# muhanzhang/IGMC

Measured on AMD Instinct MI355X. Metric: enclosing-subgraphs/sec (train step, batch=50) + test RMSE, higher is better.
Workload: dtype f32; 1 GPU; ml_1m, hop 1, max-nodes-per-hop 100, batch 50 per GPU, adj-dropout 0, dynamic-train, ARR 0.001, Adam; parallelism=dp1, global_batch=50, graphs_captured_before_timing=True, steps_per_graph_launch=100, group_steps=50

## Files before the change

### igmc_amd/csrc/capi.hip

```cpp
#include "launch.h"
#include "sortpool.h"
#include "g2_image.h"

#include <algorithm>
#include <climits>
#include <cmath>
#include <cstdio>
#include <cstring>
#include <map>
#include <string>
#include <vector>

static thread_local std::string g_err;
int g_igmc_prof_on = 0;

#define IGMC_FAIL(msg)                                                      \
  do {                                                                      \
    g_err = std::string(__func__) + ": " + (msg);                           \
    return 1;                                                               \
  } while (0)
#define HIPCHECK(expr)                                                      \
  do {                                                                      \
    hipError_t e_ = (expr);                                                 \
    if (e_ != hipSuccess) {                                                 \
// ... 626 lines not shown
  if (!out) IGMC_FAIL("null out");
  if (num_bases != 4) IGMC_FAIL("the gfx950 kernels are built for num_bases == 4 (reference Main.py:393)");
  if (num_relations < 1 || num_relations > 255) IGMC_FAIL("num_relations out of range");
  if (num_relations * num_labels + num_labels + 1 > 320) IGMC_FAIL("num_relations * num_labels too large for the layer-0 gradient kernel");
  if (num_labels < 2 || n_side < 0 || max_nodes < 1 || max_graphs < 1) IGMC_FAIL("bad sizes");
  HIPCHECK(hipSetDevice(device));
  igmc_model* m = new igmc_model();
  m->device = device;
  m->last_B = 0;
  m->last_training = 0;
  m->last_flags = 0;
  m->img_valid = 0;
  m->img_hint = 0;
  m->img_params = nullptr;
  ModelDev& d = m->d;
  d.img_current = 0;
  d.adam_m1 = nullptr;
  d.adam_m2 = nullptr;
  d.R = num_relations;
  d.Bs = 4;
  d.L = num_labels;
  d.S = n_side;
  d.D = 256 + n_side;
  int64_t off = 0;
  for (int l = 0; l < 4; ++l) {
    const int fin = l == 0 ? d.L : 32;
    d.off_basis[l] = off; off += (int64_t)4 * fin * 32;
    d.off_root[l] = off;  off += (int64_t)fin * 32;
    d.off_bias[l] = off;  off += 32;
    d.off_att[l] = off;   off += (int64_t)d.R * 4;
  }
  d.off_l1w = off; off += (int64_t)128 * d.D;
  d.off_l1b = off; off += 128;
  d.off_l2w = off; off += 128;
  d.off_l2b = off; off += 1;
  d.n_params = off;
  d.node_cap = max_nodes;
  d.edge_cap = max_edges;
  d.graph_cap = max_graphs;
  Allocs& M = m->mem;
  int fail = 0;
  const size_t N = (size_t)max_nodes, Bc = (size_t)max_graphs;
  for (int l = 0; l < 4; ++l) fail |= M.get(&d.h[l], N * 32) | M.get(&d.dpre[l], N * 32);
  fail |= M.get(&d.agg, N * 128);
  for (int l = 0; l < 3; ++l) fail |= M.get(&d.gagg[l], N * 128) | M.get(&d.Y[l], N * 128);
  fail |= M.get(&d.feat, Bc * d.D) | M.get(&d.a1, Bc * 128) | M.get(&d.lmask, Bc * 128) | M.get(&d.dz, Bc * 128) |
          M.get(&d.gfeat, Bc * d.D) | M.get(&d.err, Bc) | M.get(&d.cnt0, N * d.R * d.L);
  const size_t rows0 = (size_t)d.R * d.L + d.L + 1;
  d.ts_part = nullptr;
  d.ts_raw = nullptr;
  d.ts_stride = (d.R * 32 + 33) * 32;
  d.fin_stash = nullptr;
  d.datt_part = nullptr;
  if (d.R <= G2_NR * G2_NG_MAX)
  {
    fail |= M.get(&d.ts_part, (size_t)4 * IGMC_TS_BLOCKS * d.ts_stride) |
            M.get(&d.ts_raw, (size_t)4 * d.ts_stride + (size_t)4 * d.ts_stride / 32 * 4);
    if (!fail) d.datt_part = d.ts_raw + (size_t)4 * d.ts_stride;
  }
  if (d.R <= 128) fail |= M.get(&d.fin_stash, (size_t)4 * IGMC_STASH_LAYER + 16);
  d.g2_ex = nullptr;
  d.g2_fx = nullptr;
  d.g2_px = nullptr;
  d.g2_px_stride = 0;
  d.g2_w = nullptr;
  d.g2_graphs = 0;
  d.ex_nodes = 256;
  d.g2_ex_stride = (size_t)Bc * 2 * 32 * d.ex_nodes;
  const int wide = d.R <= G2_NR * G2_NG_MAX;
  const int xcd_ok = igmc_g2_xcd_ok();
  if (wide && Bc <= 2048 && xcd_ok) {
    fail |= M.get(&d.g2_ex, 5 * d.g2_ex_stride) | M.get(&d.g2_fx, Bc * 256) | M.get(&d.g2_w, g2_w_words(d.R, d.L));
    d.g2_graphs = (int)Bc;
    if (d.R <= G2_NR && Bc <= 1024) {
      d.g2_px_stride = (size_t)Bc * 2 * 32768;
      fail |= M.get(&d.g2_px, 5 * d.g2_px_stride);
    } else if (d.R <= G2_NR) {
      static bool told = false;
      if (!told) fprintf(stderr, "[igmc] batches of more than 1024 subgraphs: no plane-exchange regions -- the dense-layer / per-layer kernels take the steps, not the subgraph kernel\n");
      told = true;
    }
  } else if (wide) {
    fail |= M.get(&d.g2_w, g2_w_words(d.R, d.L));
  }
  fail |= M.get(&d.gs_bar, 2 * Bc + 1);
  fail |= M.get(&d.gs_ts, 4);
  d.gs_err = d.gs_bar ? d.gs_bar + 2 * Bc : nullptr;
  fail |= M.get(&d.wg_part, (size_t)4 * IGMC_WG_BLOCKS * igmc_wg_stride()) |
          M.get(&d.gatt_part, (size_t)3 * IGMC_GATHER_BLOCKS * d.R * 4) |
          M.get(&d.l0_part, (size_t)IGMC_L0_BLOCKS * rows0 * 32) |
          M.get(&d.graw, (size_t)3 * igmc_wg_stride() + 3 * d.R * 4 + rows0 * 32) | M.get(&d.arr_part, 4);
  d.side = nullptr;
  d.ctrl = nullptr;
  d.dcat[0] = d.dcat[1] = d.dcat[2] = nullptr;
  fail |= M.get(&m->done_ctr, 8);
  if (fail) {
    M.release();
    delete m;
    IGMC_FAIL("hipMalloc failed (model workspace)");
  }
  {
    hipStream_t st1, st2;
    if (hipStreamCreateWithFlags(&st1, hipStreamNonBlocking) != hipSuccess ||
        hipStreamCreateWithFlags(&st2, hipStreamNonBlocking) != hipSuccess) {
      M.release();
      delete m;
      IGMC_FAIL("hipStreamCreate failed");
    }
    m->ax.s1 = st1;
    m->ax.s2 = st2;
    for (int i = 0; i < 8; ++i) {
      hipEvent_t e;
      if (hipEventCreateWithFlags(&e, hipEventDisableTiming) != hipSuccess) IGMC_FAIL("hipEventCreate failed");
      m->ax.ev[i] = e;
    }
  }
  HIPCHECK(hipMemset(m->done_ctr, 0, 8 * sizeof(int)));
  HIPCHECK(hipMemset(m->d.gs_bar, 0, (2 * (size_t)max_graphs + 1) * sizeof(int)));
  {
    const unsigned long long ts0[4] = {~0ull, 0ull, 0ull, 0ull};
    HIPCHECK(hipMemcpy(m->d.gs_ts, ts0, sizeof(ts0), hipMemcpyHostToDevice));
  }
  if (m->d.g2_ex) {
    HIPCHECK(hipMemset(m->d.g2_ex, 0, 5 * m->d.g2_ex_stride * sizeof(unsigned long long)));
    HIPCHECK(hipMemset(m->d.g2_fx, 0, (size_t)max_graphs * 256 * sizeof(unsigned long long)));
    if (m->d.g2_px) HIPCHECK(hipMemset(m->d.g2_px, 0, 5 * m->d.g2_px_stride));
  }
  if (igmc_model_prepare(d)) {
    M.release();
    delete m;
    IGMC_FAIL("hipFuncSetAttribute failed");
  }
  *out = m;
  return 0;
}

extern "C" int igmc_debug_lin_mask(const igmc_model* m, uint8_t* h_out, int64_t n) {
  if (!m || !h_out) IGMC_FAIL("null argument");
  if (n < 0 || n > (int64_t)m->d.graph_cap * 128) IGMC_FAIL("mask size out of range");
  HIPCHECK(hipDeviceSynchronize());
  HIPCHECK(hipMemcpy(h_out, m->d.lmask, (size_t)n, hipMemcpyDeviceToHost));
  return 0;
}

extern "C" int igmc_debug_head_array(const igmc_model* m, int which, float* h_out, int64_t n) {
  if (!m || !h_out) IGMC_FAIL("null argument");
  if (which < 0 || which > 3) IGMC_FAIL("no such array");
  const float* src = which == 0 ? m->d.a1 : which == 1 ? m->d.dz : which == 2 ? m->d.feat : m->d.gfeat;
  if (n < 0 || n > (int64_t)m->d.graph_cap * (which < 2 ? 128 : m->d.D)) IGMC_FAIL("size out of range");
  HIPCHECK(hipDeviceSynchronize());
  HIPCHECK(hipMemcpy(h_out, src, (size_t)n * sizeof(float), hipMemcpyDeviceToHost));
  return 0;
}

extern "C" void igmc_model_destroy(igmc_model* m) {
  if (!m) return;
  for (int i = 0; i < 8; ++i) hipEventDestroy((hipEvent_t)m->ax.ev[i]);
  hipStreamDestroy((hipStream_t)m->ax.s1);
  hipStreamDestroy((hipStream_t)m->ax.s2);
  m->mem.release();
  delete m;
}

extern "C" int64_t igmc_param_count(const igmc_model* m) { return m ? m->d.n_params : 0; }

extern "C" int64_t igmc_param_offset(const igmc_model* m, int layer, int which, int64_t* count) {
  if (!m) return -1;
  const ModelDev& d = m->d;
  const int fin = (layer == 0) ? d.L : 32;
  int64_t off = -1, n = 0;
  switch (which) {
    case IGMC_P_BASIS: off = d.off_basis[layer & 3]; n = (int64_t)4 * fin * 32; break;
    case IGMC_P_ROOT: off = d.off_root[layer & 3]; n = (int64_t)fin * 32; break;
    case IGMC_P_BIAS: off = d.off_bias[layer & 3]; n = 32; break;
    case IGMC_P_ATT: off = d.off_att[layer & 3]; n = (int64_t)d.R * 4; break;
    case IGMC_P_LIN1_W: off = d.off_l1w; n = (int64_t)128 * d.D; break;
    case IGMC_P_LIN1_B: off = d.off_l1b; n = 128; break;
    case IGMC_P_LIN2_W: off = d.off_l2w; n = 128; break;
    case IGMC_P_LIN2_B: off = d.off_l2b; n = 1; break;
  }
  if (count) *count = n;
  return off;
}

static StepPlan plan_query(const igmc_model* m, const igmc_batch* b, int B) {
  StepPlan sp;
  igmc_step_plan(m->d, b->d, B, IGMC_CALL_STEP, &sp);
  return sp;
}

extern "C" int igmc_model_dense_layers(const igmc_model* m, const igmc_batch* b, int B) {
  return (m && b) ? plan_query(m, b, B).dense_layers : 0;
}

extern "C" int igmc_model_dense_path(const igmc_model* m, const igmc_batch* b, int B) {
  return (m && b) ? plan_query(m, b, B).family == IGMC_FAM_G2 : 0;
}

extern "C" int igmc_model_step_form(const igmc_model* m, const igmc_batch* b, int B) {
  return (m && b) ? plan_query(m, b, B).step_form : 0;
}

extern "C" int igmc_model_step_geometry(const igmc_model* m, const igmc_batch* b, int B, int32_t* out, int n) {
  if (!m || !b || !out || n < 0) IGMC_FAIL("bad arguments");
// ... 215 lines not shown
  if (n < 1 || n > (int64_t)INT32_MAX) IGMC_FAIL("n must be in [1, 2^31)");
  if (nq < 0 || nq > (int64_t)INT32_MAX) IGMC_FAIL("nq must be in [0, 2^31)");
  if (ns < 1 || geometry < 0 || geometry > IGMC_SEGSEL_MAX_SPLIT) IGMC_FAIL("ns must be at least 1, geometry in [0, 64]");
  igmc_launch_rank_segments(d_keys, d_ids, n, d_seg_off, ns, d_q_off, d_q_id, nq,
                            geometry > 0 ? geometry : igmc_segsel_default_split(ns), d_q_pos, d_q_rank, d_err, stream);
  HIPCHECK(hipGetLastError());
  return 0;
}
extern "C" int igmc_rank_metrics(const int32_t* d_q_rank, const int64_t* d_q_off, const uint8_t* d_q_rel, int64_t nq, int ns,
                                 const int32_t* d_ks, int nk, int32_t* d_cnt, double* d_dcg, int32_t* d_err, int grid,
                                 void* stream) {
  if (!d_q_off || !d_ks || !d_cnt || !d_dcg || !d_err) IGMC_FAIL("null argument");
  if (nq > 0 && !d_q_rank) IGMC_FAIL("null argument");
  if (nq < 0 || nq > (int64_t)INT32_MAX) IGMC_FAIL("nq must be in [0, 2^31)");
  if (ns < 1 || nk < 1 || nk > IGMC_RANK_MAX_KS || grid < 0 || grid > 65536)
    IGMC_FAIL("ns must be at least 1, nk in [1, 8], grid in [0, 65536]");
  igmc_launch_rank_metrics(d_q_rank, d_q_off, d_q_rel, d_ks, nk, ns, nq, grid, d_cnt, d_dcg, d_err, stream);
  HIPCHECK(hipGetLastError());
  return 0;
}

extern "C" int igmc_ctrl_tick(int64_t* d_ctrl, void* stream) {
  if (!d_ctrl) IGMC_FAIL("null ctrl");
  igmc_launch_tick(d_ctrl, stream);
  HIPCHECK(hipGetLastError());
  return 0;
}
extern "C" int igmc_ctrl_regroup(int64_t* d_ctrl, int M, int64_t first_cur, int64_t first_next, void* stream) {
  if (!d_ctrl || M < 1 || first_cur < 0 || first_next < 0) IGMC_FAIL("bad arguments");
  igmc_launch_regroup(d_ctrl, M, first_cur, first_next, stream);
  HIPCHECK(hipGetLastError());
  return 0;
}
extern "C" int igmc_ctrl_gate(int64_t* d_ctrl, int q, int gk_min, double delay_us, int delay_always, double timeout_us,
                              void* stream) {
  if (!d_ctrl || gk_min < 0 || !(timeout_us >= 0.0) || !(delay_us >= 0.0) || delay_us > 1000.0) IGMC_FAIL("bad arguments");
  igmc_launch_gate(d_ctrl, q & 1, gk_min, (long long)(delay_us * 100.0), delay_always != 0, (long long)(timeout_us * 100.0), stream);
  HIPCHECK(hipGetLastError());
  return 0;
}
extern "C" int igmc_batch_set_ctrl(igmc_batch* b, const int64_t* d_ctrl) {
  if (!b) IGMC_FAIL("null batch");
  b->ctrl = d_ctrl;
  return 0;
}
extern "C" int igmc_model_set_ctrl(igmc_model* m, const int64_t* d_ctrl) {
  if (!m) IGMC_FAIL("null model");
  m->d.ctrl = d_ctrl;
  return 0;
}
extern "C" int igmc_model_reset_exchange(igmc_model* m, void* stream) {
  if (!m) IGMC_FAIL("null model");
  hipStream_t st = (hipStream_t)stream;
  if (m->d.g2_ex) {
    HIPCHECK(hipMemsetAsync(m->d.g2_ex, 0, 5 * m->d.g2_ex_stride * sizeof(unsigned long long), st));
    HIPCHECK(hipMemsetAsync(m->d.g2_fx, 0, (size_t)m->d.g2_graphs * 256 * sizeof(unsigned long long), st));
    if (m->d.g2_px) HIPCHECK(hipMemsetAsync(m->d.g2_px, 0, 5 * m->d.g2_px_stride, st));
  }
  return 0;
}
extern "C" int igmc_model_check(igmc_model* m, void* stream) {
  if (!m) IGMC_FAIL("null model");
  int v = 0;
  if (m->d.gs_err) {
    HIPCHECK(hipStreamSynchronize((hipStream_t)stream));
    HIPCHECK(hipMemcpy(&v, m->d.gs_err, sizeof(int), hipMemcpyDeviceToHost));
    if (v) {
      HIPCHECK(hipMemset(m->d.gs_bar, 0, (2 * (size_t)m->d.graph_cap + 1) * sizeof(int)));
      (void)igmc_model_reset_exchange(m, stream);
      HIPCHECK(hipStreamSynchronize((hipStream_t)stream));
      IGMC_FAIL("a workgroup-cluster exchange of k_graph_step2 timed out (GPU shared with another job?): results of the "
                "affected steps are invalid; set IGMC_GS_CLUSTER=1 or IGMC_GRAPH_STEP=0");
    }
  }
  return 0;
}
extern "C" int igmc_adam_step_ctrl(float* d_params, const float* d_grad, float* d_exp_avg, float* d_exp_avg_sq,
                                   int64_t n, const int64_t* d_ctrl, void* stream) {
  if (!d_params || !d_grad || !d_exp_avg || !d_exp_avg_sq || n <= 0 || !d_ctrl) IGMC_FAIL("bad arguments");
  igmc_launch_adam(d_params, d_grad, d_exp_avg, d_exp_avg_sq, n, 0.f, 0.f, 0.f, 0.f, 0.f, 0.f, (int64_t*)d_ctrl, 0, stream);
  HIPCHECK(hipGetLastError());
  return 0;
}

extern "C" int igmc_step_finish(igmc_model* m, const igmc_batch* b, float* d_params, const float* d_grad,
                                float* d_exp_avg, float* d_exp_avg_sq, float ARR, float* d_loss, double* d_total,
                                int64_t* d_ctrl, int64_t step, float lr, float beta1, float beta2, float eps,
                                float weight_decay, void* stream) {
  if (!m || !b || !d_params || !d_grad || !d_exp_avg || !d_exp_avg_sq || !d_loss) IGMC_FAIL("bad arguments");
  if (!d_ctrl && step < 1) IGMC_FAIL("step must be >= 1");
  const AdamScalars as = adam_scalars(d_ctrl, step, lr, beta1, beta2);
  igmc_launch_finish(m->d, b->d, d_params, d_grad, d_exp_avg, d_exp_avg_sq, as.step_size, as.inv_sqrt_bc2, beta1, beta2, eps,
                     weight_decay, d_ctrl, ARR, d_loss, d_total, m->last_flags, stream);
  m->img_valid = 0;
  m->img_hint = 0;
  HIPCHECK(hipGetLastError());
  return 0;
}

extern "C" int igmc_train_step(igmc_model* m, float* d_params, const igmc_batch* b, int use_edge_flags,
                               const uint8_t* d_lin_mask, uint64_t seed, uint64_t step, float multiply_by, float ARR,
                               float* d_out, float* d_grad, float* d_exp_avg, float* d_exp_avg_sq, float* d_loss,
                               double* d_total, int64_t* d_ctrl, int64_t adam_t, float lr, float beta1, float beta2,
                               float eps, float weight_decay, void* stream) {
  std::string why;
  if (check_call(m, b, d_params && d_out && d_grad && d_exp_avg && d_exp_avg_sq && d_loss, &why)) IGMC_FAIL(why);
  if (!d_ctrl && adam_t < 1) IGMC_FAIL("adam_t must be >= 1");
  const AdamScalars as = adam_scalars(d_ctrl, adam_t, lr, beta1, beta2);
  const StepPlan sp = begin_call(m, b, IGMC_CALL_STEP, stream);
  ImgScope img(m, d_params);
  int emitted = 0;
  igmc_launch_train_step(m->d, b->d, sp, d_params, b->last_B, use_edge_flags, d_lin_mask, seed, step, multiply_by, ARR,
                         d_out, d_grad, d_exp_avg, d_exp_avg_sq, as.step_size, as.inv_sqrt_bc2, beta1, beta2, eps, weight_decay,
                         d_ctrl, m->done_ctr, d_loss, d_total, stream, 0.f, nullptr, &emitted);
  img.done_updated(emitted);
  HIPCHECK(hipGetLastError());
  end_call(m, b, 1, use_edge_flags);
  return 0;
}

#define IGMC_MAX_PEERS 16
struct igmc_comm {
  void* nccl;
  int rank, world, device;
  igmc_allreduce_fn host_fn;
// ... 564 lines not shown
```

### igmc_amd/csrc/g2_compose.h

```cpp
#pragma once

__global__ __launch_bounds__(G2C_THREADS) void k_g2_compose(ModelDev m, const float* P, float* w) {
  __shared__ float s_att[4 * G2_NR * G2_NG_MAX];
  const int tid = threadIdx.x, R = m.R, L = m.L, RL = R * L, LF = L * 32;
  const int ng = g2_groups(R, L);
  const int tableb = 2 * 3 * ng * (G2_NR + 1);
  const int mi = (int)(blockIdx.x >> 1);
  const int l = ((int)blockIdx.x >= tableb) ? 0 : 1 + mi / (ng * (G2_NR + 1)), trans = blockIdx.x & 1;
  if ((int)blockIdx.x >= tableb) {
    const int c0 = 32 * ((int)blockIdx.x - tableb);
    const float attv = (tid < R * 4) ? P[m.off_att[0] + tid] : 0.f;
    float bv[4][4], rv[4];
#pragma unroll
    for (int q = 0; q < 4; ++q) {
      const int i = tid + q * G2C_THREADS, c = c0 + (i >> 5), f = i & 31;
      const int cf = (c < RL) ? (c % L) * 32 + f : 0;
#pragma unroll
      for (int bb = 0; bb < 4; ++bb) bv[q][bb] = (c < RL) ? P[m.off_basis[0] + bb * LF + cf] : 0.f;
      rv[q] = (c >= RL && c < RL + L) ? P[m.off_root[0] + (c - RL) * 32 + f] : ((c == RL + L) ? P[m.off_bias[0] + f] : 0.f);
    }
    if (tid < 4 * G2_NR * G2_NG_MAX) s_att[tid] = attv;
    __syncthreads();
#pragma unroll
    for (int q = 0; q < 4; ++q) {
// ... 32 lines not shown
      } else {
#pragma unroll
        for (int q = 0; q < 4; ++q) bq[bb][q] = basis[bb * 1024 + (4 * kg + q) * 32 + n];
      }
    }
    float at[4];
#pragma unroll
    for (int bb = 0; bb < 4; ++bb) at[bb] = P[m.off_att[l] + r * 4 + bb];
#pragma unroll
    for (int q = 0; q < 4; ++q) v[q] = g2_wsum(at[0], at[1], at[2], at[3], bq[0][q], bq[1][q], bq[2][q], bq[3][q]);
  }
  uint32_t h01, m01, l01, h23, m23, l23;
  g2_split2(v[0], v[1], h01, m01, l01);
  g2_split2(v[2], v[3], h23, m23, l23);
  const int lane = (kg & 3) * 16 + (n & 15), nt = n >> 4, e0 = 4 * (kg >> 2);
  const uint32_t t3[3][2] = {{h01, h23}, {m01, m23}, {l01, l23}};
#pragma unroll
  for (int t = 0; t < G2_NT; ++t)
    *(uint2*)(img + ((size_t)(((t * (G2_NR + 1) + blk) * 2 + nt) * 64 + lane)) * 8 + e0) = make_uint2(t3[t][0], t3[t][1]);
}

static int igmc_g2_layout(const ModelDev& m, const BatchDev& b, int cs, G2Layout* lay) {
  const int RL = m.R * m.L;
  if (m.S != 0 || m.D != 256 || m.R > G2_NR || m.L > 8 || RL + m.L + 1 > 32 || !m.ts_part || !m.g2_px || !m.g2_fx || !m.g2_w || !b.relm) return 0;
  const int half = 2 * cs;
  const int cmax = b.cap_u > b.cap_v ? b.cap_u : b.cap_v;
  if (cmax > 16 * half || cmax > 128) return 0;
  if (b.graph_cap > m.g2_graphs) return 0;
  const int kmax = ((cmax + 31) >> 5) << 5;
  lay->kp = kmax + 8;
  lay->nsides = (cs == 1) ? 2 : 1;
  lay->rmr = ((cmax + 15) >> 4) << 4;
  lay->rmc = kmax;
  int o = 0;
  lay->pside = ((G2_NT * 32 * lay->kp * 2 + 1023) & ~1023) >> 2;
  lay->planes = o; o += lay->nsides * lay->pside;
  lay->ohp = o; o += lay->nsides * (8 * lay->kp >> 1);
  lay->lab = o; o += 64;
  lay->xo = o; o += 2 * G2_NB * 16 * G2_XP;
  lay->hs = o; o += G2_NB * 16 * G2_XP;
  int tw = G2_NB * 16 * G2_TP;
  if (tw < (G2_THREADS / 64) * 256) tw = (G2_THREADS / 64) * 256;
  const int rw = 2 * lay->rmr * (lay->rmc + 8) / 4;
  if (rw > tw) tw = rw;
  if (tw < 1024) tw = 1024;
  lay->tile = o; o += tw;
  lay->hist = o; o += G2_NB * 16 * G2_XP;
  lay->px = o; o += G2_NB * 2 * 64 * 4;
  lay->wreg = o; o += G2_WIMG;
  lay->t0 = o; o += 1024;
  lay->att = o; o += 64;
  lay->head = o; o += 256 + 256 + 3 * 128 + 512 + 16;
  lay->words = o;
  return (size_t)o * 4 <= 160 * 1024;
}

__global__ void k_g2_xcc_probe(int* out) {
  if (threadIdx.x == 0) out[blockIdx.x] = (int)(g2_xcc_id() & 15ull);
}
int igmc_g2_xcd_ok() {
#ifdef IGMC_HIPEMU
  return 1;
#else
  static int oks[64];
  static bool init = false;
  if (!init) {
    for (int i = 0; i < 64; ++i) oks[i] = -1;
    init = true;
  }
  int dev = 0;
  if (hipGetDevice(&dev) != hipSuccess || dev < 0 || dev >= 64) dev = 0;
  int& ok = oks[dev];
  if (ok >= 0) return ok;
  ok = 0;
  int* d = nullptr;
  int h[64];
  if (hipMalloc((void**)&d, sizeof(h)) != hipSuccess) return ok;
  hipLaunchKernelGGL(k_g2_xcc_probe, dim3(64), dim3(64), 0, 0, d);
  if (hipMemcpy(h, d, sizeof(h), hipMemcpyDeviceToHost) == hipSuccess) {
    ok = 1;
    for (int b = 0; b + 8 < 64; ++b)
      if (h[b] != h[b + 8]) ok = 0;
  }
  (void)hipFree(d);
  if (!ok) fprintf(stderr, "[igmc] device %d: workgroups b and b + 8 of a launch do not share an XCD: the subgraph kernel and the one-launch dense layers are not used\n", dev);
  return ok;
#endif
}

int g_igmc_compose_count = 0;

int igmc_launch_graph_step2(const ModelDev& m, const BatchDev& b, const StepPlan& sp, const float* P, int B, int training,
                            int use_flags, const uint8_t* inj_mask, uint64_t seed, uint64_t step, float mult, float grad_scale,
                            float* out, void* stream) {
  const G2Layout& lay = sp.lay;
  const int cs = sp.cs;
  G2Args a;
  memset(&a, 0, sizeof(a));
  a.n_users = b.n_users; a.n_items = b.n_items; a.B = B; a.s_lab = b.s_lab; a.relm = b.relm; a.y = b.y;
  a.cap_u = b.cap_u; a.cap_v = b.cap_v; a.slot = b.slot; a.relm_ld = b.relm_ld; a.graph_cap = b.graph_cap;
  a.R = m.R; a.L = m.L; a.D = m.D; a.ts_stride = m.ts_stride;
  for (int l = 0; l < 4; ++l) {
    a.h[l] = m.h[l];
    a.off_bias[l] = (int)m.off_bias[l];
  }
  a.ts_part = m.ts_part; a.g2_px = m.g2_px; a.g2_fx = m.g2_fx; a.g2_px_stride = m.g2_px_stride; a.g2_w = m.g2_w;
  a.gs_bar = m.gs_bar; a.gs_err = m.gs_err; a.a1 = m.a1; a.dz = m.dz; a.feat = m.feat; a.gfeat = m.gfeat; a.err = m.err;
  a.lmask = m.lmask; a.ctrl = m.ctrl;
  a.off_l1w = (int)m.off_l1w; a.off_l1b = (int)m.off_l1b; a.off_l2w = (int)m.off_l2w; a.off_l2b = (int)m.off_l2b;
  a.P = P;
  a.inj_mask = inj_mask;
  a.seed = seed;
  a.step = step;
  a.mult = mult;
  a.grad_scale = grad_scale;
  a.out = out;
  a.lay2 = lay;
  a.timing = getenv("IGMC_GS_TIMING") ? 1 : 0;
  a.ts = (g_igmc_prof_on == 2) ? m.gs_ts : nullptr;
  a.self_seq = (!training || a.ts) ? 1 : 0;
  a.cs = cs;
  a.stride = (cs > 1) ? ((B + 7) & ~7) : 1;
  const int grid = sp.grid;
  const size_t sm = (size_t)lay.words * 4;
  if (!m.img_current) {
    IGMC_PLAUNCH("k_g2_compose", k_g2_compose, 2 * 3 * g2_groups(m.R, m.L) * (G2_NR + 1) + g2_t0_rows(m.R, m.L) / 32, G2C_THREADS, 0, stream, m, P, m.g2_w);
    ++g_igmc_compose_count;
  }
#ifdef IGMC_HIPEMU
  if (cs > 1) {
    hipemu::rt().co_cs = cs;
    hipemu::rt().co_stride = 8;
    hipemu::rt().co_block = 8 * cs;
  }
#endif
  if (getenv("IGMC_GS_TRACE")) fprintf(stderr, "[igmc] k_graph_step B=%d train=%d flags=%d v2 kp=%d lds=%zu cluster=%d grid=%d\n", B, training, use_flags, lay.kp, sm, cs, grid);
  igmc_dispatch([&](auto uf, auto tr, auto cl) {
    IGMC_PLAUNCH(tr() ? "k_graph_step" : "k_graph_fwd", (k_graph_step2<uf(), tr(), cl()>), grid, G2_THREADS, sm, stream, a);
  }, use_flags != 0, training != 0, cs > 1);
  return a.self_seq ? 0 : 1;
}

int igmc_dl_prepare();
int igmc_gs_prepare() { return igmc_g2_prepare(); }
int igmc_g2_prepare() {
  if (igmc_dl_prepare()) return 1;
  (void)igmc_g2_xcd_ok();
#ifndef IGMC_HIPEMU
  const int mx = 160 * 1024;
  const void* fns[8] = {(const void*)k_graph_step2<true, true, true>,   (const void*)k_graph_step2<false, true, true>,
                        (const void*)k_graph_step2<true, false, true>,  (const void*)k_graph_step2<false, false, true>,
                        (const void*)k_graph_step2<true, true, false>,  (const void*)k_graph_step2<false, true, false>,
                        (const void*)k_graph_step2<true, false, false>, (const void*)k_graph_step2<false, false, false>};
  for (const void* fn : fns)
    if (hipFuncSetAttribute(fn, hipFuncAttributeMaxDynamicSharedMemorySize, mx) != hipSuccess) return 1;
#endif
  return 0;
}
```

### igmc_amd/csrc/g2_prims.h

```cpp
#pragma once

#ifdef IGMC_HIPEMU
#define G2_STAMP(k) do { } while (0)
#else
#define G2_STAMP(k)                                                                                        \
  do {                                                                                                     \
    if (a.timing && threadIdx.x == 0) {                                                                    \
      if (blockIdx.x == 0) g_g2_clk[k] = __builtin_readcyclecounter();                                     \
      else if (a.cs > 2 && (int)blockIdx.x == 8 * (a.cs / 2) && (k) < 40) g_g2_clk[64 + (k)] = __builtin_readcyclecounter(); \
    }                                                                                                      \
  } while (0)
#endif

#ifdef IGMC_HIPEMU
#define DL_STAMP(k) do { } while (0)
#else
#define DL_STAMP(k)                                                                               \
  do {                                                                                            \
    if (a.timing && threadIdx.x == 0 && (int)blockIdx.x == a.timing - 1 && (k) < 128)             \
      g_g2_clk[k] = __builtin_readcyclecounter();                                                 \
  } while (0)
#endif

#ifdef IGMC_HIPEMU
// ... 23 lines not shown
  const uint32_t eq = ~(t + 0x7F7F7F7Fu) & 0x80808080u;
  const uint32_t mask = (eq >> 7) * 0xFFu;
#ifdef IGMC_HIPEMU
  o01 = ((mask & 0xFFu) ? 0x3F80u : 0u) | ((mask & 0xFF00u) ? 0x3F800000u : 0u);
  o23 = ((mask & 0xFF0000u) ? 0x3F80u : 0u) | ((mask & 0xFF000000u) ? 0x3F800000u : 0u);
#else
  o01 = __builtin_amdgcn_perm(mask, mask, 0x01010000u) & 0x3F803F80u;
  o23 = __builtin_amdgcn_perm(mask, mask, 0x03030202u) & 0x3F803F80u;
#endif
}

template <bool FLAGS>
__device__ __forceinline__ uint32_t g2_bytemask(uint32_t w, uint32_t r1, int keepbit) {
  uint32_t mk = w & (0x01010101u * IGMC_RELM_CODE);
  if (FLAGS) mk &= ((w >> keepbit) & 0x01010101u) * IGMC_RELM_CODE;
  const uint32_t t = mk ^ (0x01010101u * r1);
  const uint32_t eq = ~(t + 0x7F7F7F7Fu) & 0x80808080u;
  return (eq >> 7) * 0xFFu;
}
__device__ __forceinline__ u32x4 g2_mask_frag(uint32_t m0, uint32_t m1) {
  u32x4 f;
#ifdef IGMC_HIPEMU
  f[0] = ((m0 & 0xFFu) ? 0x3F80u : 0u) | ((m0 & 0xFF00u) ? 0x3F800000u : 0u);
  f[1] = ((m0 & 0xFF0000u) ? 0x3F80u : 0u) | ((m0 & 0xFF000000u) ? 0x3F800000u : 0u);
  f[2] = ((m1 & 0xFFu) ? 0x3F80u : 0u) | ((m1 & 0xFF00u) ? 0x3F800000u : 0u);
  f[3] = ((m1 & 0xFF0000u) ? 0x3F80u : 0u) | ((m1 & 0xFF000000u) ? 0x3F800000u : 0u);
#else
  f[0] = __builtin_amdgcn_perm(m0, m0, 0x01010000u) & 0x3F803F80u;
  f[1] = __builtin_amdgcn_perm(m0, m0, 0x03030202u) & 0x3F803F80u;
  f[2] = __builtin_amdgcn_perm(m1, m1, 0x01010000u) & 0x3F803F80u;
  f[3] = __builtin_amdgcn_perm(m1, m1, 0x03030202u) & 0x3F803F80u;
#endif
  return f;
}

__device__ __forceinline__ float g2_tanh(float x) {
#ifdef IGMC_HIPEMU
  return tanhf(x);
#else
  return 1.f - 2.f * __builtin_amdgcn_rcpf(1.f + __expf(2.f * x));
#endif
}

template <int AUX = 0>
__device__ __forceinline__ void g2_glds16(const float4* src_wave, float4* lds_wave, int lane) {
#ifndef IGMC_HIPEMU
  __builtin_amdgcn_global_load_lds((const __attribute__((address_space(1))) void*)(src_wave + lane),
                                   (__attribute__((address_space(3))) void*)lds_wave, 16, 0, AUX);
#else
  lds_wave[lane] = src_wave[lane];
#endif
}

__device__ __forceinline__ void g2_pub_f32(unsigned long long* p, float v, uint32_t tag) {
#ifndef IGMC_HIPEMU
  __hip_atomic_store(p, ((unsigned long long)tag << 32) | (unsigned long long)__float_as_uint(v), __ATOMIC_RELAXED,
                     __HIP_MEMORY_SCOPE_WAVEFRONT);
#else
  uint32_t bits;
  memcpy(&bits, &v, 4);
  *p = ((unsigned long long)tag << 32) | (unsigned long long)bits;
#endif
}

#define G2_PX_BYTES 32768
#define G2_PX_FLAGS 28672
#define DLX_PX_BYTES 65536
#define DLX_PX_FLAGS 61440
__device__ __forceinline__ void g2_publish_planes(unsigned char* px, int kp, int f, int node0, const float (&v)[4]) {
  uint32_t h0, m0, l0, h1, m1, l1;
  g2_split2(v[0], v[1], h0, m0, l0);
  g2_split2(v[2], v[3], h1, m1, l1);
  unsigned char* p = px + ((size_t)f * kp + node0) * 2;
  const size_t ts = (size_t)32 * kp * 2;
  *(uint2*)p = make_uint2(h0, h1);
  *(uint2*)(p + ts) = make_uint2(m0, m1);
  *(uint2*)(p + 2 * ts) = make_uint2(l0, l1);
}
__device__ __forceinline__ void g2_flag_raise(unsigned char* px, int slot, uint32_t tag, int lane, int flags_off = G2_PX_FLAGS) {
#ifndef IGMC_HIPEMU
  asm volatile("s_waitcnt vmcnt(0)" ::: "memory");
  if (lane == 0) __hip_atomic_store((unsigned long long*)(px + flags_off) + slot, (unsigned long long)tag, __ATOMIC_RELAXED, __HIP_MEMORY_SCOPE_WAVEFRONT);
#else
  if (lane == 0) ((unsigned long long*)(px + flags_off))[slot] = (unsigned long long)tag;
#endif
}
__device__ __forceinline__ void g2_flags_wait(const unsigned char* px, int n, uint32_t tag, int lane, int* err, int flags_off = G2_PX_FLAGS) {
  const unsigned long long* fl = (const unsigned long long*)(px + flags_off);
  for (long it = 0;; ++it) {
#ifndef IGMC_HIPEMU
    const unsigned long long w = (lane < n) ? __hip_atomic_load(fl + lane, __ATOMIC_RELAXED, __HIP_MEMORY_SCOPE_AGENT) : (unsigned long long)tag;
#else
    const unsigned long long w = (lane < n) ? fl[lane] : (unsigned long long)tag;
#endif
    if (__ballot(w != (unsigned long long)tag) == 0ull) break;
    if (it > (1L << 20)) {
      *err = 1;
      break;
    }
#ifndef IGMC_HIPEMU
    __builtin_amdgcn_s_sleep(1);
#else
    hipemu::yield();
#endif
  }
}
__device__ __forceinline__ void g2_planes_load_exact(uint32_t* pl, const unsigned char* px, int bytes, int wave, int lane, int nwaves) {
  const int pieces = (bytes + 1023) >> 10;
  for (int c = wave; c < pieces; c += nwaves)
    if (c * 1024 + lane * 16 < bytes) g2_glds16<16>((const float4*)px + c * 64, (float4*)pl + c * 64, lane);
}
__device__ __forceinline__ void g2_planes_load(uint32_t* pl, const unsigned char* px, int kp, int wave, int lane, int nwaves) {
  const int pieces = (192 * kp + 1023) >> 10;
  for (int c = wave; c < pieces; c += nwaves) g2_glds16<16>((const float4*)px + c * 64, (float4*)pl + c * 64, lane);
}

__device__ __forceinline__ float g2_poll_f32(const unsigned long long* p, uint32_t tag, int* err) {
  for (long it = 0;; ++it) {
#ifndef IGMC_HIPEMU
    const unsigned long long w = __hip_atomic_load(p, __ATOMIC_RELAXED, __HIP_MEMORY_SCOPE_AGENT);
#else
    const unsigned long long w = *p;
#endif
    if ((uint32_t)(w >> 32) == tag) return __uint_as_float((uint32_t)w);
    if (it > (1L << 22)) {
      *err = 1;
      return 0.f;
    }
#ifndef IGMC_HIPEMU
    __builtin_amdgcn_s_sleep(2);
#else
    hipemu::yield();
#endif
  }
}

#ifdef IGMC_HIPEMU
#define G2_SCHED_BARRIER() do { } while (0)
#else
#define G2_SCHED_BARRIER() __builtin_amdgcn_sched_barrier(0)
#endif

__device__ __forceinline__ uint32_t g2_ld_seq(const int* gs_bar) {
#ifndef IGMC_HIPEMU
  return (uint32_t)__hip_atomic_load(gs_bar + 1, __ATOMIC_RELAXED, __HIP_MEMORY_SCOPE_AGENT);
#else
  return (uint32_t)gs_bar[1];
#endif
}
__device__ __forceinline__ bool g2_last_workgroup_advances(int* gs_bar) {
#ifndef IGMC_HIPEMU
  if (__hip_atomic_fetch_add(gs_bar, 1, __ATOMIC_RELAXED, __HIP_MEMORY_SCOPE_AGENT) != (int)gridDim.x - 1) return false;
  __hip_atomic_store(gs_bar, 0, __ATOMIC_RELAXED, __HIP_MEMORY_SCOPE_AGENT);
  __hip_atomic_fetch_add(gs_bar + 1, 1, __ATOMIC_RELAXED, __HIP_MEMORY_SCOPE_AGENT);
  return true;
#else
  if (gs_bar[0]++ != (int)gridDim.x - 1) return false;
  gs_bar[0] = 0;
  gs_bar[1] += 1;
  return true;
#endif
}
__device__ __forceinline__ void g2_wait_vm0() {
#ifndef IGMC_HIPEMU
  asm volatile("s_waitcnt vmcnt(0)" ::: "memory");
#endif
}
__device__ __forceinline__ unsigned long long g2_wall_clock() {
#ifndef IGMC_HIPEMU
  return (unsigned long long)wall_clock64();
#else
  return 0ull;
#endif
}
__device__ __forceinline__ unsigned long long g2_xcc_id() {
#ifndef IGMC_HIPEMU
  return (unsigned long long)__builtin_amdgcn_s_getreg((20 << 0) | (0 << 6) | (3 << 11));
#else
  return 0ull;
#endif
}
__device__ __forceinline__ void g2_clock_open(unsigned long long* ts) {
#ifndef IGMC_HIPEMU
  atomicMin(ts, (unsigned long long)wall_clock64());
#else
  (void)ts;
#endif
}
__device__ __forceinline__ void g2_clock_close(unsigned long long* ts, unsigned long long t1) {
// ... 23 lines not shown
```

### igmc_amd/csrc/g2_subgraph.h

```cpp
#pragma once

struct G2Args {
  const int32_t* n_users;
  const int32_t* n_items;
  int B;
  const uint8_t* s_lab;
  const uint8_t* relm;
  const float* y;
  int cap_u, cap_v, slot, relm_ld, graph_cap;
  int R, L, D, ts_stride;
  float* h[4];
  float* ts_part;
  unsigned char* g2_px;
  unsigned long long* g2_fx;
  size_t g2_px_stride;
  const float* g2_w;
  int* gs_bar;
  int* gs_err;
  float* a1;
  float* dz;
  float* feat;
  float* gfeat;
  float* err;
  uint8_t* lmask;
  const int64_t* ctrl;
  int off_bias[4];
  int off_l1w, off_l1b, off_l2w, off_l2b;
  const float* P;
  const uint8_t* inj_mask;
  uint64_t seed, step;
  float mult, grad_scale;
  float* out;
  unsigned long long* ts;
  int timing, cs, stride, self_seq;
  G2Layout lay2;
};

template <bool FLAGS, bool TRAIN, bool ONCE>
__global__ __launch_bounds__(G2_THREADS) void k_graph_step2(G2Args a) {
  __builtin_amdgcn_s_setprio(3);
  const float* P = a.P;
  IGMC_DYN_SMEM(smem);
  float* S = (float*)smem;
  const G2Layout lay = a.lay2;
  const int kp = lay.kp, nsides = lay.nsides;
  uint32_t* PLN = (uint32_t*)(S + lay.planes);
  uint32_t* OHP = (uint32_t*)(S + lay.ohp);
  unsigned char* slab = (unsigned char*)(S + lay.lab);
  float* XOA = S + lay.xo;
  float* HSS = S + lay.hs;
  float* TILES = S + lay.tile;
  float* HIST = S + lay.hist;
  float* PXA = S + lay.px;
  float2* sW2 = (float2*)(S + lay.wreg);
  float* sT0 = S + lay.t0;
  float* sfeat = S + lay.head;
  float* sgf = sfeat + 256;
  float* sa1 = sgf + 256;
  float* skeep = sa1 + 128;
  float* sdz = skeep + 128;
  float* sred = sdz + 128;
  float* misc = sred + 512;
  const int R = a.R, L = a.L, RL = R * L;
  const int tid = threadIdx.x, lane = tid & 63, wave = tid >> 6;
  const int li = lane & 15, kq = lane >> 4;
  const int B = a.B;
  const int ts = a.ts_stride;
  const int cs = a.cs;
  const int cm = (cs > 1) ? (int)((blockIdx.x >> 3) % cs) : 0;
  const int half = 2 * cs;
  const uint32_t seq = g2_ld_seq(a.gs_bar);
  const uint32_t tag0 = seq * 8u + 1u;
  const uint64_t step = a.ctrl ? (uint64_t)a.ctrl[IGMC_CTRL_STEP] : a.step;
  if (a.ts && tid == 0) g2_clock_open(a.ts);
  auto xtag = [&](int x) { return tag0 + (uint32_t)x; };
  G2_STAMP(0);
  if (a.timing && tid == 0 && blockIdx.x < 1024) {
    g_g2_wg[blockIdx.x][0] = g2_wall_clock();
    g_g2_wg[blockIdx.x][2] = g2_xcc_id();
  }

  const int g_first = (cs > 1) ? (int)(blockIdx.x / (8 * cs)) * 8 + (int)(blockIdx.x & 7) : (int)blockIdx.x;
  const int g_pre = (g_first < a.graph_cap) ? g_first : a.graph_cap - 1;
  const int pre_cu = a.n_users[g_pre], pre_cv = a.n_items[g_pre];
  const int ld = a.relm_ld;
  auto load_label = [&](int g2) {
    const int hi = (tid >> 7) & 1, t7 = tid & 127;
    const int capx = a.cap_u + hi * (a.cap_v - a.cap_u);
    return (int)a.s_lab[(size_t)g2 * a.slot + hi * a.cap_u + ((t7 < capx) ? t7 : 0)];
  };
  int labv_raw = 0;
  if (tid < 256) g2_glds16((const float4*)(a.g2_w + 6 * G2_WIMG) + (tid & ~63), (float4*)sT0 + (tid & ~63), tid & 63);
  const int tslot = (cs > 1) ? g_first + cm * a.stride : (int)blockIdx.x;
  f32x4 acc0 = (f32x4){0.f, 0.f, 0.f, 0.f};
  bool first_graph = true;
  G2_STAMP(1);

  int g = g_first;
  if (g < B) do {
    int tid_g = threadIdx.x;
    G2_OPAQUE(tid_g);
    const int tid = tid_g, lane = tid & 63, wave = tid >> 6;
    const int li = lane & 15, kq = lane >> 4;
    const int bw = wave >> 1, hf = wave & 1;
    const int gw = cm * G2_NB + bw;
    const int side = gw / half, bi = gw - side * half;
    labv_raw = load_label(g);
    uint32_t bw0[G2_KS], bw1[G2_KS];
    {
      const unsigned char* rmg = a.relm + (size_t)g * a.cap_u * ld;
      const uint32_t rrow = (uint32_t)(16 * bi + li);
#pragma unroll
      for (int s = 0; s < G2_KS; ++s) {
        const uint32_t c0 = (uint32_t)(32 * s + 8 * kq);
        if (side == 0) {
          const uint32_t* p4 = (const uint32_t*)(rmg + (rrow * (uint32_t)ld + c0));
          bw0[s] = p4[0];
          bw1[s] = p4[1];
        } else {
          const unsigned char* pc = rmg + (c0 * (uint32_t)ld + rrow);
          bw0[s] = (uint32_t)pc[0] | ((uint32_t)pc[ld] << 8) | ((uint32_t)pc[2 * ld] << 16) | ((uint32_t)pc[3 * ld] << 24);
          bw1[s] = (uint32_t)pc[4 * ld] | ((uint32_t)pc[5 * ld] << 8) | ((uint32_t)pc[6 * ld] << 16) | ((uint32_t)pc[7 * ld] << 24);
        }
      }
    }
    G2_STAMP(48);
    {
      const float4 z4 = make_float4(0.f, 0.f, 0.f, 0.f);
      for (int i = tid; i < 2 * G2_NB * 16 * G2_XP / 4; i += G2_THREADS) ((float4*)XOA)[i] = z4;
      for (int i = tid; i < G2_NB * 16 * G2_XP / 4; i += G2_THREADS) ((float4*)HIST)[i] = z4;
    }
    G2_STAMP(49);
    const int cu = first_graph ? pre_cu : a.n_users[g], cv = first_graph ? pre_cv : a.n_items[g];
// ... 426 lines not shown
            for (int s4 = 0; s4 < 4; ++s4) {
              av[s4] = Hb[(4 * s4 + kq) * G2_XP + m2w * 16 + li];
              const float* tb = Tb + (4 * s4 + kq) * G2_TP + li;
              const float* db = Db + (4 * s4 + kq) * G2_XP + li;
#pragma unroll
              for (int i3 = 0; i3 < 3; ++i3) {
                const int nt = 3 * wo + i3;
                bw3[s4][i3] = (nt < 2 * G2_NR) ? tb[nt * 16] : db[(nt - 2 * G2_NR) * 16];
              }
            }
            G2_SCHED_BARRIER();
#pragma unroll
            for (int s4 = 0; s4 < 4; ++s4)
#pragma unroll
              for (int i3 = 0; i3 < 3; ++i3)
                w3[i3] = __builtin_amdgcn_mfma_f32_16x16x4f32(av[s4], bw3[s4][i3], w3[i3], 0, 0, 0);
          }
#pragma unroll
          for (int i3 = 0; i3 < 3; ++i3) {
            const int m2 = m2w, nt = 3 * wo + i3;
            const int r = nt >> 1;
            if (r >= R && r < G2_NR) continue;
            float* pp = wpart + (kq * 4) * 32 + li + (r < R ? r : R) * 1024 + m2 * 512 + (nt & 1) * 16;
            if (first_graph) {
#pragma unroll
              for (int rr = 0; rr < 4; ++rr) pp[rr * 32] = w3[i3][rr];
            } else {
#pragma unroll
              for (int rr = 0; rr < 4; ++rr) pp[rr * 32] += w3[i3][rr];
            }
          }
        }
        G2_STAMP(22 + 5 * (3 - l));
        if (l > 1) fetch(6 - l);
        __syncthreads();
        G2_STAMP(23 + 5 * (3 - l));
      }

      if (wave < 4) {
        const int m2 = wave >> 1, wn = wave & 1;
        for (int wb = 0; wb < G2_NB; ++wb) {
          const float* Hb = HIST + wb * 16 * G2_XP;
          const float* Db = XOA + (G2_NB + wb) * 16 * G2_XP;
#pragma unroll
          for (int s4 = 0; s4 < 4; ++s4)
            acc0 = __builtin_amdgcn_mfma_f32_16x16x4f32(Hb[(4 * s4 + kq) * G2_XP + m2 * 16 + li],
                                                        Db[(4 * s4 + kq) * G2_XP + wn * 16 + li], acc0, 0, 0, 0);
        }
      }
      first_graph = false;
      __syncthreads();
      G2_STAMP(34);
    }
  } while (!ONCE && (g += (int)gridDim.x) < B);

  if (TRAIN && wave < 4) {
    float* part0 = a.ts_part + (size_t)tslot * ts;
    const int m2 = wave >> 1, wn = wave & 1;
#pragma unroll
    for (int rr = 0; rr < 4; ++rr) {
      const int c = m2 * 16 + kq * 4 + rr;
      if (c < RL + L + 1) part0[c * 32 + wn * 16 + li] = acc0[rr];
    }
  }
  if (tid == 0 && a.self_seq) {
    const unsigned long long t1 = a.ts ? g2_wall_clock() : 0ull;
    if (g2_last_workgroup_advances(a.gs_bar) && a.ts) g2_clock_close(a.ts, t1);
  }
  G2_STAMP(35);
  if (a.timing && tid == 0 && blockIdx.x < 1024) g_g2_wg[blockIdx.x][1] = g2_wall_clock();
}

extern "C" int igmc_debug_g2_wg_clocks(unsigned long long* out, int n_wg) {
#ifndef IGMC_HIPEMU
  if (n_wg > 1024) n_wg = 1024;
  if (hipDeviceSynchronize() != hipSuccess) return 1;
  if (hipMemcpyFromSymbol(out, HIP_SYMBOL(g_g2_wg), (size_t)n_wg * 3 * sizeof(unsigned long long)) != hipSuccess) return 1;
#else
  for (int i = 0; i < 3 * n_wg; ++i) out[i] = 0;
#endif
  return 0;
}

extern "C" int igmc_debug_g2_clocks(unsigned long long* out, int n) {
#ifndef IGMC_HIPEMU
  if (n > 128) n = 128;
  if (hipDeviceSynchronize() != hipSuccess) return 1;
  if (hipMemcpyFromSymbol(out, HIP_SYMBOL(g_g2_clk), (size_t)n * sizeof(unsigned long long)) != hipSuccess) return 1;
#else
  for (int i = 0; i < n; ++i) out[i] = 0;
#endif
  return 0;
}
```

### igmc_amd/csrc/graphstep2.hip

```cpp
#include "launch.h"
#include "g2_image.h"
#include "head_sub.h"
#include <stdlib.h>
#include <stdio.h>
#include <string.h>

#define G2_THREADS 512
#define G2_NB 4
#define G2C_THREADS 256
#define G2_KS 4
#define G2_TP (G2_NR * 32 + 4)
#define G2_XP 36
#define G2_FXTAG 7

__device__ unsigned long long g_g2_clk[128];
__device__ unsigned long long g_g2_wg[1024][3];
#include "g2_prims.h"

template <typename Frag>
__device__ __forceinline__ void g2_gather_h(const uint32_t* pl, int kp, int nks, Frag frag, int li, int kq, int hf, f32x4 (&acc)[G2_NR]) {
#pragma unroll
  for (int r = 0; r < G2_NR; ++r) acc[r] = (f32x4){0.f, 0.f, 0.f, 0.f};
  const int tstride = 32 * kp >> 1;
  const uint32_t* base = pl + ((16 * hf + li) * kp >> 1) + 4 * kq;
  u32x4 pf[2][G2_NT];
  auto request = [&](int s, int buf) {
#pragma unroll
    for (int sp = 0; sp < G2_NT; ++sp) pf[buf][sp] = *(const u32x4*)(base + sp * tstride + 16 * s);
  };
  request(0, 0);
#pragma unroll
  for (int s = 0; s < G2_KS; ++s) {
    if (s < nks) {
      if (s + 1 < G2_KS) request(s + 1, (s + 1) & 1);
      G2_SCHED_BARRIER();
#pragma unroll
      for (int r = 0; r < G2_NR; ++r) {
        const u32x4 fr = frag(r, s);
#pragma unroll
        for (int q = 0; q < G2_NT; ++q) acc[r] = g2_mfma_bf16(pf[s & 1][q], fr, acc[r]);
      }
      G2_SCHED_BARRIER();
    }
  }
}

__device__ __forceinline__ void g2_transform_h(const f32x4 (&acc)[G2_NR], const float* xrows, const uint32_t* sW, int li, int kq, int hf,
                                               f32x4 (&o)[2]) {
  f32x4 o0a = (f32x4){0.f, 0.f, 0.f, 0.f}, o0b = o0a, o1a = o0a, o1b = o0a;
  const float4 xv = *(const float4*)(xrows + li * G2_XP + 16 * hf + 4 * kq);
  const uint2* wf = (const uint2*)sW + 2 * (kq * 16 + li) + hf;
  uint2 bf[2][2 * G2_NT][2];
  auto request = [&](int st, int buf) {
#pragma unroll
    for (int t = 0; t < G2_NT; ++t)
// ... 114 lines not shown
```

### igmc_amd/csrc/launch.h

```cpp
#pragma once
#include "model.h"
#include <string.h>
#include <type_traits>

size_t igmc_extract_smem_bytes(const GraphDev& g);
void igmc_launch_extract(const GraphDev& g, const BatchDev& b, const int32_t* link_u, const int32_t* link_v,
                         const float* link_y, const int32_t* link_idx, int first, int B, int replay,
                         double sample_ratio, uint64_t seed, uint64_t epoch, const int64_t* ctrl, int lean, void* stream);
void igmc_launch_extract_set(const GraphDev& g, const BatchDev* d_set, const BatchDev& b0, int count, const int32_t* link_u,
                             const int32_t* link_v, const float* link_y, const int32_t* link_idx, int sel0, int B,
                             double sample_ratio, uint64_t seed, const int64_t* ctrl, float drop_p, int force_undirected,
                             uint64_t drop_seed, void* stream);
void igmc_launch_emit(const BatchDev& b, int B, void* stream);
void igmc_launch_emit_nodes(const BatchDev& b, int B, void* stream);
void igmc_launch_load_nodes(const BatchDev& b, const int64_t* uoff, const int32_t* unodes, const uint8_t* udist,
                            const int64_t* voff, const int32_t* vnodes, const uint8_t* vdist, const float* link_y,
                            const int32_t* link_idx, int first, int B, const int64_t* ctrl, void* stream);
void igmc_launch_edge_flags(const BatchDev& b, float p, int force_undirected, uint64_t seed, uint64_t step,
                            const int64_t* ctrl, void* stream);
void igmc_launch_relm_flags(const BatchDev& b, void* stream);
void igmc_launch_relm_dropout(const BatchDev& b, int B, float p, int force_undirected, uint64_t seed, uint64_t step,
                              const int64_t* ctrl, void* stream);
void igmc_launch_tick(int64_t* ctrl, void* stream);
void igmc_launch_regroup(int64_t* ctrl, int M, int64_t first_cur, int64_t first_next, void* stream);
// ... 51 lines not shown
                                 void* stream);
int igmc_segsel_default_split(int ns);
void igmc_launch_select_segments(const float* keys, const int64_t* seg_off, int ns, int num, int k, void* scratch,
                                 int32_t* idx_out, float* key_out, int32_t* count, void* stream);
#define IGMC_RANK_MAX_KS 8
void igmc_launch_rank_segments(const float* keys, const int32_t* ids, int64_t n, const int64_t* seg_off, int ns,
                               const int64_t* q_off, const int32_t* q_id, int64_t nq, int k, int32_t* q_pos, int32_t* q_rank,
                               int32_t* err, void* stream);
void igmc_launch_rank_metrics(const int32_t* q_rank, const int64_t* q_off, const uint8_t* q_rel, const int32_t* ks, int nk,
                              int ns, int64_t nq, int grid, int32_t* cnt, double* dcg, int32_t* err, void* stream);
int igmc_model_prepare(const ModelDev& m);
void igmc_launch_adam(float* p, const float* g, float* m1, float* m2, int64_t n, float step_size,
                      float inv_sqrt_bc2, float beta1, float beta2, float eps, float wd, int64_t* ctrl, int tick,
                      void* stream);
void igmc_launch_finish(const ModelDev& m, const BatchDev& b, float* p, const float* g, float* m1, float* m2,
                        float step_size, float inv_sqrt_bc2, float beta1, float beta2, float eps, float wd,
                        int64_t* ctrl, float ARR, float* loss, double* total, int use_flags, void* stream);

int igmc_g2_xcd_ok();
struct G2Layout {
  int kp, nsides, rmr, rmc, pside;
  int planes, ohp, lab, xo, hs, tile, hist, px, wreg, t0, att, head, words;
};
void igmc_launch_side_gather(const float* src, int S, const int32_t* link_idx, int first, int B, const int64_t* ctrl,
                             float* dst, void* stream);
int igmc_gs_prepare();
int igmc_g2_prepare();

#define IGMC_CALL_EVAL 0
#define IGMC_CALL_CONV 1
#define IGMC_CALL_STEP 2
#define IGMC_FAM_ROWS 0
#define IGMC_FAM_G2 1
#define IGMC_FAM_DLF 2
#define IGMC_FAM_DL 3
#define IGMC_TAIL_HANDOFF 0
#define IGMC_TAIL_TS 1
#define IGMC_TAIL_BS 2
struct StepPlan {
  int kind;
  int fast_head;
  int family;
  int cs, grid;
  G2Layout lay;
  int wide, dl, dlts, dlf, dlb;
  int nqu, nqv, dl_grid;
  int gsplit;
  int self_seq;
  int head_inside;
  int bwd_dense;
  int need_y;
  int tail;
  int exchange_inside;
  int needs_csr;
  int dense_layers;
  int step_form;
};
void igmc_step_plan(const ModelDev& m, const BatchDev& b, int B, int kind, StepPlan* p);
int igmc_dl_always();
void igmc_launch_g2_compose(const ModelDev& m, const float* P, void* stream);
void igmc_launch_dl_layer0(const ModelDev& m, const BatchDev& b, int B, int training, int use_flags, void* stream);
struct DlHead {
  const float* P;
  const uint8_t* inj_mask;
  uint64_t seed, step;
  float mult, grad_scale;
  float* out;
};
void igmc_launch_dl_bwd(const ModelDev& m, const BatchDev& b, const StepPlan& sp, int B, int use_flags, void* stream,
                        const DlHead* head = nullptr, int dense3 = 0);
void igmc_launch_dl_fwd(const ModelDev& m, const BatchDev& b, const StepPlan& sp, const float* P, int B, int training,
                        int use_flags, float* zero_out, void* stream);
void igmc_launch_head_sub(const ModelDev& m, const BatchDev& b, const float* P, int B, const uint8_t* inj_mask, uint64_t seed,
                          uint64_t step, float mult, float grad_scale, float* out, void* stream);
void igmc_launch_dl_layer(const ModelDev& m, const BatchDev& b, const float* P, int B, int l, int bwd, int use_flags,
                          float* zero_out, void* stream, int tables = 0);
int igmc_launch_graph_step2(const ModelDev& m, const BatchDev& b, const StepPlan& sp, const float* P, int B, int training,
                            int use_flags, const uint8_t* inj_mask, uint64_t seed, uint64_t step, float mult, float grad_scale,
                            float* out, void* stream);

void igmc_prof_begin(const char* name, void* stream);
void igmc_prof_end(void* stream);
extern int g_igmc_prof_on;

#define IGMC_PLAUNCH(name, kern, grid, block, shmem, stream, ...)          \
  do {                                                                     \
    if (g_igmc_prof_on == 1) igmc_prof_begin(name, stream);                \
    IGMC_LAUNCH(kern, grid, block, shmem, stream, __VA_ARGS__);            \
    if (g_igmc_prof_on == 1) igmc_prof_end(stream);                        \
  } while (0)

template <typename F>
static inline void igmc_dispatch(F&& f) { f(); }
template <typename F, typename... Rest>
static inline void igmc_dispatch(F&& f, bool v, Rest... rest) {
  if (v) igmc_dispatch([&](auto... cs) { f(std::true_type{}, cs...); }, rest...);
  else igmc_dispatch([&](auto... cs) { f(std::false_type{}, cs...); }, rest...);
}
```

### igmc_amd/csrc/model.h

```cpp
#pragma once
#include "common.h"

#define IGMC_KCAT 160
#ifndef IGMC_WG_BLOCKS
#define IGMC_WG_BLOCKS 64
#endif
#define IGMC_STASH_LAYER 672
#define IGMC_TS_BLOCKS 256
#define IGMC_GATHER_BLOCKS 4096
#define IGMC_FBS_MAX_R 32
#define IGMC_L0_BLOCKS 256
#define IGMC_HG 8

struct ModelDev {
  int R, Bs, L, S, D;
  int64_t off_basis[4], off_root[4], off_bias[4], off_att[4];
  int64_t off_l1w, off_l1b, off_l2w, off_l2b, n_params;
  int node_cap, edge_cap, graph_cap;
  float* h[4];
  float* agg;
  float* gagg[3];
  float* Y[3];
  float* dpre[4];
  float* feat;
  float* a1;
  uint8_t* lmask;
  float* dz;
  float* gfeat;
  float* err;
  uint16_t* cnt0;
  float* wg_part;
  float* gatt_part;
  float* l0_part;
  float* graw;
  float* ts_part;
  float* ts_raw;
  int ts_stride;
  float* fin_stash;
  float* datt_part;
  int* gs_bar;
  int* gs_err;
  unsigned long long* gs_ts;
  unsigned long long* g2_ex;
  size_t g2_ex_stride;
  unsigned long long* g2_fx;
  unsigned char* g2_px;
  size_t g2_px_stride;
  int g2_graphs;
  float* g2_w;
  int ex_nodes;
  int img_current;
  const float* adam_m1;
  const float* adam_m2;
  float* arr_part;
  const float* dcat[3];
  const float* side;
  const int64_t* ctrl;
};

static inline int igmc_wg_stride() { return 32 * IGMC_KCAT + 32; }

__device__ __forceinline__ float igmc_wave_sum_f(float v) {
#pragma unroll
  for (int d = 32; d >= 1; d >>= 1) v += __shfl_xor(v, d, 64);
  return v;
}
__device__ __forceinline__ float igmc_group16_sum_f(float v) {
#ifdef IGMC_HIPEMU
#pragma unroll
  for (int d = 8; d >= 1; d >>= 1) v += __shfl_xor(v, d, 16);
  return v;
#else
  v += __int_as_float(__builtin_amdgcn_update_dpp(0, __float_as_int(v), 0x128, 0xf, 0xf, false));
  v += __int_as_float(__builtin_amdgcn_update_dpp(0, __float_as_int(v), 0x124, 0xf, 0xf, false));
  v += __int_as_float(__builtin_amdgcn_update_dpp(0, __float_as_int(v), 0x122, 0xf, 0xf, false));
  v += __int_as_float(__builtin_amdgcn_update_dpp(0, __float_as_int(v), 0x121, 0xf, 0xf, false));
  return v;
#endif
}
__device__ __forceinline__ float igmc_block_sum_f(float v, float* sm) {
  v = igmc_wave_sum_f(v);
  const int lane = threadIdx.x & 63, wave = threadIdx.x >> 6;
  if (lane == 0) sm[wave] = v;
  __syncthreads();
  float tot = 0.f;
  const int nw = (blockDim.x + 63) >> 6;
  for (int w = 0; w < nw; ++w) tot += sm[w];
  __syncthreads();
  return tot;
}

__device__ __forceinline__ void ctrl_advance(int64_t* ctrl) {
// ... 18 lines not shown
```

### igmc_amd/csrc/model.hip

```cpp
#include "model.h"
#include "g2_image.h"
#include <stdlib.h>

struct XcdSeg {
  int lo, hi;
  int j, nj;
};
__device__ __forceinline__ XcdSeg igmc_xcd_segment(const BatchDev& b) {
  XcdSeg s;
  const int B = b.totals[3];
  const int x = blockIdx.x & 7;
  s.j = blockIdx.x >> 3;
  s.nj = (gridDim.x + 7 - x) >> 3;
  s.lo = b.node_off[(x * B) >> 3];
  s.hi = b.node_off[((x + 1) * B) >> 3];
  return s;
}


template <bool FLAGS, bool STORE>
__global__ __launch_bounds__(IGMC_BLOCK) void k_l0_fwd(BatchDev b, ModelDev m, const float* __restrict__ P,
                                                         float* __restrict__ out) {
  igmc_kernarg_warm<sizeof(BatchDev) + sizeof(ModelDev) + 32>();
  IGMC_DYN_SMEM(smem);
  const int RL = m.R * m.L, LF = m.L * 32;
  float* sW0 = (float*)smem;
  float* sroot = sW0 + RL * 32;
  float* sbias = sroot + LF;
  int* shist = (int*)(sbias + 32);
  for (int i = threadIdx.x; i < RL * 32; i += IGMC_BLOCK) {
    const int r = i / LF, cf = i % LF;
    float s = 0.f;
#pragma unroll
    for (int bb = 0; bb < 4; ++bb) s += P[m.off_att[0] + r * 4 + bb] * P[m.off_basis[0] + bb * LF + cf];
    sW0[i] = s;
  }
  for (int i = threadIdx.x; i < LF; i += IGMC_BLOCK) sroot[i] = P[m.off_root[0] + i];
  if (threadIdx.x < 32) sbias[threadIdx.x] = P[m.off_bias[0] + threadIdx.x];
  __syncthreads();
  const int N = b.totals[0];
  const int lane = threadIdx.x & 63, wave = threadIdx.x >> 6;
  const int grp = lane >> 4, t = lane & 15;
  int* hist = shist + wave * RL;
  const XcdSeg seg = igmc_xcd_segment(b);
  (void)N;
  for (int i = seg.lo + seg.j * 4 + wave; i < seg.hi; i += seg.nj * 4) {
    float ax = 0.f, ay = 0.f;
    if (STORE) {
      for (int c = lane; c < RL; c += 64) hist[c] = 0;
      IGMC_WAVE_SYNC();
    }
    const int beg = b.row_ptr[i], end = b.row_ptr[i + 1];
    for (int c0 = beg + grp * 16; c0 < end; c0 += 64) {
      const int e = c0 + t;
// ... 1038 lines not shown
#pragma unroll
    for (int u = 0; u < 8; ++u) {
      const bool ok = g0 + 4 * u + kq < B;
      if (!ok) { av[u] = 0.f; bv[u] = 0.f; }
      if (extra) {
        dpv[u] = ok ? (from_err ? 2.f * dpv[u] * grad_scale : dpv[u]) * mult : 0.f;
        ad[u] = (ok && mk[u]) ? ad[u] * drop_scale : 0.f;
      }
    }
#pragma unroll
    for (int u = 0; u < 8; ++u) {
      acc = __builtin_amdgcn_mfma_f32_16x16x4f32(av[u], bv[u], acc, 0, 0, 0);
      if (extra) {
        accb1 = __builtin_amdgcn_mfma_f32_16x16x4f32(av[u], (g0 + 4 * u + kq < B) ? 1.f : 0.f, accb1, 0, 0, 0);
        accw2 = __builtin_amdgcn_mfma_f32_16x16x4f32(ad[u], dpv[u], accw2, 0, 0, 0);
        accb2 = __builtin_amdgcn_mfma_f32_16x16x4f32(1.f, dpv[u], accb2, 0, 0, 0);
      }
    }
  }
#pragma unroll
  for (int rr = 0; rr < 4; ++rr) grad[m.off_l1w + (int64_t)(j0 + kq * 4 + rr) * D + n0 + li] = acc[rr];
  if (extra && li == 0) {
#pragma unroll
    for (int rr = 0; rr < 4; ++rr) {
      grad[m.off_l1b + j0 + kq * 4 + rr] = accb1[rr];
      grad[m.off_l2w + j0 + kq * 4 + rr] = accw2[rr];
    }
    if (bx == 0 && kq == 0) grad[m.off_l2b] = accb2[0];
  }
}

__global__ __launch_bounds__(IGMC_BLOCK) void k_head_bwd_w_mfma(BatchDev b, ModelDev m, const float* __restrict__ P,
                                                                  const float* __restrict__ gout, int from_err,
                                                                  float grad_scale, float mult, float drop_scale,
                                                                  float* __restrict__ grad) {
  igmc_kernarg_warm<sizeof(BatchDev) + sizeof(ModelDev) + 32>();
  head_bwd_w_body(b, m, P, gout, from_err, grad_scale, mult, drop_scale, grad, blockIdx.x, blockIdx.y);
}

__global__ __launch_bounds__(IGMC_BLOCK) void k_wgrad_head(BatchDev b, ModelDev m, const float* __restrict__ P,
                                                             const float* __restrict__ gout, int from_err,
                                                             float grad_scale, float mult, float drop_scale,
                                                             float* __restrict__ grad, int nsl) {
  igmc_kernarg_warm<sizeof(BatchDev) + sizeof(ModelDev) + 32>();
  if ((int)blockIdx.y < nsl) {
    wgrad_body(b, m, blockIdx.y);
  } else {
    const int ny = (m.D / 16 + 3) / 4;
    if ((int)blockIdx.x < 8 * ny)
      head_bwd_w_body(b, m, P, gout, from_err, grad_scale, mult, drop_scale, grad, blockIdx.x & 7, blockIdx.x >> 3);
  }
}

__device__ __forceinline__ void fin_stash_body(const ModelDev& m, const float* __restrict__ P, int l, const int64_t* ctrl);

__global__ __launch_bounds__(IGMC_BLOCK) void k_reduce_partials(ModelDev m, int n_gatt_parts, int l0_mfma,
                                                                  int n_wg_parts, const float* __restrict__ P,
                                                                  const int64_t* ctrl, int nstash) {
  igmc_kernarg_warm<sizeof(ModelDev) + 32>();
  __shared__ float sred[4][64];
  if (nstash && (int)blockIdx.x >= (int)gridDim.x - nstash) {
    fin_stash_body(m, P, (int)blockIdx.x - ((int)gridDim.x - nstash), ctrl);
    return;
  }
  const int wgs = 32 * IGMC_KCAT + 32, na = m.R * 4, rows0 = m.R * m.L + m.L + 1, n0 = rows0 * 32;
  const int nlay = l0_mfma ? 4 : 3;
  const int nblkA = (nlay * wgs + 63) / 64, nblkB = (3 * na + 3) / 4, nblkC = l0_mfma ? 0 : (n0 + 63) / 64;
  const int lane = threadIdx.x & 63, wave = threadIdx.x >> 6;
  int blk = blockIdx.x;
  if (blk < nblkA + nblkC) {
    const bool secA = blk < nblkA;
    const int o = (secA ? blk : blk - nblkA) * 64 + lane;
    const int nout = secA ? nlay * wgs : n0;
    float s = 0.f;
    if (o < nout) {
      if (secA) {
        const int l = o / wgs, i = o % wgs;
        const float* p = m.wg_part + (size_t)l * IGMC_WG_BLOCKS * wgs + i;
        for (int k0 = wave; k0 < n_wg_parts; k0 += 64) {
          float v[16];
#pragma unroll
          for (int u = 0; u < 16; ++u) {
            const int k = k0 + 4 * u;
            v[u] = p[(size_t)(k < n_wg_parts ? k : n_wg_parts - 1) * wgs];
          }
#pragma unroll
          for (int u = 0; u < 16; ++u)
            if (k0 + 4 * u < n_wg_parts) s += v[u];
        }
      } else {
        const float* p = m.l0_part + o;
        for (int k0 = wave; k0 < IGMC_L0_BLOCKS; k0 += 64) {
          float v[16];
#pragma unroll
          for (int u = 0; u < 16; ++u) {
            const int k = k0 + 4 * u;
            v[u] = p[(size_t)(k < IGMC_L0_BLOCKS ? k : IGMC_L0_BLOCKS - 1) * n0];
          }
#pragma unroll
          for (int u = 0; u < 16; ++u)
            if (k0 + 4 * u < IGMC_L0_BLOCKS) s += v[u];
        }
      }
    }
    sred[wave][lane] = s;
    __syncthreads();
    if (wave == 0 && o < nout) {
      const float tot = (sred[0][lane] + sred[1][lane]) + (sred[2][lane] + sred[3][lane]);
      if (secA && o >= 3 * wgs) {
        const int i = o - 3 * wgs, c = i / IGMC_KCAT, col = i % IGMC_KCAT;
        if (i < 32 * IGMC_KCAT && c < rows0 && col >= 128) m.graw[3 * wgs + 3 * na + c * 32 + (col - 128)] = tot;
      } else {
        m.graw[secA ? o : 3 * wgs + 3 * na + o] = tot;
      }
    }
  } else {
    blk -= nblkA + nblkC;
    const int o = blk * 4 + wave;
    if (o < 3 * na && blk < nblkB) {
      const int l = o / na, i = o % na;
      const float* p = m.gatt_part + (size_t)l * IGMC_GATHER_BLOCKS * na + i;
      float s = 0.f;
      for (int k0 = lane; k0 < n_gatt_parts; k0 += 64 * 8) {
        float v[8];
#pragma unroll
        for (int u = 0; u < 8; ++u) {
          const int k = k0 + 64 * u;
          v[u] = p[(size_t)(k < n_gatt_parts ? k : n_gatt_parts - 1) * na];
        }
#pragma unroll
        for (int u = 0; u < 8; ++u)
          if (k0 + 64 * u < n_gatt_parts) s += v[u];
      }
      s = igmc_wave_sum_f(s);
      if (lane == 0) m.graw[3 * wgs + o] = s;
    }
  }
}

__device__ __forceinline__ void reduce_ts_body(const ModelDev& m, int nparts, int stride, int B, int blk,
                                               const float* __restrict__ Pold = nullptr) {
  __shared__ float4 sred4[16][16];
  const int ts = m.ts_stride, rows0 = m.R * m.L + m.L + 1;
  const int lane = threadIdx.x & 63, wave = threadIdx.x >> 6;
  const int o4 = lane & 15, pg = wave * 4 + (lane >> 4);
  const int o0 = blk * 64 + 4 * o4;
  const int l = o0 / ts, i0 = o0 % ts;
  const bool ok4 = l < 4 && (l > 0 || i0 < rows0 * 32);
  float pbv[4] = {0.f, 0.f, 0.f, 0.f};
  if (Pold && wave == 0) {
    const int o = blk * 64 + lane, lo_ = o / ts, i = o % ts;
    if (lo_ < 4) {
      const int nE = ((lo_ == 0) ? m.L : 32) * 32;
      if (i < m.R * nE) {
        const float* basis = Pold + m.off_basis[lo_] + i % nE;
#pragma unroll
        for (int bb = 0; bb < 4; ++bb) pbv[bb] = basis[bb * nE];
      }
    }
  }
  float4 s4 = make_float4(0.f, 0.f, 0.f, 0.f);
  if (ok4) {
    const float* p = m.ts_part + (size_t)l * IGMC_TS_BLOCKS * ts + i0;
    const int ng = (nparts < stride) ? nparts : ((B < stride) ? B : stride), cs = (nparts + stride - 1) / stride;
    const int nq = cs * ng;
    for (int q0 = pg; q0 < nq; q0 += 16 * 14) {
      float4 v[14];
#pragma unroll
      for (int u = 0; u < 14; ++u) {
        const int q = q0 + 16 * u, qc = q < nq ? q : nq - 1;
        const int c = qc / ng, g = qc - c * ng;
        v[u] = *(const float4*)(p + (size_t)(c * stride + g) * ts);
      }
#pragma unroll
      for (int u = 0; u < 14; ++u)
        if (q0 + 16 * u < nq) {
          s4.x += v[u].x; s4.y += v[u].y; s4.z += v[u].z; s4.w += v[u].w;
        }
    }
  }
  sred4[pg][o4] = s4;
  __syncthreads();
  if (wave == 0) {
    const float* sr = (const float*)sred4;
    float tot = 0.f;
#pragma unroll
    for (int g16 = 0; g16 < 16; ++g16) tot += sr[(g16 * 16 + (lane >> 2)) * 4 + (lane & 3)];
    const int o = blk * 64 + lane;
    const int lo_ = o / ts, i = o % ts;
    const bool ok = lo_ < 4 && (lo_ > 0 || i < rows0 * 32);
    if (!ok) tot = 0.f;
    if (ok) m.ts_raw[o] = tot;
    if (Pold) {
      float pb[4];
#pragma unroll
      for (int bb = 0; bb < 4; ++bb) pb[bb] = tot * pbv[bb];
#pragma unroll
      for (int bb = 0; bb < 4; ++bb)
#pragma unroll
        for (int d = 16; d >= 1; d >>= 1) pb[bb] += __shfl_xor(pb[bb], d, 64);
      if ((lane & 31) == 0 && lo_ < 4) *(float4*)(m.datt_part + (size_t)(o >> 5) * 4) = make_float4(pb[0], pb[1], pb[2], pb[3]);
    }
  }
}

#define IGMC_STASH_G 0
#define IGMC_STASH_M 16
#define IGMC_STASH_ATTM1 32
#define IGMC_STASH_ATTM2 96
#define IGMC_STASH_ATT 160
#define IGMC_STASH_SCAL (4 * IGMC_STASH_LAYER)
__device__ __forceinline__ void fin_stash_body(const ModelDev& m, const float* __restrict__ P, int l,
                                               const int64_t* ctrl) {
  __shared__ float sg10[4][10];
  __shared__ float sG[16];
  __shared__ float s_att[128];
  const int tid = threadIdx.x, lane = tid & 63, wave = tid >> 6;
  const int nE = ((l == 0) ? m.L : 32) * 32, R = m.R, na = R * 4;
  const float* basis = P + m.off_basis[l];
  const float* attg = P + m.off_att[l];
  float* st = m.fin_stash + l * IGMC_STASH_LAYER;
  const bool small = na <= 128;
  const float attv = (small && tid < na) ? attg[tid] : 0.f;
  float bq[4][4];
#pragma unroll
  for (int it = 0; it < 4; ++it) {
    const int e = tid + it * IGMC_BLOCK, ec = e < nE ? e : nE - 1;
#pragma unroll
    for (int q = 0; q < 4; ++q) bq[it][q] = (e < nE) ? basis[q * nE + ec] : 0.f;
  }
  float m1v = 0.f, m2v = 0.f;
  const bool mom = m.adam_m1 && na <= 64 && tid >= 128 && tid < 128 + na;
  if (mom) {
    m1v = m.adam_m1[m.off_att[l] + tid - 128];
    m2v = m.adam_m2[m.off_att[l] + tid - 128];
  }
  double scal = 0.0;
  const bool sc = l == 0 && ctrl && tid >= 192 && tid < 198;
  if (sc) {
    const double* d = (const double*)ctrl;
    const int k = tid - 192;
    const int src = (k == 0) ? IGMC_CTRL_STEP_SIZE : (k == 1) ? IGMC_CTRL_INV_SQRT_BC2 : (k == 2) ? IGMC_CTRL_BETA1
                  : (k == 3) ? IGMC_CTRL_BETA2 : (k == 4) ? IGMC_CTRL_EPS : IGMC_CTRL_WD;
    scal = d[src];
  }
  if (small && tid < na) s_att[tid] = attv;
  float gp[10];
#pragma unroll
  for (int q = 0; q < 10; ++q) gp[q] = 0.f;
#pragma unroll
  for (int it = 0; it < 4; ++it) {
    if (tid + it * IGMC_BLOCK < nE) {
      const float b0 = bq[it][0], b1 = bq[it][1], b2 = bq[it][2], b3 = bq[it][3];
      gp[0] += b0 * b0; gp[1] += b0 * b1; gp[2] += b0 * b2; gp[3] += b0 * b3;
      gp[4] += b1 * b1; gp[5] += b1 * b2; gp[6] += b1 * b3;
      gp[7] += b2 * b2; gp[8] += b2 * b3; gp[9] += b3 * b3;
    }
  }
  for (int e = tid + 4 * IGMC_BLOCK; e < nE; e += IGMC_BLOCK) {
    const float b0 = basis[e], b1 = basis[nE + e], b2 = basis[2 * nE + e], b3 = basis[3 * nE + e];
    gp[0] += b0 * b0; gp[1] += b0 * b1; gp[2] += b0 * b2; gp[3] += b0 * b3;
    gp[4] += b1 * b1; gp[5] += b1 * b2; gp[6] += b1 * b3;
    gp[7] += b2 * b2; gp[8] += b2 * b3; gp[9] += b3 * b3;
  }
#pragma unroll
  for (int q = 0; q < 10; ++q) gp[q] = igmc_wave_sum_f(gp[q]);
  if (lane == 0) {
#pragma unroll
    for (int q = 0; q < 10; ++q) sg10[wave][q] = gp[q];
  }
  __syncthreads();
  const float* att = small ? (const float*)s_att : attg;
  if (tid >= 64 && tid < 80) {
    const int bb = (tid - 64) >> 2, bp = tid & 3;
    float sacc = 0.f;
    for (int r = 0; r < R; ++r) {
      const float dm = (r > 0) ? att[r * 4 + bp] - att[(r - 1) * 4 + bp] : 0.f;
      const float dn = (r + 1 < R) ? att[(r + 1) * 4 + bp] - att[r * 4 + bp] : 0.f;
      sacc += att[r * 4 + bb] * 2.f * (dm - dn);
    }
    st[IGMC_STASH_M + tid - 64] = sacc;
  }
  if (tid >= 128 && na <= IGMC_STASH_LAYER - IGMC_STASH_ATT) {
    for (int i = tid - 128; i < na; i += IGMC_BLOCK - 128) {
      st[IGMC_STASH_ATT + i] = att[i];
      if (m.adam_m1 && na <= 64) {
        st[IGMC_STASH_ATTM1 + i] = mom && i == tid - 128 ? m1v : m.adam_m1[m.off_att[l] + i];
        st[IGMC_STASH_ATTM2 + i] = mom && i == tid - 128 ? m2v : m.adam_m2[m.off_att[l] + i];
      }
    }
  }
  if (sc) m.fin_stash[IGMC_STASH_SCAL + tid - 192] = (float)scal;
  if (tid == 0) {
    const int ij[10][2] = {{0, 0}, {0, 1}, {0, 2}, {0, 3}, {1, 1}, {1, 2}, {1, 3}, {2, 2}, {2, 3}, {3, 3}};
    for (int q = 0; q < 10; ++q) {
      const float v = (sg10[0][q] + sg10[1][q]) + (sg10[2][q] + sg10[3][q]);
      sG[ij[q][0] * 4 + ij[q][1]] = v;
      sG[ij[q][1] * 4 + ij[q][0]] = v;
    }
    float reg = 0.f;
    for (int r = 0; r + 1 < R; ++r) {
      float d[4];
      for (int q = 0; q < 4; ++q) d[q] = att[(r + 1) * 4 + q] - att[r * 4 + q];
      for (int p1 = 0; p1 < 4; ++p1)
        for (int p2 = 0; p2 < 4; ++p2) reg += d[p1] * sG[p1 * 4 + p2] * d[p2];
    }
    m.arr_part[l] = reg;
    for (int q = 0; q < 16; ++q) st[IGMC_STASH_G + q] = sG[q];
  }
}

__global__ __launch_bounds__(IGMC_BLOCK) void k_tail_ts(BatchDev b, ModelDev m, const float* __restrict__ P,
                                                          float grad_scale, float mult, float drop_scale,
                                                          float* __restrict__ grad, int nlin, int nparts, int stride,
                                                          int B, int nstash, const int64_t* ctrl, int bump_seq) {
  __builtin_amdgcn_s_setprio(3);
  igmc_kernarg_warm<sizeof(BatchDev) + sizeof(ModelDev) + 64>();
  const int nred = (int)gridDim.x - nlin - nstash;
  if (bump_seq && blockIdx.x == 0 && threadIdx.x == 0) m.gs_bar[1] += 1;
  if ((int)blockIdx.x < nlin)
    head_bwd_w_body(b, m, P, nullptr, 1, grad_scale, mult, drop_scale, grad, blockIdx.x & 7, blockIdx.x >> 3, B);
  else if ((int)blockIdx.x < nlin + nred)
    reduce_ts_body(m, nparts, stride, B, blockIdx.x - nlin, nstash ? P : nullptr);
  else
    fin_stash_body(m, P, blockIdx.x - nlin - nred, ctrl);
}

struct FinishArgs {
  int enabled;
  int use_flags;
  BatchDev b;
  ModelDev m;
  float ARR;
  float* loss;
  double* total;
};

__device__ __forceinline__ void ctrl_check_and_advance(int64_t* ctrl, const BatchDev& b, int use_flags) {
  const int64_t gq = ctrl[IGMC_CTRL_GQ] & 1;
  const int64_t want = ctrl[gq ? IGMC_CTRL_FIRST_ODD : IGMC_CTRL_FIRST] + ctrl[IGMC_CTRL_GK] * ctrl[IGMC_CTRL_BATCH];
  const int64_t got = b.stamp[0];
  int bad = 0;
  if (got >= 0 && got != want) bad |= 2;
  if (use_flags && got >= 0 && b.stamp[1] >= 0 && (uint64_t)b.stamp[1] != igmc_ctrl_drop_key(ctrl, (int)want)) bad |= 4;
  if (bad) ctrl[IGMC_CTRL_SYNC_ERR] |= bad;
  ctrl_advance(ctrl);
}

__device__ __forceinline__ void loss_body(const BatchDev& b, const ModelDev& m, float ARR, float* loss,
                                          double* total, float* smf) {
  const int B = b.totals[3];
  float s = 0.f;
  for (int g = threadIdx.x; g < B; g += IGMC_BLOCK) s += m.err[g] * m.err[g];
  s = igmc_block_sum_f(s, smf);
  if (threadIdx.x == 0) {
    const float reg = m.arr_part[0] + m.arr_part[1] + m.arr_part[2] + m.arr_part[3];
    const float l0 = s / (float)B + ARR * reg;
    loss[0] = l0;
    loss[1] = s;
    if (total) total[0] += (double)l0 * (double)B;
  }
}

__device__ __forceinline__ void adam_elem(float* __restrict__ p, const float* __restrict__ g, float* __restrict__ m1,
                                          float* __restrict__ m2, int64_t i, float step_size, float inv_sqrt_bc2,
                                          float beta1, float beta2, float eps, float wd) {
  float gi = g[i];
  const float pi = p[i];
  if (wd != 0.f) gi += wd * pi;
  const float a = beta1 * m1[i] + (1.f - beta1) * gi;
  const float v = beta2 * m2[i] + (1.f - beta2) * gi * gi;
  m1[i] = a;
  m2[i] = v;
  p[i] = pi - step_size * a / (sqrtf(v) * inv_sqrt_bc2 + eps);
}

template <int NB>
__device__ __forceinline__ void adam_range(float* p, const float* g, float* m1, float* m2, int64_t lo, int64_t hi,
                                           float step_size, float inv_sqrt_bc2, float beta1, float beta2, float eps,
                                           float wd) {
  for (int64_t i0 = lo + threadIdx.x; i0 < hi; i0 += (int64_t)NB * IGMC_BLOCK) {
    float gv[NB], pv[NB], av[NB], vv[NB];
#pragma unroll
    for (int k = 0; k < NB; ++k) {
      const int64_t i = i0 + (int64_t)k * IGMC_BLOCK;
      const int64_t ic = i < hi ? i : hi - 1;
      gv[k] = g[ic];
      pv[k] = p[ic];
      av[k] = m1[ic];
      vv[k] = m2[ic];
    }
#pragma unroll
    for (int k = 0; k < NB; ++k) {
      const int64_t i = i0 + (int64_t)k * IGMC_BLOCK;
      if (i < hi) {
        float gi = gv[k];
        if (wd != 0.f) gi += wd * pv[k];
        const float a = beta1 * av[k] + (1.f - beta1) * gi;
        const float v = beta2 * vv[k] + (1.f - beta2) * gi * gi;
        m1[i] = a;
        m2[i] = v;
        p[i] = pv[k] - step_size * a / (sqrtf(v) * inv_sqrt_bc2 + eps);
      }
    }
  }
}

struct AdamTail {
  int enabled;
  float* p;
  float* m1;
  float* m2;
  float step_size, inv_sqrt_bc2, beta1, beta2, eps, wd;
  int64_t* ctrl;
  int* done;
  BatchDev b;
  float ARR;
  float* loss;
  double* total;
  int use_flags;
  const int* skip;
};

#define IGMC_FIN_NB 8
__global__ __launch_bounds__(IGMC_BLOCK) void k_finalize(ModelDev m, const float* P, float* __restrict__ grad,
                                                           float arr_coef, AdamTail at, int ts_mode) {
  igmc_kernarg_warm<sizeof(ModelDev) + sizeof(AdamTail) + 32>();
  if (at.skip && *at.skip) return;
  __shared__ float smf[8];
  __shared__ float sG[16], sM[16];
  __shared__ int s_lastl;
  __shared__ float sg10[4][10];
  __shared__ int s_last;
  if (at.enabled && at.ctrl) {
    const double* d = (const double*)at.ctrl;
    at.step_size = (float)d[IGMC_CTRL_STEP_SIZE];
    at.inv_sqrt_bc2 = (float)d[IGMC_CTRL_INV_SQRT_BC2];
    at.beta1 = (float)d[IGMC_CTRL_BETA1];
    at.beta2 = (float)d[IGMC_CTRL_BETA2];
    at.eps = (float)d[IGMC_CTRL_EPS];
    at.wd = (float)d[IGMC_CTRL_WD];
  }
  auto finish = [&](int64_t i, float g) { grad[i] = g; };
  if (blockIdx.x >= 4 * IGMC_FIN_NB) {
    const int64_t n_lin = m.n_params - m.off_l1w;
    const int nb = gridDim.x - 4 * IGMC_FIN_NB;
    const int64_t chunk = (n_lin + nb - 1) / nb;
    const int64_t lo = m.off_l1w + (int64_t)(blockIdx.x - 4 * IGMC_FIN_NB) * chunk;
    const int64_t hi = (lo + chunk < m.n_params) ? lo + chunk : m.n_params;
    adam_range<8>(at.p, grad, at.m1, at.m2, lo, hi, at.step_size, at.inv_sqrt_bc2, at.beta1, at.beta2, at.eps, at.wd);
  } else {
    const int l = blockIdx.x / IGMC_FIN_NB, part = blockIdx.x % IGMC_FIN_NB, tid = threadIdx.x;
    const int lane = tid & 63, wave = tid >> 6;
    const int fin = (l == 0) ? m.L : 32;
    const int nE = fin * 32;
    const int wgs = 32 * IGMC_KCAT + 32, na = m.R * 4, R = m.R;
// ... 99 lines not shown
      if (lane == 0) finish(m.off_att[l] + rb, g);
    }
    if (at.enabled) {
      __syncthreads();
      if (tid == 0) {
        __threadfence();
        s_lastl = (atomicAdd(at.done + 1 + l, 1) == IGMC_FIN_NB - 1);
      }
      __syncthreads();
      if (s_lastl) {
        __threadfence();
        adam_range<12>(at.p, grad, at.m1, at.m2, m.off_basis[l], m.off_att[l] + na, at.step_size, at.inv_sqrt_bc2,
                       at.beta1, at.beta2, at.eps, at.wd);
        if (tid == 0) at.done[1 + l] = 0;
      }
    }
  }
  if (at.enabled) {
    __syncthreads();
    if (threadIdx.x == 0) {
      __threadfence();
      s_last = (atomicAdd(at.done, 1) == (int)gridDim.x - 1);
    }
    __syncthreads();
    if (s_last) {
      __threadfence();
      loss_body(at.b, m, at.ARR, at.loss, at.total, smf);
      if (threadIdx.x == 0) {
        *at.done = 0;
        if (at.ctrl) ctrl_check_and_advance(at.ctrl, at.b, at.use_flags);
      }
    }
  }
}

#define IGMC_FTS_NB 4
__device__ __forceinline__ float fts_emit(float* __restrict__ grad, const AdamTail& at, int64_t i, float g, float pold,
                                          float m1old, float m2old, bool store = true) {
  if (store) grad[i] = g;
  if (!at.enabled) return pold;
  float gi = g;
  if (at.wd != 0.f) gi += at.wd * pold;
  const float a = at.beta1 * m1old + (1.f - at.beta1) * gi;
  const float v = at.beta2 * m2old + (1.f - at.beta2) * gi * gi;
  const float pnew = pold - at.step_size * a / (sqrtf(v) * at.inv_sqrt_bc2 + at.eps);
  if (store) {
    at.m1[i] = a;
    at.m2[i] = v;
    at.p[i] = pnew;
  }
  return pnew;
}

__global__ __launch_bounds__(IGMC_BLOCK) void k_finalize_ts(ModelDev m, const float* P, float* __restrict__ grad,
                                                              float arr_coef, AdamTail at, int nlin, int bs, int img) {
  __builtin_amdgcn_s_setprio(3);
  igmc_kernarg_warm<sizeof(ModelDev) + sizeof(AdamTail) + 48>();
  if (at.skip && *at.skip) return;
  __shared__ float smf[8];
  const int tid = threadIdx.x;
  const float* stash = m.fin_stash;
  if (at.enabled && at.ctrl) {
    at.step_size = stash[IGMC_STASH_SCAL + 0];
    at.inv_sqrt_bc2 = stash[IGMC_STASH_SCAL + 1];
    at.beta1 = stash[IGMC_STASH_SCAL + 2];
    at.beta2 = stash[IGMC_STASH_SCAL + 3];
    at.eps = stash[IGMC_STASH_SCAL + 4];
    at.wd = stash[IGMC_STASH_SCAL + 5];
  }
  if ((int)blockIdx.x < 4 * IGMC_FTS_NB) {
    const int l = blockIdx.x / IGMC_FTS_NB, part = blockIdx.x % IGMC_FTS_NB;
    const int fin = (l == 0) ? m.L : 32, nE = fin * 32, R = m.R, na = R * 4;
    const float* stg = stash + l * IGMC_STASH_LAYER;
    __shared__ float s_st[IGMC_STASH_LAYER];
    float stq[(IGMC_STASH_LAYER + IGMC_BLOCK - 1) / IGMC_BLOCK];
#pragma unroll
    for (int u = 0; u < (IGMC_STASH_LAYER + IGMC_BLOCK - 1) / IGMC_BLOCK; ++u) {
      const int i = tid + u * IGMC_BLOCK;
      stq[u] = stg[i < IGMC_STASH_LAYER ? i : IGMC_STASH_LAYER - 1];
    }
    const float* st = s_st;
    const int wgs = 32 * IGMC_KCAT + 32;
    const bool table = !bs || l == 0;
    const float* t0 = bs ? m.graw + 3 * wgs + 3 * na : m.ts_raw + (size_t)l * m.ts_stride;
    const float* raw = m.graw + (size_t)(l >= 1 ? l - 1 : 0) * wgs;
    __shared__ float s_gatt0[512];
    if (bs && l == 0) {
      if (part == 0) {
        __shared__ float s_gpart[IGMC_BLOCK / 64][32];
        const int lane = tid & 63, wave = tid >> 6;
        if (R <= 8) {
          float acc[32];
#pragma unroll
          for (int i = 0; i < 32; ++i) acc[i] = 0.f;
          for (int e0 = 0; e0 < nE; e0 += IGMC_BLOCK) {
            const int e = e0 + tid, ec = e < nE ? e : nE - 1;
            float tv[8], bq[4];
#pragma unroll
            for (int r = 0; r < 8; ++r) tv[r] = t0[(size_t)(r < R ? r : R - 1) * nE + ec];
#pragma unroll
            for (int bb = 0; bb < 4; ++bb) bq[bb] = P[m.off_basis[0] + (int64_t)bb * nE + ec];
#pragma unroll
            for (int r = 0; r < 8; ++r)
#pragma unroll
              for (int bb = 0; bb < 4; ++bb)
                if (r < R && e < nE) acc[r * 4 + bb] += tv[r] * bq[bb];
// ... 46 lines not shown
      m2v[q] = (has && at.enabled) ? at.m2[idx[q]] : 0.f;
      g[q] = 0.f;
    }
#pragma unroll
    for (int r = 0; r < 8; ++r) tv[r] = 0.f;
    if (has) {
      if (table) {
#pragma unroll
        for (int r = 0; r < 8; ++r) tv[r] = (r < R) ? t0[(size_t)r * nE + e] : 0.f;
        g[4] = t0[(size_t)R * nE + e];
      } else {
#pragma unroll
        for (int bb = 0; bb < 4; ++bb) g[bb] = raw[(e >> 5) * IGMC_KCAT + bb * 32 + (e & 31)];
        g[4] = raw[(e >> 5) * IGMC_KCAT + 128 + (e & 31)];
      }
    }
    const bool roles = part == 0 || emit;
    const bool bias_role = roles && tid < 32 && part == 0;
    const bool att_role = roles && !bias_role && tid >= 64 && tid - 64 < na;
    float bq[4] = {0.f, 0.f, 0.f, 0.f};
    if (bias_role) {
      const int64_t i = m.off_bias[l] + tid;
      bq[0] = table ? t0[(size_t)(R * fin + fin) * 32 + tid] : raw[32 * IGMC_KCAT + tid];
      bq[1] = P[i];
      bq[2] = at.enabled ? at.m1[i] : 0.f;
      bq[3] = at.enabled ? at.m2[i] : 0.f;
    }
    float dpre[32], am1 = 0.f, am2 = 0.f, ag = 0.f;
#pragma unroll
    for (int k = 0; k < 32; ++k) dpre[k] = 0.f;
    if (att_role) {
      const int rb = tid - 64, r = rb >> 2, bb = rb & 3;
      const int64_t i = m.off_att[l] + rb;
      if (at.enabled && !emit) {
        am1 = at.m1[i];
        am2 = at.m2[i];
      }
      if (bs) {
        if (l > 0) ag = m.graw[3 * wgs + (size_t)(l - 1) * na + rb];
      } else {
        const float* dp = m.datt_part + ((size_t)l * m.ts_stride + (size_t)r * nE) / 32 * 4 + bb;
#pragma unroll
        for (int k = 0; k < 32; ++k) dpre[k] = (k < fin) ? dp[(size_t)k * 4] : 0.f;
      }
    }
#pragma unroll
    for (int u = 0; u < (IGMC_STASH_LAYER + IGMC_BLOCK - 1) / IGMC_BLOCK; ++u) {
      const int i = tid + u * IGMC_BLOCK;
      if (i < IGMC_STASH_LAYER) s_st[i] = stq[u];
    }
    __syncthreads();
    if (roles) {
      if (bias_role) {
        const int64_t i = m.off_bias[l] + tid;
        const float bnew = fts_emit(grad, at, i, bq[0], bq[1], bq[2], bq[3]);
        if (emit && l == 0) m.g2_w[g2_t0_off(ng) + (R * fin + fin) * 32 + tid] = bnew;
      } else if (tid >= 64) {
       for (int rb = tid - 64; rb < na; rb += IGMC_BLOCK - 64) {
        const int r = rb >> 2, bb = rb & 3;
        const bool first = rb == tid - 64;
        const int64_t i = m.off_att[l] + rb;
        const float pold = st[IGMC_STASH_ATT + rb];
        const float m1o = !at.enabled ? 0.f : emit ? st[IGMC_STASH_ATTM1 + rb] : first ? am1 : at.m1[i];
        const float m2o = !at.enabled ? 0.f : emit ? st[IGMC_STASH_ATTM2 + rb] : first ? am2 : at.m2[i];
        float g = 0.f;
        if (bs) {
          g = (l == 0) ? s_gatt0[rb] : first ? ag : m.graw[3 * wgs + (size_t)(l - 1) * na + rb];
        } else if (first && fin <= 32) {
#pragma unroll
          for (int k = 0; k < 32; ++k) g += dpre[k];
        } else {
          const float* dp = m.datt_part + ((size_t)l * m.ts_stride + (size_t)r * nE) / 32 * 4 + bb;
          for (int k0 = 0; k0 < fin; k0 += 32) {
            float v[32];
#pragma unroll
            for (int k = 0; k < 32; ++k) v[k] = (k0 + k < fin) ? dp[(size_t)(k0 + k) * 4] : 0.f;
#pragma unroll
            for (int k = 0; k < 32; ++k) g += v[k];
          }
        }
        if (arr_coef != 0.f) {
          float sacc = 0.f;
          for (int bp = 0; bp < 4; ++bp) {
            const float a0 = st[IGMC_STASH_ATT + r * 4 + bp];
            const float dm = (r > 0) ? a0 - st[IGMC_STASH_ATT + (r - 1) * 4 + bp] : 0.f;
            const float dn = (r + 1 < R) ? st[IGMC_STASH_ATT + (r + 1) * 4 + bp] - a0 : 0.f;
            sacc += 2.f * (dm - dn) * st[IGMC_STASH_G + bp * 4 + bb];
          }
          g += arr_coef * sacc;
        }
        const float anew = fts_emit(grad, at, i, g, pold, m1o, m2o, part == 0);
        if (emit) s_attn[rb] = anew;
       }
      }
    }
    if (has) {
      if (table) {
#pragma unroll
        for (int r = 0; r < 8; ++r)
          if (r < R) {
#pragma unroll
            for (int bb = 0; bb < 4; ++bb) g[bb] += st[IGMC_STASH_ATT + r * 4 + bb] * tv[r];
          }
        for (int r = 8; r < R; ++r) {
          const float tvr = t0[(size_t)r * nE + e];
#pragma unroll
          for (int bb = 0; bb < 4; ++bb) g[bb] += st[IGMC_STASH_ATT + r * 4 + bb] * tvr;
        }
      }
      if (arr_coef != 0.f) {
#pragma unroll
        for (int bb = 0; bb < 4; ++bb)
          g[bb] += arr_coef * (st[IGMC_STASH_M + bb * 4 + 0] * pv[0] + st[IGMC_STASH_M + bb * 4 + 1] * pv[1] +
                               st[IGMC_STASH_M + bb * 4 + 2] * pv[2] + st[IGMC_STASH_M + bb * 4 + 3] * pv[3]);
      }
#pragma unroll
      for (int q = 0; q < 5; ++q) pn[q] = fts_emit(grad, at, idx[q], g[q], pv[q], m1v[q], m2v[q]);
      e_img = e;
    }
    if (emit) {
      __syncthreads();
      if (e_img >= 0) {
        const int c = e_img >> 5, f = e_img & 31;
        if (l == 0) {
          float* t0w = m.g2_w + g2_t0_off(ng);
          for (int r = 0; r < R; ++r)
            t0w[(r * fin + c) * 32 + f] = g2_wsum(s_attn[r * 4], s_attn[r * 4 + 1], s_attn[r * 4 + 2], s_attn[r * 4 + 3],
                                                  pn[0], pn[1], pn[2], pn[3]);
          t0w[(R * fin + c) * 32 + f] = pn[4];
        } else {
#pragma unroll 3
          for (int r = 0; r <= R; ++r) {
            const float v = (r == R) ? pn[4]
                          : g2_wsum(s_attn[r * 4], s_attn[r * 4 + 1], s_attn[r * 4 + 2], s_attn[r * 4 + 3], pn[0], pn[1], pn[2], pn[3]);
            const int grp = (r == R) ? 0 : r / G2_NR, blk = (r == R) ? G2_NR : r % G2_NR;
            uint16_t* imf = (uint16_t*)(m.g2_w + g2_img_off(ng, l, 0, grp));
            uint16_t* imt = (uint16_t*)(m.g2_w + g2_img_off(ng, l, 1, grp));
            uint32_t h, mi, lo;
            g2_split2(v, 0.f, h, mi, lo);
            const uint32_t t3[3] = {h, mi, lo};
#pragma unroll
            for (int t = 0; t < G2_NT; ++t) {
              imf[g2_img_index(t, blk, c, f)] = (uint16_t)t3[t];
              imt[g2_img_index(t, blk, f, c)] = (uint16_t)t3[t];
            }
          }
        }
      }
    }
  } else if ((int)blockIdx.x < 4 * IGMC_FTS_NB + nlin) {
    const int64_t n_lin = m.n_params - m.off_l1w;
    const int64_t chunk = (n_lin + nlin - 1) / nlin;
    const int64_t lo = m.off_l1w + (int64_t)(blockIdx.x - 4 * IGMC_FTS_NB) * chunk;
    const int64_t hi = (lo + chunk < m.n_params) ? lo + chunk : m.n_params;
    adam_range<8>(at.p, grad, at.m1, at.m2, lo, hi, at.step_size, at.inv_sqrt_bc2, at.beta1, at.beta2, at.eps, at.wd);
  } else {
    loss_body(at.b, m, at.ARR, at.loss, at.total, smf);
    if (tid == 0 && at.ctrl) ctrl_check_and_advance(at.ctrl, at.b, at.use_flags);
  }
}

__global__ __launch_bounds__(IGMC_BLOCK) void k_loss(BatchDev b, ModelDev m, float ARR, float* __restrict__ loss) {
  igmc_kernarg_warm<sizeof(BatchDev) + sizeof(ModelDev) + 32>();
  __shared__ float smf[8];
  loss_body(b, m, ARR, loss, nullptr, smf);
}

__global__ __launch_bounds__(IGMC_BLOCK) void k_sse_acc(BatchDev b, const float* __restrict__ out, double* acc, int64_t* ctrl) {
  igmc_kernarg_warm<sizeof(BatchDev) + 32>();
  __shared__ float smf[8];
  const int B = b.totals[3];
  float s = 0.f;
  for (int g = threadIdx.x; g < B; g += IGMC_BLOCK) {
    const float d = out[g] - b.y[g];
    s += d * d;
  }
  s = igmc_block_sum_f(s, smf);
  if (threadIdx.x == 0) {
    acc[0] += (double)s;
    acc[1] += (double)B;
    if (ctrl) ctrl_advance(ctrl);
  }
}

__global__ void k_tick(int64_t* ctrl) {
  if (threadIdx.x == 0 && blockIdx.x == 0) ctrl_advance(ctrl);
}
__global__ void k_regroup(int64_t* ctrl, int M, int64_t first_cur, int64_t first_next) {
  if (threadIdx.x != 0 || blockIdx.x != 0) return;
  ctrl[IGMC_CTRL_GROUP] = M > 0 ? M : 1;
  ctrl[IGMC_CTRL_GK] = 0;
  ctrl[IGMC_CTRL_GQ] = 0;
  ctrl[IGMC_CTRL_FIRST] = first_cur;
  ctrl[IGMC_CTRL_FIRST_ODD] = first_next;
}

__global__ void k_step_gate(int64_t* ctrl, int q, int gk_min, long long delay_ticks, int delay_always,
                            long long timeout_ticks) {
#ifndef IGMC_HIPEMU
  if (threadIdx.x != 0 || blockIdx.x != 0) return;
  const long long t0 = wall_clock64();
  bool waited = false;
  for (;;) {
    if ((igmc_ctrl_ld(ctrl + IGMC_CTRL_GQ) & 1) != (int64_t)(q & 1)) return;
    if (igmc_ctrl_ld(ctrl + IGMC_CTRL_GK) >= (int64_t)gk_min) break;
    if (wall_clock64() - t0 > timeout_ticks) {
      atomicAdd((unsigned long long*)(ctrl + IGMC_CTRL_GATE_TIMEOUTS), 1ull);
      return;
    }
    waited = true;
    __builtin_amdgcn_s_sleep(16);
// ... 69 lines not shown
  if (sp.dl) igmc_launch_g2_compose(m, P, stream);
  if (sp.dlf) {
    igmc_launch_dl_fwd(m, b, sp, P, B, training, use_flags, training ? m.dpre[3] : nullptr, stream);
  } else if (sp.dl) {
    igmc_launch_dl_layer0(m, b, B, training, use_flags, stream);
  } else {
    const size_t l0s = (size_t)(m.R * m.L * 32 + m.L * 32 + 32) * sizeof(float) + (size_t)4 * m.R * m.L * sizeof(int);
    igmc_dispatch([&](auto uf, auto tr) {
      IGMC_PLAUNCH("k_l0_fwd", (k_l0_fwd<uf(), tr()>), igmc_l0_grid(m, B), IGMC_BLOCK, l0s, stream, b, m, P, m.h[0]);
    }, use_flags != 0, training != 0);
  }
  const int gt = igmc_xcd_grid(m, B, 16, 2048);
  const size_t fsm4 = (size_t)(16 * IGMC_TP + 1024 + m.R * 4) * sizeof(float);
  for (int l = 1; l < 4 && !sp.dlf; ++l) {
    float* zo = (training && l == 3) ? m.dpre[3] : nullptr;
    if (sp.dl) igmc_launch_dl_layer(m, b, P, B, l, 0, use_flags, zo, stream);
    else igmc_dispatch([&](auto uf) {
      IGMC_PLAUNCH("k_rgcn_layer_fwd", (k_rgcn_layer4<uf(), false>), gt, IGMC_BLOCK, fsm4, stream, b, m, P, l, zo);
    }, use_flags != 0);
  }
  if (training && sp.need_y)
    IGMC_PLAUNCH("k_dense_y_all", k_dense_y_all, dim3(igmc_rows_grid(m.node_cap, 64, 512), 3), IGMC_BLOCK,
                 (size_t)32 * (128 + 4) * sizeof(float), stream, b, m, P);
}

static void launch_layers_bwd(const ModelDev& m, const BatchDev& b, const StepPlan& sp, const float* P, int B, int use_flags,
                              int tables, void* stream) {
  const int gt = igmc_xcd_grid(m, B, 16, 2048);
  const size_t bsm4 = (size_t)(16 * IGMC_TP + 1024 + m.R * 4 + 16 * m.R * 4) * sizeof(float);
  for (int l = 3; l >= 1; --l) {
    if (sp.bwd_dense) igmc_launch_dl_layer(m, b, P, B, l, 1, use_flags, nullptr, stream, tables);
    else igmc_dispatch([&](auto uf) {
      IGMC_PLAUNCH("k_rgcn_layer_bwd", (k_rgcn_layer4<uf(), true>), gt, IGMC_BLOCK, bsm4, stream, b, m, P, l, (float*)nullptr);
    }, use_flags != 0);
  }
}

static void launch_reduce(const ModelDev& m, const BatchDev& b, const StepPlan& sp, const float* P, int B, const int64_t* ctrl,
                          int nstash, void* stream) {
  const int rows0 = m.R * m.L + m.L + 1, l0_mfma = rows0 <= 32;
  const float* d0 = m.dpre[0];
  if (l0_mfma) {
  } else if (rows0 <= 64) IGMC_PLAUNCH("k_l0_bwd", (k_l0_bwd<8>), IGMC_L0_BLOCKS, IGMC_BLOCK, 0, stream, b, m, d0, m.l0_part);
  else IGMC_PLAUNCH("k_l0_bwd", (k_l0_bwd<40>), IGMC_L0_BLOCKS, IGMC_BLOCK, 0, stream, b, m, d0, m.l0_part);
  const int nblk = ((l0_mfma ? 4 : 3) * igmc_wg_stride() + 63) / 64 + (l0_mfma ? 0 : (rows0 * 32 + 63) / 64) + (3 * m.R * 4 + 3) / 4;
  IGMC_PLAUNCH("k_reduce_partials", k_reduce_partials, nblk + nstash, IGMC_BLOCK, 0, stream, m,
               sp.bwd_dense ? sp.dl_grid : igmc_xcd_grid(m, B, 16, 2048), l0_mfma, IGMC_WG_BLOCKS, P, ctrl, nstash);
}

static void launch_tail_ts(const ModelDev& m, const BatchDev& b, const float* P, int B, float grad_scale, float mult, float* grad,
                           int nlin, int nparts, int stride, int nstash, const int64_t* ctrl, int bump_seq, void* stream) {
  IGMC_PLAUNCH("k_tail_ts", k_tail_ts, nlin + (4 * m.ts_stride + 63) / 64 + nstash, IGMC_BLOCK, 0, stream, b, m, P, grad_scale,
               mult, 2.f, grad, nlin, nparts, stride, B, nstash, ctrl, bump_seq);
}

static int launch_exchange(const ModelDev& m, int tail, const StepExchange* xch, float* grad, void* stream) {
  if (!xch || tail == IGMC_TAIL_HANDOFF) return 0;
  const int rows0 = m.R * m.L + m.L + 1;
  const int64_t n = tail == IGMC_TAIL_TS ? (int64_t)4 * m.ts_stride + (int64_t)4 * m.ts_stride / 32 * 4
                                         : (int64_t)3 * igmc_wg_stride() + 3 * m.R * 4 + rows0 * 32;
  return xch->sum(xch->user, tail == IGMC_TAIL_TS ? m.ts_raw : m.graw, n, grad + m.off_l1w, m.n_params - m.off_l1w, stream);
}

static void launch_finalize(const ModelDev& m, const BatchDev& b, const float* P, float* grad, float arr_coef, int tail,
                            int ts_mode, const AdamTail& at, int img, float ARR, float* loss, int* img_emitted, void* stream) {
  const int bs = tail == IGMC_TAIL_BS;
  if (tail == IGMC_TAIL_HANDOFF) {
    if (at.enabled) IGMC_PLAUNCH("k_finalize_adam", k_finalize, 4 * IGMC_FIN_NB + 32, IGMC_BLOCK, 0, stream, m, P, grad, arr_coef, at, ts_mode);
    else IGMC_PLAUNCH("k_finalize", k_finalize, 4 * IGMC_FIN_NB, IGMC_BLOCK, 0, stream, m, P, grad, arr_coef, at, ts_mode);
  } else if (at.enabled) {
    IGMC_PLAUNCH("k_finalize_adam", k_finalize_ts, 4 * IGMC_FTS_NB + 32 + 1, IGMC_BLOCK, 0, stream, m, P, grad, arr_coef, at, 32, bs, img);
    if (img_emitted) *img_emitted = img;
  } else {
    IGMC_PLAUNCH("k_finalize", k_finalize_ts, 4 * IGMC_FTS_NB, IGMC_BLOCK, 0, stream, m, P, grad, arr_coef, at, 0, bs, 0);
  }
  if (!at.enabled && loss) igmc_launch_loss(m, b, ARR, loss, stream);
}


void igmc_launch_forward(const ModelDev& m, const BatchDev& b, const StepPlan& sp, const float* P, int B, int training,
                         int use_flags, const uint8_t* inj_mask, uint64_t seed, uint64_t step, float mult,
                         float* out, void* stream) {
  if (sp.family == IGMC_FAM_G2) {
    igmc_launch_graph_step2(m, b, sp, P, B, 0, use_flags, nullptr, seed, step, mult, 0.f, out, stream);
    return;
  }
  launch_conv_fwd(m, b, sp, P, B, training, use_flags, stream);
  const int hgrid = (B + IGMC_HG - 1) / IGMC_HG;
  const size_t fs = (size_t)IGMC_HG * m.D * sizeof(float);
  if (m.D % 16 == 0)
    IGMC_PLAUNCH("k_head_fwd", k_head_fwd_mfma, (B + 15) / 16, 512, 0, stream, b, m, P, training, inj_mask, seed, step,
                 mult, out);
  else if (fs <= 48 * 1024)
    IGMC_PLAUNCH("k_head_fwd", (k_head_fwd<true>), hgrid, 512, fs, stream, b, m, P, training, inj_mask, seed, step,
                 mult, out);
  else
    IGMC_PLAUNCH("k_head_fwd", (k_head_fwd<false>), hgrid, 512, 0, stream, b, m, P, training, inj_mask, seed, step,
                 mult, out);
}

void igmc_launch_conv_forward(const ModelDev& m, const BatchDev& b, const StepPlan& sp, const float* P, int B, int training,
                              int use_flags, void* stream) {
  launch_conv_fwd(m, b, sp, P, B, training, use_flags, stream);
}

void igmc_launch_backward(const ModelDev& m, const BatchDev& b, const StepPlan& sp, const float* P, int B, int use_flags,
// ... 18 lines not shown
void igmc_launch_conv_backward(const ModelDev& m, const BatchDev& b, const StepPlan& sp, const float* P, int B, int use_flags,
                               float arr_coef, float* grad, void* stream) {
  AdamTail none;
  memset(&none, 0, sizeof(none));
  if (sp.dlb) {
    const int gstride = (B + 7) & ~7;
    igmc_launch_dl_bwd(m, b, sp, B, use_flags, stream, nullptr, 1);
    launch_tail_ts(m, b, P, B, 0.f, 1.f, grad, 0, (sp.nqu + sp.nqv) * gstride, gstride, 4, nullptr, 1, stream);
  } else {
    const int l0_mfma = m.R * m.L + m.L + 1 <= 32;
    launch_layers_bwd(m, b, sp, P, B, use_flags, 0, stream);
    IGMC_PLAUNCH("k_wgrad", k_wgrad, dim3(IGMC_WG_BLOCKS, l0_mfma ? 4 : 3), IGMC_BLOCK, 0, stream, b, m, 0);
    launch_reduce(m, b, sp, nullptr, B, nullptr, 0, stream);
  }
  launch_finalize(m, b, P, grad, arr_coef, sp.tail, 0, none, 0, 0.f, nullptr, nullptr, stream);
}

int igmc_launch_loss_grad(const ModelDev& m_in, const BatchDev& b, const StepPlan& sp, float* P, int B, int use_flags,
                          const uint8_t* inj_mask, uint64_t seed, uint64_t step, float mult, float ARR,
                          float grad_scale, float arr_scale, float* out, float* grad, float* loss, const AdamTail* adam,
                          void* stream, const StepExchange* xch, int* img_emitted) {
  ModelDev m = m_in;
  m.adam_m1 = adam ? adam->m1 : nullptr;
  m.adam_m2 = adam ? adam->m2 : nullptr;
  if (img_emitted) *img_emitted = 0;
  const int rows0 = m.R * m.L + m.L + 1;
  const int img = adam && m.g2_w && m.R <= G2_NR * G2_NG_MAX && rows0 <= (g2_t0_rows(m.R, m.L) == 32 ? 32 : 48);
  const int ny = (m.D / 16 + 3) / 4;
  const float* Pc = P;
  AdamTail at;
  memset(&at, 0, sizeof(at));
  if (adam) {
    at = *adam;
    at.enabled = sp.fast_head;
    at.b = b;
    at.ARR = ARR;
  }
  at.use_flags = use_flags;
  at.skip = xch ? xch->failed : nullptr;
  const int64_t* ctrl = adam ? at.ctrl : nullptr;
  if (!sp.fast_head) {
    igmc_launch_forward(m, b, sp, Pc, B, 1, use_flags, inj_mask, seed, step, mult, out, stream);
    igmc_launch_backward(m, b, sp, Pc, B, use_flags, nullptr, 1, grad_scale, mult, 2.f, ARR * arr_scale, grad, stream);
    if (adam) {
      igmc_launch_finish(m, b, at.p, grad, at.m1, at.m2, at.step_size, at.inv_sqrt_bc2, at.beta1, at.beta2, at.eps, at.wd,
                         at.ctrl, ARR, at.loss, at.total, use_flags, stream);
    } else if (loss) {
      igmc_launch_loss(m, b, ARR, loss, stream);
    }
    return 0;
  }
  const int tables = sp.tail == IGMC_TAIL_TS;
  if (sp.family == IGMC_FAM_G2) {
    const int bump_seq = igmc_launch_graph_step2(m, b, sp, Pc, B, 1, use_flags, inj_mask, seed, step, mult, grad_scale, out, stream);
    launch_tail_ts(m, b, Pc, B, grad_scale, mult, grad, 8 * ny, sp.grid, (sp.cs > 1) ? ((B + 7) & ~7) : IGMC_TS_BLOCKS,
                   tables ? 4 : 0, ctrl, bump_seq, stream);
  } else {
    launch_conv_fwd(m, b, sp, Pc, B, 1, use_flags, stream);
    if (sp.dlts) {
      const DlHead hd = {Pc, inj_mask, seed, step, mult, grad_scale, out};
      const int inside = sp.dlb && sp.head_inside;
      if (!inside) igmc_launch_head_sub(m, b, Pc, B, inj_mask, seed, step, mult, grad_scale, out, stream);
      if (sp.dlb) igmc_launch_dl_bwd(m, b, sp, B, use_flags, stream, inside ? &hd : nullptr);
      else launch_layers_bwd(m, b, sp, Pc, B, use_flags, 1, stream);
      const int gstride = (B + 7) & ~7;
      launch_tail_ts(m, b, Pc, B, grad_scale, mult, grad, 8 * ny, (sp.nqu + sp.nqv) * gstride, gstride, 4, ctrl, sp.dlf ? 1 : 0, stream);
    } else {
      const int gy = igmc_rows_grid(m.node_cap, 128, 512), hb = (B + 15) / 16, nsl = rows0 <= 32 ? 4 : 3;
      IGMC_PLAUNCH("k_head_train", k_head_train, dim3(hb > gy ? hb : gy, 4), 512, (size_t)32 * (128 + 4) * sizeof(float), stream,
                   b, m, Pc, inj_mask, seed, step, mult, grad_scale, out);
      launch_layers_bwd(m, b, sp, Pc, B, use_flags, 0, stream);
      IGMC_PLAUNCH("k_wgrad_head", k_wgrad_head, dim3(IGMC_WG_BLOCKS, nsl + 1), IGMC_BLOCK, 0, stream, b, m, Pc,
                   (const float*)nullptr, 1, grad_scale, mult, 2.f, grad, nsl);
      launch_reduce(m, b, sp, Pc, B, ctrl, sp.tail == IGMC_TAIL_BS ? 4 : 0, stream);
    }
  }
  if (const int rc = launch_exchange(m, sp.tail, xch, grad, stream)) return rc;
  launch_finalize(m, b, Pc, grad, ARR * arr_scale, sp.tail, sp.family == IGMC_FAM_G2, at, img, ARR, loss, img_emitted, stream);
  return 0;
}

int igmc_launch_train_step(const ModelDev& m, const BatchDev& b, const StepPlan& sp, float* P, int B, int use_flags,
                           const uint8_t* inj_mask, uint64_t seed, uint64_t step, float mult, float ARR, float* out,
                           float* grad, float* m1, float* m2, float step_size, float inv_sqrt_bc2, float beta1,
                           float beta2, float eps, float wd, int64_t* ctrl, int* done, float* loss, double* total,
                           void* stream, float grad_scale, const StepExchange* xch, int* img_emitted) {
  AdamTail at;
  memset(&at, 0, sizeof(at));
  at.p = P; at.m1 = m1; at.m2 = m2;
  at.step_size = step_size; at.inv_sqrt_bc2 = inv_sqrt_bc2; at.beta1 = beta1; at.beta2 = beta2; at.eps = eps; at.wd = wd;
  at.ctrl = ctrl; at.done = done; at.loss = loss; at.total = total;
  return igmc_launch_loss_grad(m, b, sp, P, B, use_flags, inj_mask, seed, step, mult, ARR,
                               grad_scale != 0.f ? grad_scale : 1.0f / (float)B, 1.0f, out, grad, nullptr, &at, stream, xch,
                               img_emitted);
}

void igmc_launch_loss(const ModelDev& m, const BatchDev& b, float ARR, float* loss, void* stream) {
  IGMC_PLAUNCH("k_loss", k_loss, 1, IGMC_BLOCK, 0, stream, b, m, ARR, loss);
}

void igmc_launch_sse(const BatchDev& b, const float* out, double* acc, int64_t* ctrl, void* stream) {
  IGMC_PLAUNCH("k_sse_acc", k_sse_acc, 1, IGMC_BLOCK, 0, stream, b, out, acc, ctrl);
}

void igmc_launch_tick(int64_t* ctrl, void* stream) { IGMC_PLAUNCH("k_tick", k_tick, 1, 64, 0, stream, ctrl); }
void igmc_launch_regroup(int64_t* ctrl, int M, int64_t first_cur, int64_t first_next, void* stream) {
  IGMC_PLAUNCH("k_regroup", k_regroup, 1, 64, 0, stream, ctrl, M, first_cur, first_next);
// ... 49 lines not shown
```

### igmc_amd/csrc/step_plan.h

```cpp
#include <limits.h>

#define IGMC_HOOK_UNSET INT_MIN
struct StepHooks {
  int graph_step;
  int gs_cluster;
  int gs_grid;
  int dl;
  int dl_fused;
  int dl_ts;
  int dl_gsplit;
  int dl_head;
  int fin_mode;
};
static int step_hook(const char* name, int unset) {
  const char* e = getenv(name);
  return e ? atoi(e) : unset;
}
static StepHooks step_hooks() {
  StepHooks hk;
  hk.graph_step = step_hook("IGMC_GRAPH_STEP", 1);
  hk.gs_cluster = step_hook("IGMC_GS_CLUSTER", IGMC_HOOK_UNSET);
  hk.gs_grid = step_hook("IGMC_GS_GRID", 0);
  hk.dl = step_hook("IGMC_DL", 1);
  hk.dl_fused = step_hook("IGMC_DL_FUSED", IGMC_HOOK_UNSET);
  hk.dl_ts = step_hook("IGMC_DL_TS", 1);
  hk.dl_gsplit = step_hook("IGMC_DL_GSPLIT", 1);
  hk.dl_head = step_hook("IGMC_DL_HEAD", 1);
  hk.fin_mode = step_hook("IGMC_FIN_MODE", 1);
  return hk;
}
int igmc_dl_always() { return step_hook("IGMC_DL_ALWAYS", 0) == 1; }

static int gs_cluster(const StepHooks& hk, int B) {
#ifdef IGMC_HIPEMU
  int want = 1;
#else
  static int cus = -1;
  if (cus < 0) {
    hipDeviceProp_t prop;
    int dev = 0;
    cus = (hipGetDevice(&dev) == hipSuccess && hipGetDeviceProperties(&prop, dev) == hipSuccess) ? prop.multiProcessorCount : 0;
  }
  int want = (cus >= 240) ? 4 : 1;
#endif
  if (hk.gs_cluster != IGMC_HOOK_UNSET) want = hk.gs_cluster;
  const int stride = (B + 7) & ~7;
  if (want >= 4 && 4 * stride <= 224) return 4;
  if (want >= 2 && 2 * stride <= 224) return 2;
  return 1;
}
static int gs_grid(const StepHooks& hk, int B) {
  int cap = IGMC_WG_BLOCKS;
  if (hk.gs_grid > 0 && hk.gs_grid < cap) cap = hk.gs_grid;
  return B < cap ? B : cap;
}
static int g2_eligible(const StepHooks& hk, const ModelDev& m, const BatchDev& b, int B, G2Layout* lay, int* cs_out) {
  if (hk.graph_step == 0 || !igmc_g2_xcd_ok()) return 0;
  const int cs = gs_cluster(hk, B);
  if (!igmc_g2_layout(m, b, cs, lay)) return 0;
  *cs_out = cs;
  return 1;
}

static int dl_kp(const BatchDev& b) {
  const int cmax = b.cap_u > b.cap_v ? b.cap_u : b.cap_v;
  return 32 * ((cmax + 31) >> 5) + 8;
}
static int dl_base_ok(const StepHooks& hk, const ModelDev& m, const BatchDev& b, int B, int wide) {
  if (hk.dl == 0) return 0;
  if (!b.relm || !b.relmT || !m.g2_w || m.L > 8) return 0;
  const int rows0 = m.R * m.L + m.L + 1;
  if (wide ? (g2_groups(m.R, m.L) == 1 || m.R > G2_NR * G2_NG_MAX || rows0 > 48) : (m.R > G2_NR || rows0 > 32)) return 0;
  const int cmax = b.cap_u > b.cap_v ? b.cap_u : b.cap_v;
  const DlSplit sq = dl_split(b.cap_u, b.cap_v, B);
  return cmax <= 256 && B * (sq.nqu + sq.nqv) <= IGMC_GATHER_BLOCKS;
}
static int dl_eligible(const StepHooks& hk, const ModelDev& m, const BatchDev& b, int B) {
  return dl_base_ok(hk, m, b, B, 0) && dl_lds(dl_kp(b)) <= (size_t)160 * 1024;
}
static int dl_ts_eligible(const StepHooks& hk, const ModelDev& m, const BatchDev& b, int B) {
  if (hk.dl_ts == 0 || !dl_eligible(hk, m, b, B) || !m.ts_part || !m.cnt0) return 0;
// ... 2 lines not shown
  if ((sq.nqu + sq.nqv) * stride > IGMC_TS_BLOCKS || m.R * m.L > 20) return 0;
  return dl_lds(dl_kp(b), true) <= (size_t)160 * 1024;
}
static int dl_fwd_eligible(const StepHooks& hk, const ModelDev& m, const BatchDev& b, int B) {
  if (!igmc_g2_xcd_ok() || hk.dl_fused == 0) return 0;
  if (!dl_eligible(hk, m, b, B) || !m.g2_ex || m.ex_nodes < DLX_K || b.graph_cap > m.g2_graphs) return 0;
  const DlSplit sq = dl_split(b.cap_u, b.cap_v, B);
  if (B * (sq.nqu + sq.nqv) > 224) return 0;
  return (size_t)dlf_words(dl_kp(b)) * 4 <= (size_t)160 * 1024;
}
static int dl_bwd_eligible(const StepHooks& hk, const ModelDev& m, const BatchDev& b, int B) {
  if (!dl_fwd_eligible(hk, m, b, B) || !dl_ts_eligible(hk, m, b, B) || hk.dl_fused == 1) return 0;
  return (size_t)dlb_words(dl_kp(b)) * 4 <= (size_t)160 * 1024;
}
static int dl_wide(const StepHooks& hk, const ModelDev& m, const BatchDev& b, int B, int tables_tail) {
  if (!igmc_g2_xcd_ok() || !dl_base_ok(hk, m, b, B, 1)) return 0;
  if ((hk.dl_fused != IGMC_HOOK_UNSET && hk.dl_fused != 2) || hk.dl_ts == 0 || !tables_tail) return 0;
  if (!m.g2_ex || m.ex_nodes < DLX_K || b.graph_cap > m.g2_graphs || !m.ts_part || !m.cnt0) return 0;
  const DlSplit sq = dl_split(b.cap_u, b.cap_v, B);
  const int stride = (B + 7) & ~7, kp = dl_kp(b);
  if (B * (sq.nqu + sq.nqv) > 224 || (sq.nqu + sq.nqv) * stride > IGMC_TS_BLOCKS) return 0;
  const int ng = g2_groups(m.R, m.L);
  return (size_t)dlf_words(kp, ng) * 4 <= (size_t)160 * 1024 && (size_t)dlb_words(kp, ng) * 4 <= (size_t)160 * 1024;
}
static int dl_gsplit(const StepHooks& hk, const ModelDev& m, const BatchDev& b, int B) {
  if (g2_groups(m.R, m.L) != 2 || g2_rel_groups(m.R) != 2 || hk.dl_gsplit == 0) return 0;
  const DlSplit sq = dl_split(b.cap_u, b.cap_v, B);
  const int nbu = (b.cap_u + 15) >> 4, nbv = (b.cap_v + 15) >> 4;
  if ((nbu + sq.nqu - 1) / sq.nqu > DL_GB || (nbv + sq.nqv - 1) / sq.nqv > DL_GB) return 0;
  const int kp = dl_kp(b);
  return (size_t)dlf_words_gs(kp) * 4 <= 160 * 1024 && (size_t)dlb_words_gs(kp) * 4 <= 160 * 1024;
}

void igmc_step_plan(const ModelDev& m, const BatchDev& b, int B, int kind, StepPlan* p) {
  memset(p, 0, sizeof(*p));
  const StepHooks hk = step_hooks();
  const int ny = (m.D / 16 + 3) / 4;
  const int l0_mfma = m.R * m.L + m.L + 1 <= 32;
  const int fin = hk.fin_mode && m.fin_stash;
  const int tables_tail = fin && m.datt_part;
  const int fts = tables_tail && m.R <= 8;
  p->kind = kind;
  p->fast_head = (m.D % 16 == 0) && 8 * ny <= IGMC_WG_BLOCKS;
  const int fused = kind == IGMC_CALL_STEP && p->fast_head;
  const int g2 = l0_mfma && g2_eligible(hk, m, b, B, &p->lay, &p->cs);
  const int narrow = dl_eligible(hk, m, b, B), wide = dl_wide(hk, m, b, B, tables_tail);
  p->dense_layers = narrow || wide;
  p->needs_csr = !(narrow || (kind != IGMC_CALL_CONV && (g2 || wide)));
  if (g2 && (fused || kind == IGMC_CALL_EVAL)) {
    p->family = IGMC_FAM_G2;
    p->grid = (p->cs > 1) ? p->cs * ((B + 7) & ~7) : gs_grid(hk, B);
    p->tail = fts ? IGMC_TAIL_TS : IGMC_TAIL_HANDOFF;
    p->exchange_inside = fused && fts;
    p->step_form = 1;
    return;
  }
  const int dlf1 = narrow && dl_fwd_eligible(hk, m, b, B), dlb1 = dlf1 && dl_bwd_eligible(hk, m, b, B);
  p->wide = wide;
  p->dl = wide || narrow;
  p->dlf = wide || dlf1;
  if (fused) {
    p->dlts = wide || (narrow && l0_mfma && fts && dl_ts_eligible(hk, m, b, B));
    p->dlb = p->dlts && (wide || dlb1);
    p->self_seq = !p->dlts;
    p->head_inside = hk.dl_head != 0;
    p->bwd_dense = p->dl;
    p->exchange_inside = fin && m.R <= IGMC_FBS_MAX_R;
    p->tail = p->dlts ? IGMC_TAIL_TS : p->exchange_inside ? IGMC_TAIL_BS : IGMC_TAIL_HANDOFF;
  } else {
    p->dlts = p->dlb = fts && l0_mfma && m.dcat[0] && dlb1;
    p->self_seq = 1;
    p->bwd_dense = narrow;
    p->need_y = kind != IGMC_CALL_EVAL && !p->dlts;
    p->tail = p->dlts ? IGMC_TAIL_TS : IGMC_TAIL_HANDOFF;
  }
  p->gsplit = p->dlf && dl_gsplit(hk, m, b, B);
  p->family = p->dlf ? IGMC_FAM_DLF : p->dl ? IGMC_FAM_DL : IGMC_FAM_ROWS;
  if (p->dl) {
    const DlSplit sq = dl_split(b.cap_u, b.cap_v, B);
    p->nqu = sq.nqu;
    p->nqv = sq.nqv;
    p->dl_grid = B * (sq.nqu + sq.nqv);
  }
  p->step_form = (wide && p->gsplit) ? 3 : p->dlf ? 2 : 0;
}
```

### igmc_amd/stepgraph.py

```python
import ctypes as C
import os
import struct
import sys

import numpy as np
import torch

from . import _lib, parallel

MAX_GROUP = 50
SPARSE_CANDIDATES = 128.0
GROUP_EXTRACT_CHUNK = 2


def _ctrl_words(step, epoch, adam_t, batch, group, lr, beta1, beta2, eps, wd):
    w = np.zeros(_lib.CTRL['WORDS'], dtype=np.int64)
    w[_lib.CTRL['STEP']], w[_lib.CTRL['EPOCH']], w[_lib.CTRL['K']] = step, epoch, 0
    w[_lib.CTRL['FIRST']], w[_lib.CTRL['FIRST_ODD']] = 0, group * batch
    w[_lib.CTRL['GROUP']], w[_lib.CTRL['GK']], w[_lib.CTRL['GQ']] = group, 0, 0
    w[_lib.CTRL['ADAM_T']], w[_lib.CTRL['BATCH']] = adam_t, batch
    step_size = float(lr) / (1.0 - float(beta1) ** adam_t)
    inv_sqrt_bc2 = 1.0 / (1.0 - float(beta2) ** adam_t) ** 0.5
    for key, val in (('LR', lr), ('BETA1', beta1), ('BETA2', beta2), ('EPS', eps), ('WD', wd),
                     ('STEP_SIZE', step_size), ('INV_SQRT_BC2', inv_sqrt_bc2)):
# ... 577 lines not shown
        launches = min(max(1, int(os.environ.get('IGMC_PRIME_LAUNCHES', '3'))), (room - 1) // 2)
        graphs = graphs if graphs is not None else [self.graph] * 3
        for g in graphs[:launches]:
            g.replay()
            torch.cuda.synchronize()
        if launches > 0 and self.pacing_fallback is None and self._paced_default() and \
                os.environ.get('IGMC_EXTRACT_PACED') is None:
            gave_up = int(self.ctrl[_lib.CTRL['GATE_TIMEOUTS']].item())
            if self.comm is not None and self.world > 1:
                gave_up = parallel.all_reduce_max_int(gave_up, self.dev.index)
            if gave_up >= 4:
                sys.stderr.write('igmc_amd: %d pacing gates timed out while the step graph was primed (streams not served '
                                 'concurrently?); pacing by graph edges\n' % gave_up)
                self.pacing_fallback = '1'
                self.drop_graphs()
        for t, k in zip((m.flat_parameters(), self.opt.exp_avg, self.opt.exp_avg_sq, self.ctrl, self.total, self.loss), keep):
            t.copy_(k)
        self._regroup()

    def run_epoch(self, perm, epoch):
        self.begin_epoch(perm, epoch)
        n = self.n_links
        self.steps(n // self.B)
        if n % self.B:
            self.step(n % self.B)
        self.detach()
        self.check()
        return self.total, n

    def check(self):
        self.lib.call('igmc_model_check', self.ws.handle, C.c_void_p(torch.cuda.current_stream().cuda_stream))
        if self.comm is not None and hasattr(self.comm, 'check'):
            self.comm.check(torch.cuda.current_stream().cuda_stream)
        words = self.ctrl.cpu()
        err = int(words[_lib.CTRL['SYNC_ERR']])
        gave_up = int(words[_lib.CTRL['GATE_TIMEOUTS']])
        if self.comm is not None and self.world > 1 and self.pacing_fallback is None and self._paced_default():
            gave_up_all = parallel.all_reduce_max_int(gave_up, self.dev.index)
        else:
            gave_up_all = gave_up
        if gave_up_all >= 4 and self.pacing_fallback is None:
            sys.stderr.write('igmc_amd: %d pacing gates of the extraction chain timed out (streams not served concurrently?); '
                             'pacing by graph edges from here on\n' % gave_up_all)
            self.pacing_fallback = '1'
            self.drop_graphs()
        if gave_up:
            self.ctrl[_lib.CTRL['GATE_TIMEOUTS']] = 0
        if err:
            what = []
            if err & 2:
                what.append('a step trained on an arena whose stamp is not the batch of its cursor')
            if err & 4:
                what.append('a step trained on edge-dropout draws keyed by another batch')
            raise RuntimeError('device-side step control: %s (sync_err=%d); results of the affected steps are invalid'
                               % ('; '.join(what) or 'error', err))


class EvalGraph(StepGraph):
    SLOT = 'evalgraph'
    TRAINING = False

    def __init__(self, model, dataset, batch_size, use_graph=None, overlap=None, group=None):
        StepGraph.__init__(self, model, None, dataset, batch_size, 0.0, use_graph=use_graph, overlap=overlap, group=group)
        if self.sp is not None:
            raise NotImplementedError('the sort-pool family evaluates through its own forward (train_eval.eval_loss)')
        self.acc = torch.zeros(2, dtype=torch.float64, device=self.dev)

    def _enqueue_step(self, arena, B):
        m, st = self.model, torch.cuda.current_stream().cuda_stream
        self.ws.forward(m.flat_parameters().data_ptr(), arena, self.out.data_ptr(), training=False,
                        multiply_by=float(m.multiply_by), stream=st)
        self.ws.sse_accumulate(self.out.data_ptr(), arena, self.acc.data_ptr(), stream=st, ctrl=self.ctrl.data_ptr())

    def _count(self, n):
        pass

    def run(self, perm, epoch):
        self.acc.zero_()
        self.begin_epoch(perm, epoch)
        n = self.n_links
        self.steps(n // self.B)
        if n % self.B:
            self.step(n % self.B)
        self.detach()
        self.check()
        return self.acc


class ScoreGraph(EvalGraph):
    SLOT = 'scoregraph'

    def __init__(self, model, dataset, batch_size, use_graph=None, overlap=None, group=None):
        EvalGraph.__init__(self, model, dataset, batch_size, use_graph=use_graph, overlap=overlap, group=group)
        n = max(len(dataset), 1)
        self.scores = torch.zeros(n, dtype=torch.float32, device=self.dev)
        self.labels = torch.zeros(n, dtype=torch.float32, device=self.dev)
        self.err = torch.zeros(1, dtype=torch.int32, device=self.dev)
        self.params_ptr = model.flat_parameters().data_ptr()

    def _enqueue_step(self, arena, B):
        m, st = self.model, torch.cuda.current_stream().cuda_stream
        self.ws.forward(self.params_ptr, arena, self.out.data_ptr(), training=False,
                        multiply_by=float(m.multiply_by), stream=st)
        self.ws.scores_store(self.out.data_ptr(), arena, self.acc.data_ptr(), self.scores.data_ptr(),
                             self.labels.data_ptr(), self.scores.numel(), self.err.data_ptr(), first=-1, stream=st,
                             ctrl=self.ctrl.data_ptr())
# ... 25 lines not shown
```

Before: 803,800 subgraphs/s.

## Fold stash computation into graph step and fuse tail into one launch

Moves the per-layer fin_stash work (basis Gram, attention moments, Adam scalars) into extra workgroups of k_graph_step2. It also replaces the two-launch tail (reduction plus finalize) with a single k_tail_fin kernel. Inside that kernel, workgroups hand off attention-gradient partials through tagged words in global memory that other workgroups poll. This removes a kernel launch and a serialized dependency per training step, at the cost of spin-waiting, a timeout error path, and slightly less dynamic LDS for the step kernel.

After: 824,500 subgraphs/s, median of 6. +2.6%, better.

```diff
diff --git a/igmc_amd/csrc/capi.hip b/igmc_amd/csrc/capi.hip
--- a/igmc_amd/csrc/capi.hip
+++ b/igmc_amd/csrc/capi.hip
@@ -702,11 +702,13 @@
   d.ts_stride = (d.R * 32 + 33) * 32;
   d.fin_stash = nullptr;
   d.datt_part = nullptr;
+  d.fold_w = nullptr;
   if (d.R <= G2_NR * G2_NG_MAX)
   {
     fail |= M.get(&d.ts_part, (size_t)4 * IGMC_TS_BLOCKS * d.ts_stride) |
             M.get(&d.ts_raw, (size_t)4 * d.ts_stride + (size_t)4 * d.ts_stride / 32 * 4);
     if (!fail) d.datt_part = d.ts_raw + (size_t)4 * d.ts_stride;
+    fail |= M.get(&d.fold_w, (size_t)4 * 32 * IGMC_FOLD_NA);
   }
   if (d.R <= 128) fail |= M.get(&d.fin_stash, (size_t)4 * IGMC_STASH_LAYER + 16);
   d.g2_ex = nullptr;
@@ -771,6 +773,7 @@
     const unsigned long long ts0[4] = {~0ull, 0ull, 0ull, 0ull};
     HIPCHECK(hipMemcpy(m->d.gs_ts, ts0, sizeof(ts0), hipMemcpyHostToDevice));
   }
+  if (m->d.fold_w) HIPCHECK(hipMemset(m->d.fold_w, 0, (size_t)4 * 32 * IGMC_FOLD_NA * sizeof(unsigned long long)));
   if (m->d.g2_ex) {
     HIPCHECK(hipMemset(m->d.g2_ex, 0, 5 * m->d.g2_ex_stride * sizeof(unsigned long long)));
     HIPCHECK(hipMemset(m->d.g2_fx, 0, (size_t)max_graphs * 256 * sizeof(unsigned long long)));
@@ -800,6 +803,19 @@
   if (n < 0 || n > (int64_t)m->d.graph_cap * (which < 2 ? 128 : m->d.D)) IGMC_FAIL("size out of range");
   HIPCHECK(hipDeviceSynchronize());
   HIPCHECK(hipMemcpy(h_out, src, (size_t)n * sizeof(float), hipMemcpyDeviceToHost));
+  return 0;
+}
+
+extern "C" int igmc_debug_weight_images(const igmc_model* m, float* h_out, int64_t* n_words) {
+  if (!m || !n_words) IGMC_FAIL("null argument");
+  const int64_t n = m->d.g2_w ? (int64_t)g2_w_words(m->d.R, m->d.L) : 0;
+  if (h_out) {
+    if (*n_words < 0 || *n_words > n) IGMC_FAIL("size out of range");
+    HIPCHECK(hipDeviceSynchronize());
+    if (*n_words) HIPCHECK(hipMemcpy(h_out, m->d.g2_w, (size_t)*n_words * sizeof(float), hipMemcpyDeviceToHost));
+  } else {
+    *n_words = n;
+  }
   return 0;
 }
 
@@ -1121,6 +1137,7 @@
 extern "C" int igmc_model_reset_exchange(igmc_model* m, void* stream) {
   if (!m) IGMC_FAIL("null model");
   hipStream_t st = (hipStream_t)stream;
+  if (m->d.fold_w) HIPCHECK(hipMemsetAsync(m->d.fold_w, 0, (size_t)4 * 32 * IGMC_FOLD_NA * sizeof(unsigned long long), st));
   if (m->d.g2_ex) {
     HIPCHECK(hipMemsetAsync(m->d.g2_ex, 0, 5 * m->d.g2_ex_stride * sizeof(unsigned long long), st));
     HIPCHECK(hipMemsetAsync(m->d.g2_fx, 0, (size_t)m->d.g2_graphs * 256 * sizeof(unsigned long long), st));
@@ -1138,8 +1155,9 @@
       HIPCHECK(hipMemset(m->d.gs_bar, 0, (2 * (size_t)m->d.graph_cap + 1) * sizeof(int)));
       (void)igmc_model_reset_exchange(m, stream);
       HIPCHECK(hipStreamSynchronize((hipStream_t)stream));
-      IGMC_FAIL("a workgroup-cluster exchange of k_graph_step2 timed out (GPU shared with another job?): results of the "
-                "affected steps are invalid; set IGMC_GS_CLUSTER=1 or IGMC_GRAPH_STEP=0");
+      IGMC_FAIL("a workgroup-cluster exchange of k_graph_step2 or a hand-off of the one-launch tail k_tail_fin timed out (GPU "
+                "shared with another job?): results of the affected steps are invalid; set IGMC_GS_CLUSTER=1 or "
+                "IGMC_GRAPH_STEP=0 (the tail alone: IGMC_TAIL_FOLD=0)");
     }
   }
   return 0;
diff --git a/igmc_amd/csrc/fin_stash.h b/igmc_amd/csrc/fin_stash.h
--- /dev/null
+++ b/igmc_amd/csrc/fin_stash.h
@@ -0,0 +1,117 @@
+#pragma once
+#include "model.h"
+struct FinStashModel {
+  int R, L;
+  int64_t off_basis[4], off_att[4];
+  float* fin_stash;
+  const float* adam_m1;
+  const float* adam_m2;
+  float* arr_part;
+};
+
+#define IGMC_STASH_G 0
+#define IGMC_STASH_M 16
+#define IGMC_STASH_ATTM1 32
+#define IGMC_STASH_ATTM2 96
+#define IGMC_STASH_ATT 160
+#define IGMC_STASH_SCAL (4 * IGMC_STASH_LAYER)
+#define IGMC_STASH_SEQ 8
+template <typename M>
+__device__ __forceinline__ void fin_stash_body(const M& m, const float* __restrict__ P, int l, const int64_t* ctrl) {
+  __shared__ float sg10[4][10];
+  __shared__ float sG[16];
+  __shared__ float s_att[128];
+  const int tid = threadIdx.x, lane = tid & 63, wave = tid >> 6;
+  const int nE = ((l == 0) ? m.L : 32) * 32, R = m.R, na = R * 4;
+  const float* basis = P + m.off_basis[l];
+  const float* attg = P + m.off_att[l];
+  float* st = m.fin_stash + l * IGMC_STASH_LAYER;
+  const bool small = na <= 128;
+  const float attv = (small && tid < na) ? attg[tid] : 0.f;
+  float bq[4][4];
+#pragma unroll
+  for (int it = 0; it < 4; ++it) {
+    const int e = tid + it * IGMC_BLOCK, ec = e < nE ? e : nE - 1;
+#pragma unroll
+    for (int q = 0; q < 4; ++q) bq[it][q] = (e < nE) ? basis[q * nE + ec] : 0.f;
+  }
+  float m1v = 0.f, m2v = 0.f;
+  const bool mom = m.adam_m1 && na <= 64 && tid >= 128 && tid < 128 + na;
+  if (mom) {
+    m1v = m.adam_m1[m.off_att[l] + tid - 128];
+    m2v = m.adam_m2[m.off_att[l] + tid - 128];
+  }
+  double scal = 0.0;
+  const bool sc = l == 0 && ctrl && tid >= 192 && tid < 198;
+  if (sc) {
+    const double* d = (const double*)ctrl;
+    const int k = tid - 192;
+    const int src = (k == 0) ? IGMC_CTRL_STEP_SIZE : (k == 1) ? IGMC_CTRL_INV_SQRT_BC2 : (k == 2) ? IGMC_CTRL_BETA1
+                  : (k == 3) ? IGMC_CTRL_BETA2 : (k == 4) ? IGMC_CTRL_EPS : IGMC_CTRL_WD;
+    scal = d[src];
+  }
+  if (small && tid < na) s_att[tid] = attv;
+  float gp[10];
+#pragma unroll
+  for (int q = 0; q < 10; ++q) gp[q] = 0.f;
+#pragma unroll
+  for (int it = 0; it < 4; ++it) {
+    if (tid + it * IGMC_BLOCK < nE) {
+      const float b0 = bq[it][0], b1 = bq[it][1], b2 = bq[it][2], b3 = bq[it][3];
+      gp[0] += b0 * b0; gp[1] += b0 * b1; gp[2] += b0 * b2; gp[3] += b0 * b3;
+      gp[4] += b1 * b1; gp[5] += b1 * b2; gp[6] += b1 * b3;
+      gp[7] += b2 * b2; gp[8] += b2 * b3; gp[9] += b3 * b3;
+    }
+  }
+  for (int e = tid + 4 * IGMC_BLOCK; e < nE; e += IGMC_BLOCK) {
+    const float b0 = basis[e], b1 = basis[nE + e], b2 = basis[2 * nE + e], b3 = basis[3 * nE + e];
+    gp[0] += b0 * b0; gp[1] += b0 * b1; gp[2] += b0 * b2; gp[3] += b0 * b3;
+    gp[4] += b1 * b1; gp[5] += b1 * b2; gp[6] += b1 * b3;
+    gp[7] += b2 * b2; gp[8] += b2 * b3; gp[9] += b3 * b3;
+  }
+#pragma unroll
+  for (int q = 0; q < 10; ++q) gp[q] = igmc_wave_sum_f(gp[q]);
+  if (lane == 0) {
+#pragma unroll
+    for (int q = 0; q < 10; ++q) sg10[wave][q] = gp[q];
+  }
+  __syncthreads();
+  const float* att = small ? (const float*)s_att : attg;
+  if (tid >= 64 && tid < 80) {
+    const int bb = (tid - 64) >> 2, bp = tid & 3;
+    float sacc = 0.f;
+    for (int r = 0; r < R; ++r) {
+      const float dm = (r > 0) ? att[r * 4 + bp] - att[(r - 1) * 4 + bp] : 0.f;
+      const float dn = (r + 1 < R) ? att[(r + 1) * 4 + bp] - att[r * 4 + bp] : 0.f;
+      sacc += att[r * 4 + bb] * 2.f * (dm - dn);
+    }
+    st[IGMC_STASH_M + tid - 64] = sacc;
+  }
+  if (tid >= 128 && na <= IGMC_STASH_LAYER - IGMC_STASH_ATT) {
+    for (int i = tid - 128; i < na; i += IGMC_BLOCK - 128) {
+      st[IGMC_STASH_ATT + i] = att[i];
+      if (m.adam_m1 && na <= 64) {
+        st[IGMC_STASH_ATTM1 + i] = mom && i == tid - 128 ? m1v : m.adam_m1[m.off_att[l] + i];
+        st[IGMC_STASH_ATTM2 + i] = mom && i == tid - 128 ? m2v : m.adam_m2[m.off_att[l] + i];
+      }
+    }
+  }
+  if (sc) m.fin_stash[IGMC_STASH_SCAL + tid - 192] = (float)scal;
+  if (tid == 0) {
+    const int ij[10][2] = {{0, 0}, {0, 1}, {0, 2}, {0, 3}, {1, 1}, {1, 2}, {1, 3}, {2, 2}, {2, 3}, {3, 3}};
+    for (int q = 0; q < 10; ++q) {
+      const float v = (sg10[0][q] + sg10[1][q]) + (sg10[2][q] + sg10[3][q]);
+      sG[ij[q][0] * 4 + ij[q][1]] = v;
+      sG[ij[q][1] * 4 + ij[q][0]] = v;
+    }
+    float reg = 0.f;
+    for (int r = 0; r + 1 < R; ++r) {
+      float d[4];
+      for (int q = 0; q < 4; ++q) d[q] = att[(r + 1) * 4 + q] - att[r * 4 + q];
+      for (int p1 = 0; p1 < 4; ++p1)
+        for (int p2 = 0; p2 < 4; ++p2) reg += d[p1] * sG[p1 * 4 + p2] * d[p2];
+    }
+    m.arr_part[l] = reg;
+    for (int q = 0; q < 16; ++q) st[IGMC_STASH_G + q] = sG[q];
+  }
+}
diff --git a/igmc_amd/csrc/g2_compose.h b/igmc_amd/csrc/g2_compose.h
--- a/igmc_amd/csrc/g2_compose.h
+++ b/igmc_amd/csrc/g2_compose.h
@@ -108,7 +108,7 @@
   lay->att = o; o += 64;
   lay->head = o; o += 256 + 256 + 3 * 128 + 512 + 16;
   lay->words = o;
-  return (size_t)o * 4 <= 160 * 1024;
+  return (size_t)o * 4 + 768 <= 160 * 1024;
 }
 
 __global__ void k_g2_xcc_probe(int* out) {
@@ -148,7 +148,7 @@
 
 int igmc_launch_graph_step2(const ModelDev& m, const BatchDev& b, const StepPlan& sp, const float* P, int B, int training,
                             int use_flags, const uint8_t* inj_mask, uint64_t seed, uint64_t step, float mult, float grad_scale,
-                            float* out, void* stream) {
+                            float* out, void* stream, int nstash, const int64_t* stash_ctrl) {
   const G2Layout& lay = sp.lay;
   const int cs = sp.cs;
   G2Args a;
@@ -177,7 +177,17 @@
   a.self_seq = (!training || a.ts) ? 1 : 0;
   a.cs = cs;
   a.stride = (cs > 1) ? ((B + 7) & ~7) : 1;
-  const int grid = sp.grid;
+  if (training && nstash) {
+    a.nstash = nstash;
+    a.stash_ctrl = stash_ctrl;
+    a.fs.R = m.R; a.fs.L = m.L;
+    for (int l = 0; l < 4; ++l) {
+      a.fs.off_basis[l] = m.off_basis[l];
+      a.fs.off_att[l] = m.off_att[l];
+    }
+    a.fs.fin_stash = m.fin_stash; a.fs.adam_m1 = m.adam_m1; a.fs.adam_m2 = m.adam_m2; a.fs.arr_part = m.arr_part;
+  }
+  const int grid = sp.grid + a.nstash;
   const size_t sm = (size_t)lay.words * 4;
   if (!m.img_current) {
     IGMC_PLAUNCH("k_g2_compose", k_g2_compose, 2 * 3 * g2_groups(m.R, m.L) * (G2_NR + 1) + g2_t0_rows(m.R, m.L) / 32, G2C_THREADS, 0, stream, m, P, m.g2_w);
@@ -208,8 +218,11 @@
                         (const void*)k_graph_step2<true, false, true>,  (const void*)k_graph_step2<false, false, true>,
                         (const void*)k_graph_step2<true, true, false>,  (const void*)k_graph_step2<false, true, false>,
                         (const void*)k_graph_step2<true, false, false>, (const void*)k_graph_step2<false, false, false>};
-  for (const void* fn : fns)
-    if (hipFuncSetAttribute(fn, hipFuncAttributeMaxDynamicSharedMemorySize, mx) != hipSuccess) return 1;
+  for (const void* fn : fns) {
+    hipFuncAttributes fa;
+    if (hipFuncGetAttributes(&fa, fn) != hipSuccess || (int)fa.sharedSizeBytes > 768) return 1;
+    if (hipFuncSetAttribute(fn, hipFuncAttributeMaxDynamicSharedMemorySize, mx - (int)fa.sharedSizeBytes) != hipSuccess) return 1;
+  }
 #endif
   return 0;
 }
diff --git a/igmc_amd/csrc/g2_prims.h b/igmc_amd/csrc/g2_prims.h
--- a/igmc_amd/csrc/g2_prims.h
+++ b/igmc_amd/csrc/g2_prims.h
@@ -99,16 +99,7 @@
 #endif
 }
 
-__device__ __forceinline__ void g2_pub_f32(unsigned long long* p, float v, uint32_t tag) {
-#ifndef IGMC_HIPEMU
-  __hip_atomic_store(p, ((unsigned long long)tag << 32) | (unsigned long long)__float_as_uint(v), __ATOMIC_RELAXED,
-                     __HIP_MEMORY_SCOPE_WAVEFRONT);
-#else
-  uint32_t bits;
-  memcpy(&bits, &v, 4);
-  *p = ((unsigned long long)tag << 32) | (unsigned long long)bits;
-#endif
-}
+#include "g2_words.h"
 
 #define G2_PX_BYTES 32768
 #define G2_PX_FLAGS 28672
@@ -162,26 +153,6 @@
   for (int c = wave; c < pieces; c += nwaves) g2_glds16<16>((const float4*)px + c * 64, (float4*)pl + c * 64, lane);
 }
 
-__device__ __forceinline__ float g2_poll_f32(const unsigned long long* p, uint32_t tag, int* err) {
-  for (long it = 0;; ++it) {
-#ifndef IGMC_HIPEMU
-    const unsigned long long w = __hip_atomic_load(p, __ATOMIC_RELAXED, __HIP_MEMORY_SCOPE_AGENT);
-#else
-    const unsigned long long w = *p;
-#endif
-    if ((uint32_t)(w >> 32) == tag) return __uint_as_float((uint32_t)w);
-    if (it > (1L << 22)) {
-      *err = 1;
-      return 0.f;
-    }
-#ifndef IGMC_HIPEMU
-    __builtin_amdgcn_s_sleep(2);
-#else
-    hipemu::yield();
-#endif
-  }
-}
-
 #ifdef IGMC_HIPEMU
 #define G2_SCHED_BARRIER() do { } while (0)
 #else
diff --git a/igmc_amd/csrc/g2_subgraph.h b/igmc_amd/csrc/g2_subgraph.h
--- a/igmc_amd/csrc/g2_subgraph.h
+++ b/igmc_amd/csrc/g2_subgraph.h
@@ -34,6 +34,9 @@
   unsigned long long* ts;
   int timing, cs, stride, self_seq;
   G2Layout lay2;
+  int nstash;
+  const int64_t* stash_ctrl;
+  FinStashModel fs;
 };
 
 template <bool FLAGS, bool TRAIN, bool ONCE>
@@ -79,6 +82,22 @@
     g_g2_wg[blockIdx.x][0] = g2_wall_clock();
     g_g2_wg[blockIdx.x][2] = g2_xcc_id();
   }
+  auto arrive = [&]() {
+    if (tid == 0 && a.self_seq) {
+      const unsigned long long t1 = a.ts ? g2_wall_clock() : 0ull;
+      if (g2_last_workgroup_advances(a.gs_bar) && a.ts) g2_clock_close(a.ts, t1);
+    }
+  };
+  const int nwork = (int)gridDim.x - (TRAIN ? a.nstash : 0);
+  if (TRAIN && (int)blockIdx.x >= nwork) {
+    if (tid < IGMC_BLOCK) {
+      const int l = (int)blockIdx.x - nwork;
+      fin_stash_body(a.fs, P, l, a.stash_ctrl);
+      if (l == 0 && tid == 0) a.fs.fin_stash[IGMC_STASH_SCAL + IGMC_STASH_SEQ] = __uint_as_float(seq);
+    }
+    arrive();
+    return;
+  }
 
   const int g_first = (cs > 1) ? (int)(blockIdx.x / (8 * cs)) * 8 + (int)(blockIdx.x & 7) : (int)blockIdx.x;
   const int g_pre = (g_first < a.graph_cap) ? g_first : a.graph_cap - 1;
@@ -611,7 +630,7 @@
       __syncthreads();
       G2_STAMP(34);
     }
-  } while (!ONCE && (g += (int)gridDim.x) < B);
+  } while (!ONCE && (g += nwork) < B);
 
   if (TRAIN && wave < 4) {
     float* part0 = a.ts_part + (size_t)tslot * ts;
@@ -622,10 +641,7 @@
       if (c < RL + L + 1) part0[c * 32 + wn * 16 + li] = acc0[rr];
     }
   }
-  if (tid == 0 && a.self_seq) {
-    const unsigned long long t1 = a.ts ? g2_wall_clock() : 0ull;
-    if (g2_last_workgroup_advances(a.gs_bar) && a.ts) g2_clock_close(a.ts, t1);
-  }
+  arrive();
   G2_STAMP(35);
   if (a.timing && tid == 0 && blockIdx.x < 1024) g_g2_wg[blockIdx.x][1] = g2_wall_clock();
 }
diff --git a/igmc_amd/csrc/g2_words.h b/igmc_amd/csrc/g2_words.h
--- /dev/null
+++ b/igmc_amd/csrc/g2_words.h
@@ -0,0 +1,49 @@
+#pragma once
+#include "common.h"
+
+__device__ __forceinline__ void g2_pub_f32(unsigned long long* p, float v, uint32_t tag) {
+#ifndef IGMC_HIPEMU
+  __hip_atomic_store(p, ((unsigned long long)tag << 32) | (unsigned long long)__float_as_uint(v), __ATOMIC_RELAXED,
+                     __HIP_MEMORY_SCOPE_WAVEFRONT);
+#else
+  uint32_t bits;
+  memcpy(&bits, &v, 4);
+  *p = ((unsigned long long)tag << 32) | (unsigned long long)bits;
+#endif
+}
+
+__device__ __forceinline__ void g2_pub_f32_agent(unsigned long long* p, float v, uint32_t tag) {
+#ifndef IGMC_HIPEMU
+  __hip_atomic_store(p, ((unsigned long long)tag << 32) | (unsigned long long)__float_as_uint(v), __ATOMIC_RELAXED,
+                     __HIP_MEMORY_SCOPE_AGENT);
+#else
+  g2_pub_f32(p, v, tag);
+#endif
+}
+__device__ __forceinline__ unsigned long long g2_ld_word(const unsigned long long* p) {
+#ifndef IGMC_HIPEMU
+  return __hip_atomic_load(p, __ATOMIC_RELAXED, __HIP_MEMORY_SCOPE_AGENT);
+#else
+  return *p;
+#endif
+}
+
+__device__ __forceinline__ float g2_poll_f32(const unsigned long long* p, uint32_t tag, int* err) {
+  for (long it = 0;; ++it) {
+#ifndef IGMC_HIPEMU
+    const unsigned long long w = __hip_atomic_load(p, __ATOMIC_RELAXED, __HIP_MEMORY_SCOPE_AGENT);
+#else
+    const unsigned long long w = *p;
+#endif
+    if ((uint32_t)(w >> 32) == tag) return __uint_as_float((uint32_t)w);
+    if (it > (1L << 22)) {
+      *err = 1;
+      return 0.f;
+    }
+#ifndef IGMC_HIPEMU
+    __builtin_amdgcn_s_sleep(2);
+#else
+    hipemu::yield();
+#endif
+  }
+}
diff --git a/igmc_amd/csrc/graphstep2.hip b/igmc_amd/csrc/graphstep2.hip
--- a/igmc_amd/csrc/graphstep2.hip
+++ b/igmc_amd/csrc/graphstep2.hip
@@ -1,6 +1,7 @@
 #include "launch.h"
 #include "g2_image.h"
 #include "head_sub.h"
+#include "fin_stash.h"
 #include <stdlib.h>
 #include <stdio.h>
 #include <string.h>
diff --git a/igmc_amd/csrc/launch.h b/igmc_amd/csrc/launch.h
--- a/igmc_amd/csrc/launch.h
+++ b/igmc_amd/csrc/launch.h
@@ -127,6 +127,7 @@
   int need_y;
   int tail;
   int exchange_inside;
+  int tail_fold;
   int needs_csr;
   int dense_layers;
   int step_form;
@@ -152,7 +153,7 @@
                           float* zero_out, void* stream, int tables = 0);
 int igmc_launch_graph_step2(const ModelDev& m, const BatchDev& b, const StepPlan& sp, const float* P, int B, int training,
                             int use_flags, const uint8_t* inj_mask, uint64_t seed, uint64_t step, float mult, float grad_scale,
-                            float* out, void* stream);
+                            float* out, void* stream, int nstash = 0, const int64_t* stash_ctrl = nullptr);
 
 void igmc_prof_begin(const char* name, void* stream);
 void igmc_prof_end(void* stream);
diff --git a/igmc_amd/csrc/model.h b/igmc_amd/csrc/model.h
--- a/igmc_amd/csrc/model.h
+++ b/igmc_amd/csrc/model.h
@@ -6,6 +6,7 @@
 #define IGMC_WG_BLOCKS 64
 #endif
 #define IGMC_STASH_LAYER 672
+#define IGMC_FOLD_NA 32
 #define IGMC_TS_BLOCKS 256
 #define IGMC_GATHER_BLOCKS 4096
 #define IGMC_FBS_MAX_R 32
@@ -38,6 +39,7 @@
   int ts_stride;
   float* fin_stash;
   float* datt_part;
+  unsigned long long* fold_w;
   int* gs_bar;
   int* gs_err;
   unsigned long long* gs_ts;
diff --git a/igmc_amd/csrc/model.hip b/igmc_amd/csrc/model.hip
--- a/igmc_amd/csrc/model.hip
+++ b/igmc_amd/csrc/model.hip
@@ -1,5 +1,7 @@
 #include "model.h"
 #include "g2_image.h"
+#include "fin_stash.h"
+#include "g2_words.h"
 #include <stdlib.h>
 
 struct XcdSeg {
@@ -1144,7 +1146,6 @@
   }
 }
 
-__device__ __forceinline__ void fin_stash_body(const ModelDev& m, const float* __restrict__ P, int l, const int64_t* ctrl);
 
 __global__ __launch_bounds__(IGMC_BLOCK) void k_reduce_partials(ModelDev m, int n_gatt_parts, int l0_mfma,
                                                                   int n_wg_parts, const float* __restrict__ P,
@@ -1230,6 +1231,22 @@
   }
 }
 
+struct TsSlots {
+  int ng, nq, stride;
+};
+__device__ __forceinline__ TsSlots ts_slots(int nparts, int stride, int B) {
+  TsSlots s;
+  s.ng = (nparts < stride) ? nparts : ((B < stride) ? B : stride);
+  s.nq = ((nparts + stride - 1) / stride) * s.ng;
+  s.stride = stride;
+  return s;
+}
+__device__ __forceinline__ int ts_slot(const TsSlots& s, int q) {
+  const int qc = q < s.nq ? q : s.nq - 1;
+  const int c = qc / s.ng, g = qc - c * s.ng;
+  return c * s.stride + g;
+}
+
 __device__ __forceinline__ void reduce_ts_body(const ModelDev& m, int nparts, int stride, int B, int blk,
                                                const float* __restrict__ Pold = nullptr) {
   __shared__ float4 sred4[16][16];
@@ -1254,16 +1271,12 @@
   float4 s4 = make_float4(0.f, 0.f, 0.f, 0.f);
   if (ok4) {
     const float* p = m.ts_part + (size_t)l * IGMC_TS_BLOCKS * ts + i0;
-    const int ng = (nparts < stride) ? nparts : ((B < stride) ? B : stride), cs = (nparts + stride - 1) / stride;
-    const int nq = cs * ng;
+    const TsSlots sl = ts_slots(nparts, stride, B);
+    const int nq = sl.nq;
     for (int q0 = pg; q0 < nq; q0 += 16 * 14) {
       float4 v[14];
 #pragma unroll
-      for (int u = 0; u < 14; ++u) {
-        const int q = q0 + 16 * u, qc = q < nq ? q : nq - 1;
-        const int c = qc / ng, g = qc - c * ng;
-        v[u] = *(const float4*)(p + (size_t)(c * stride + g) * ts);
-      }
+      for (int u = 0; u < 14; ++u) v[u] = *(const float4*)(p + (size_t)ts_slot(sl, q0 + 16 * u) * ts);
 #pragma unroll
       for (int u = 0; u < 14; ++u)
         if (q0 + 16 * u < nq) {
@@ -1296,111 +1309,6 @@
   }
 }
 
-#define IGMC_STASH_G 0
-#define IGMC_STASH_M 16
-#define IGMC_STASH_ATTM1 32
-#define IGMC_STASH_ATTM2 96
-#define IGMC_STASH_ATT 160
-#define IGMC_STASH_SCAL (4 * IGMC_STASH_LAYER)
-__device__ __forceinline__ void fin_stash_body(const ModelDev& m, const float* __restrict__ P, int l,
-                                               const int64_t* ctrl) {
-  __shared__ float sg10[4][10];
-  __shared__ float sG[16];
-  __shared__ float s_att[128];
-  const int tid = threadIdx.x, lane = tid & 63, wave = tid >> 6;
-  const int nE = ((l == 0) ? m.L : 32) * 32, R = m.R, na = R * 4;
-  const float* basis = P + m.off_basis[l];
-  const float* attg = P + m.off_att[l];
-  float* st = m.fin_stash + l * IGMC_STASH_LAYER;
-  const bool small = na <= 128;
-  const float attv = (small && tid < na) ? attg[tid] : 0.f;
-  float bq[4][4];
-#pragma unroll
-  for (int it = 0; it < 4; ++it) {
-    const int e = tid + it * IGMC_BLOCK, ec = e < nE ? e : nE - 1;
-#pragma unroll
-    for (int q = 0; q < 4; ++q) bq[it][q] = (e < nE) ? basis[q * nE + ec] : 0.f;
-  }
-  float m1v = 0.f, m2v = 0.f;
-  const bool mom = m.adam_m1 && na <= 64 && tid >= 128 && tid < 128 + na;
-  if (mom) {
-    m1v = m.adam_m1[m.off_att[l] + tid - 128];
-    m2v = m.adam_m2[m.off_att[l] + tid - 128];
-  }
-  double scal = 0.0;
-  const bool sc = l == 0 && ctrl && tid >= 192 && tid < 198;
-  if (sc) {
-    const double* d = (const double*)ctrl;
-    const int k = tid - 192;
-    const int src = (k == 0) ? IGMC_CTRL_STEP_SIZE : (k == 1) ? IGMC_CTRL_INV_SQRT_BC2 : (k == 2) ? IGMC_CTRL_BETA1
-                  : (k == 3) ? IGMC_CTRL_BETA2 : (k == 4) ? IGMC_CTRL_EPS : IGMC_CTRL_WD;
-    scal = d[src];
-  }
-  if (small && tid < na) s_att[tid] = attv;
-  float gp[10];
-#pragma unroll
-  for (int q = 0; q < 10; ++q) gp[q] = 0.f;
-#pragma unroll
-  for (int it = 0; it < 4; ++it) {
-    if (tid + it * IGMC_BLOCK < nE) {
-      const float b0 = bq[it][0], b1 = bq[it][1], b2 = bq[it][2], b3 = bq[it][3];
-      gp[0] += b0 * b0; gp[1] += b0 * b1; gp[2] += b0 * b2; gp[3] += b0 * b3;
-      gp[4] += b1 * b1; gp[5] += b1 * b2; gp[6] += b1 * b3;
-      gp[7] += b2 * b2; gp[8] += b2 * b3; gp[9] += b3 * b3;
-    }
-  }
-  for (int e = tid + 4 * IGMC_BLOCK; e < nE; e += IGMC_BLOCK) {
-    const float b0 = basis[e], b1 = basis[nE + e], b2 = basis[2 * nE + e], b3 = basis[3 * nE + e];
-    gp[0] += b0 * b0; gp[1] += b0 * b1; gp[2] += b0 * b2; gp[3] += b0 * b3;
-    gp[4] += b1 * b1; gp[5] += b1 * b2; gp[6] += b1 * b3;
-    gp[7] += b2 * b2; gp[8] += b2 * b3; gp[9] += b3 * b3;
-  }
-#pragma unroll
-  for (int q = 0; q < 10; ++q) gp[q] = igmc_wave_sum_f(gp[q]);
-  if (lane == 0) {
-#pragma unroll
-    for (int q = 0; q < 10; ++q) sg10[wave][q] = gp[q];
-  }
-  __syncthreads();
-  const float* att = small ? (const float*)s_att : attg;
-  if (tid >= 64 && tid < 80) {
-    const int bb = (tid - 64) >> 2, bp = tid & 3;
-    float sacc = 0.f;
-    for (int r = 0; r < R; ++r) {
-      const float dm = (r > 0) ? att[r * 4 + bp] - att[(r - 1) * 4 + bp] : 0.f;
-      const float dn = (r + 1 < R) ? att[(r + 1) * 4 + bp] - att[r * 4 + bp] : 0.f;
-      sacc += att[r * 4 + bb] * 2.f * (dm - dn);
-    }
-    st[IGMC_STASH_M + tid - 64] = sacc;
-  }
-  if (tid >= 128 && na <= IGMC_STASH_LAYER - IGMC_STASH_ATT) {
-    for (int i = tid - 128; i < na; i += IGMC_BLOCK - 128) {
-      st[IGMC_STASH_ATT + i] = att[i];
-      if (m.adam_m1 && na <= 64) {
-        st[IGMC_STASH_ATTM1 + i] = mom && i == tid - 128 ? m1v : m.adam_m1[m.off_att[l] + i];
-        st[IGMC_STASH_ATTM2 + i] = mom && i == tid - 128 ? m2v : m.adam_m2[m.off_att[l] + i];
-      }
-    }
-  }
-  if (sc) m.fin_stash[IGMC_STASH_SCAL + tid - 192] = (float)scal;
-  if (tid == 0) {
-    const int ij[10][2] = {{0, 0}, {0, 1}, {0, 2}, {0, 3}, {1, 1}, {1, 2}, {1, 3}, {2, 2}, {2, 3}, {3, 3}};
-    for (int q = 0; q < 10; ++q) {
-      const float v = (sg10[0][q] + sg10[1][q]) + (sg10[2][q] + sg10[3][q]);
-      sG[ij[q][0] * 4 + ij[q][1]] = v;
-      sG[ij[q][1] * 4 + ij[q][0]] = v;
-    }
-    float reg = 0.f;
-    for (int r = 0; r + 1 < R; ++r) {
-      float d[4];
-      for (int q = 0; q < 4; ++q) d[q] = att[(r + 1) * 4 + q] - att[r * 4 + q];
-      for (int p1 = 0; p1 < 4; ++p1)
-        for (int p2 = 0; p2 < 4; ++p2) reg += d[p1] * sG[p1 * 4 + p2] * d[p2];
-    }
-    m.arr_part[l] = reg;
-    for (int q = 0; q < 16; ++q) st[IGMC_STASH_G + q] = sG[q];
-  }
-}
 
 __global__ __launch_bounds__(IGMC_BLOCK) void k_tail_ts(BatchDev b, ModelDev m, const float* __restrict__ P,
                                                           float grad_scale, float mult, float drop_scale,
@@ -1435,7 +1343,7 @@
   int bad = 0;
   if (got >= 0 && got != want) bad |= 2;
   if (use_flags && got >= 0 && b.stamp[1] >= 0 && (uint64_t)b.stamp[1] != igmc_ctrl_drop_key(ctrl, (int)want)) bad |= 4;
-  if (bad) ctrl[IGMC_CTRL_SYNC_ERR] |= bad;
+  if (bad) atomicOr((unsigned long long*)(ctrl + IGMC_CTRL_SYNC_ERR), (unsigned long long)bad);
   ctrl_advance(ctrl);
 }
 
@@ -1467,6 +1375,30 @@
   p[i] = pi - step_size * a / (sqrtf(v) * inv_sqrt_bc2 + eps);
 }
 
+__device__ __forceinline__ void adam_store(float* p, float* m1, float* m2, int64_t i, float gi, float pv, float av, float vv,
+                                           float step_size, float inv_sqrt_bc2, float beta1, float beta2, float eps, float wd) {
+  if (wd != 0.f) gi += wd * pv;
+  const float a = beta1 * av + (1.f - beta1) * gi;
+  const float v = beta2 * vv + (1.f - beta2) * gi * gi;
+  m1[i] = a;
+  m2[i] = v;
+  p[i] = pv - step_size * a / (sqrtf(v) * inv_sqrt_bc2 + eps);
+}
+
+__device__ __forceinline__ void adam_store_sep(float* p, float* m1, float* m2, int64_t i, float gi, float pv, float av, float vv,
+                                               float step_size, float inv_sqrt_bc2, float beta1, float beta2, float eps, float wd) {
+  if (wd != 0.f) gi += wd * pv;
+  float a, v;
+  {
+#pragma clang fp contract(off)
+    a = beta1 * av + (1.f - beta1) * gi;
+    v = beta2 * vv + (1.f - beta2) * gi * gi;
+  }
+  m1[i] = a;
+  m2[i] = v;
+  p[i] = pv - step_size * a / (sqrtf(v) * inv_sqrt_bc2 + eps);
+}
+
 template <int NB>
 __device__ __forceinline__ void adam_range(float* p, const float* g, float* m1, float* m2, int64_t lo, int64_t hi,
                                            float step_size, float inv_sqrt_bc2, float beta1, float beta2, float eps,
@@ -1485,15 +1417,7 @@
 #pragma unroll
     for (int k = 0; k < NB; ++k) {
       const int64_t i = i0 + (int64_t)k * IGMC_BLOCK;
-      if (i < hi) {
-        float gi = gv[k];
-        if (wd != 0.f) gi += wd * pv[k];
-        const float a = beta1 * av[k] + (1.f - beta1) * gi;
-        const float v = beta2 * vv[k] + (1.f - beta2) * gi * gi;
-        m1[i] = a;
-        m2[i] = v;
-        p[i] = pv[k] - step_size * a / (sqrtf(v) * inv_sqrt_bc2 + eps);
-      }
+      if (i < hi) adam_store_sep(p, m1, m2, i, gv[k], pv[k], av[k], vv[k], step_size, inv_sqrt_bc2, beta1, beta2, eps, wd);
     }
   }
 }
@@ -1699,6 +1623,77 @@
   return pnew;
 }
 
+__device__ __forceinline__ float fts_att_entry(float* __restrict__ grad, const AdamTail& at, const float* st, int R, int rb,
+                                               float g, float arr_coef, int64_t i, float pold, float m1o, float m2o, bool store) {
+  const int r = rb >> 2, bb = rb & 3;
+  if (arr_coef != 0.f) {
+    float sacc = 0.f;
+    for (int bp = 0; bp < 4; ++bp) {
+      const float a0 = st[IGMC_STASH_ATT + r * 4 + bp];
+      const float dm = (r > 0) ? a0 - st[IGMC_STASH_ATT + (r - 1) * 4 + bp] : 0.f;
+      const float dn = (r + 1 < R) ? st[IGMC_STASH_ATT + (r + 1) * 4 + bp] - a0 : 0.f;
+      sacc += 2.f * (dm - dn) * st[IGMC_STASH_G + bp * 4 + bb];
+    }
+    g += arr_coef * sacc;
+  }
+  return fts_emit(grad, at, i, g, pold, m1o, m2o, store);
+}
+__device__ __forceinline__ void fts_col_table8(float (&g)[5], const float* st, const float (&tv)[8], int R) {
+#pragma unroll
+  for (int r = 0; r < 8; ++r)
+    if (r < R) {
+#pragma unroll
+      for (int bb = 0; bb < 4; ++bb) g[bb] += st[IGMC_STASH_ATT + r * 4 + bb] * tv[r];
+    }
+}
+__device__ __forceinline__ void fts_col_emit(float* __restrict__ grad, const AdamTail& at, const float* st, float arr_coef,
+                                             const int64_t (&idx)[5], float (&g)[5], const float (&pv)[5], const float (&m1v)[5],
+                                             const float (&m2v)[5], float (&pn)[5]) {
+  if (arr_coef != 0.f) {
+#pragma unroll
+    for (int bb = 0; bb < 4; ++bb) {
+      float t = fmaf(st[IGMC_STASH_M + bb * 4 + 0], pv[0], st[IGMC_STASH_M + bb * 4 + 1] * pv[1]);
+      t = fmaf(st[IGMC_STASH_M + bb * 4 + 2], pv[2], t);
+      t = fmaf(st[IGMC_STASH_M + bb * 4 + 3], pv[3], t);
+      g[bb] = fmaf(arr_coef, t, g[bb]);
+    }
+  }
+#pragma unroll
+  for (int q = 0; q < 5; ++q) pn[q] = fts_emit(grad, at, idx[q], g[q], pv[q], m1v[q], m2v[q]);
+}
+__device__ __forceinline__ void fts_image_col(const ModelDev& m, int ng, int l, int R, int fin, int c, int f, const float* s_attn,
+                                              const float (&pn)[5], int r0, int rstep) {
+  if (l == 0) {
+    float* t0w = m.g2_w + g2_t0_off(ng);
+    for (int r = r0; r <= R; r += rstep)
+      t0w[(r * fin + c) * 32 + f] = (r == R) ? pn[4]
+                                  : g2_wsum(s_attn[r * 4], s_attn[r * 4 + 1], s_attn[r * 4 + 2], s_attn[r * 4 + 3], pn[0], pn[1], pn[2], pn[3]);
+  } else {
+#pragma unroll 3
+    for (int r = r0; r <= R; r += rstep) {
+      const float v = (r == R) ? pn[4]
+                    : g2_wsum(s_attn[r * 4], s_attn[r * 4 + 1], s_attn[r * 4 + 2], s_attn[r * 4 + 3], pn[0], pn[1], pn[2], pn[3]);
+      const int grp = (r == R) ? 0 : r / G2_NR, blk = (r == R) ? G2_NR : r % G2_NR;
+      uint16_t* imf = (uint16_t*)(m.g2_w + g2_img_off(ng, l, 0, grp));
+      uint16_t* imt = (uint16_t*)(m.g2_w + g2_img_off(ng, l, 1, grp));
+      uint32_t h, mi, lo;
+      g2_split2(v, 0.f, h, mi, lo);
+      const uint32_t t3[3] = {h, mi, lo};
+#pragma unroll
+      for (int t = 0; t < G2_NT; ++t) {
+        imf[g2_img_index(t, blk, c, f)] = (uint16_t)t3[t];
+        imt[g2_img_index(t, blk, f, c)] = (uint16_t)t3[t];
+      }
+    }
+  }
+}
+__device__ __forceinline__ void fts_bias(const ModelDev& m, float* __restrict__ grad, const AdamTail& at, int ng, int l, int R,
+                                         int fin, int f, const float (&bq)[4], bool emit) {
+  const int64_t i = m.off_bias[l] + f;
+  const float bnew = fts_emit(grad, at, i, bq[0], bq[1], bq[2], bq[3]);
+  if (emit && l == 0) m.g2_w[g2_t0_off(ng) + (R * fin + fin) * 32 + f] = bnew;
+}
+
 __global__ __launch_bounds__(IGMC_BLOCK) void k_finalize_ts(ModelDev m, const float* P, float* __restrict__ grad,
                                                               float arr_coef, AdamTail at, int nlin, int bs, int img) {
   __builtin_amdgcn_s_setprio(3);
@@ -1851,9 +1846,7 @@
     __syncthreads();
     if (roles) {
       if (bias_role) {
-        const int64_t i = m.off_bias[l] + tid;
-        const float bnew = fts_emit(grad, at, i, bq[0], bq[1], bq[2], bq[3]);
-        if (emit && l == 0) m.g2_w[g2_t0_off(ng) + (R * fin + fin) * 32 + tid] = bnew;
+        fts_bias(m, grad, at, ng, l, R, fin, tid, bq, emit);
       } else if (tid >= 64) {
        for (int rb = tid - 64; rb < na; rb += IGMC_BLOCK - 64) {
         const int r = rb >> 2, bb = rb & 3;
@@ -1878,74 +1871,26 @@
             for (int k = 0; k < 32; ++k) g += v[k];
           }
         }
-        if (arr_coef != 0.f) {
-          float sacc = 0.f;
-          for (int bp = 0; bp < 4; ++bp) {
-            const float a0 = st[IGMC_STASH_ATT + r * 4 + bp];
-            const float dm = (r > 0) ? a0 - st[IGMC_STASH_ATT + (r - 1) * 4 + bp] : 0.f;
-            const float dn = (r + 1 < R) ? st[IGMC_STASH_ATT + (r + 1) * 4 + bp] - a0 : 0.f;
-            sacc += 2.f * (dm - dn) * st[IGMC_STASH_G + bp * 4 + bb];
-          }
-          g += arr_coef * sacc;
-        }
-        const float anew = fts_emit(grad, at, i, g, pold, m1o, m2o, part == 0);
+        const float anew = fts_att_entry(grad, at, st, R, rb, g, arr_coef, i, pold, m1o, m2o, part == 0);
         if (emit) s_attn[rb] = anew;
        }
       }
     }
     if (has) {
       if (table) {
-#pragma unroll
-        for (int r = 0; r < 8; ++r)
-          if (r < R) {
-#pragma unroll
-            for (int bb = 0; bb < 4; ++bb) g[bb] += st[IGMC_STASH_ATT + r * 4 + bb] * tv[r];
-          }
+        fts_col_table8(g, st, tv, R);
         for (int r = 8; r < R; ++r) {
           const float tvr = t0[(size_t)r * nE + e];
 #pragma unroll
           for (int bb = 0; bb < 4; ++bb) g[bb] += st[IGMC_STASH_ATT + r * 4 + bb] * tvr;
         }
       }
-      if (arr_coef != 0.f) {
-#pragma unroll
-        for (int bb = 0; bb < 4; ++bb)
-          g[bb] += arr_coef * (st[IGMC_STASH_M + bb * 4 + 0] * pv[0] + st[IGMC_STASH_M + bb * 4 + 1] * pv[1] +
-                               st[IGMC_STASH_M + bb * 4 + 2] * pv[2] + st[IGMC_STASH_M + bb * 4 + 3] * pv[3]);
-      }
-#pragma unroll
-      for (int q = 0; q < 5; ++q) pn[q] = fts_emit(grad, at, idx[q], g[q], pv[q], m1v[q], m2v[q]);
+      fts_col_emit(grad, at, st, arr_coef, idx, g, pv, m1v, m2v, pn);
       e_img = e;
     }
     if (emit) {
       __syncthreads();
-      if (e_img >= 0) {
-        const int c = e_img >> 5, f = e_img & 31;
-        if (l == 0) {
-          float* t0w = m.g2_w + g2_t0_off(ng);
-          for (int r = 0; r < R; ++r)
-            t0w[(r * fin + c) * 32 + f] = g2_wsum(s_attn[r * 4], s_attn[r * 4 + 1], s_attn[r * 4 + 2], s_attn[r * 4 + 3],
-                                                  pn[0], pn[1], pn[2], pn[3]);
-          t0w[(R * fin + c) * 32 + f] = pn[4];
-        } else {
-#pragma unroll 3
-          for (int r = 0; r <= R; ++r) {
-            const float v = (r == R) ? pn[4]
-                          : g2_wsum(s_attn[r * 4], s_attn[r * 4 + 1], s_attn[r * 4 + 2], s_attn[r * 4 + 3], pn[0], pn[1], pn[2], pn[3]);
-            const int grp = (r == R) ? 0 : r / G2_NR, blk = (r == R) ? G2_NR : r % G2_NR;
-            uint16_t* imf = (uint16_t*)(m.g2_w + g2_img_off(ng, l, 0, grp));
-            uint16_t* imt = (uint16_t*)(m.g2_w + g2_img_off(ng, l, 1, grp));
-            uint32_t h, mi, lo;
-            g2_split2(v, 0.f, h, mi, lo);
-            const uint32_t t3[3] = {h, mi, lo};
-#pragma unroll
-            for (int t = 0; t < G2_NT; ++t) {
-              imf[g2_img_index(t, blk, c, f)] = (uint16_t)t3[t];
-              imt[g2_img_index(t, blk, f, c)] = (uint16_t)t3[t];
-            }
-          }
-        }
-      }
+      if (e_img >= 0) fts_image_col(m, ng, l, R, fin, e_img >> 5, e_img & 31, s_attn, pn, 0, 1);
     }
   } else if ((int)blockIdx.x < 4 * IGMC_FTS_NB + nlin) {
     const int64_t n_lin = m.n_params - m.off_l1w;
@@ -1956,6 +1901,298 @@
   } else {
     loss_body(at.b, m, at.ARR, at.loss, at.total, smf);
     if (tid == 0 && at.ctrl) ctrl_check_and_advance(at.ctrl, at.b, at.use_flags);
+  }
+}
+
+#define IGMC_TF_SETS 3
+#define IGMC_TF_ROWS 384
+#define IGMC_TF_O_ROWS (IGMC_TF_SETS * 1024)
+#define IGMC_TF_O_ST (IGMC_TF_O_ROWS + IGMC_TF_ROWS)
+#define IGMC_TF_O_DATT (IGMC_TF_O_ST + IGMC_STASH_LAYER)
+#define IGMC_TF_O_ATTN (IGMC_TF_O_DATT + 32 * IGMC_FOLD_NA)
+#define IGMC_TF_O_PN (IGMC_TF_O_ATTN + 64)
+#define IGMC_TF_O_SMF (IGMC_TF_O_PN + 5 * 32)
+#define IGMC_TF_WORDS (IGMC_TF_O_SMF + 16)
+#define IGMC_TF_POLL ((32 * IGMC_FOLD_NA + IGMC_BLOCK - 1) / IGMC_BLOCK)
+#define IGMC_TF_TIMEOUT_TICKS 20000000ll
+#define IGMC_SYNC_ERR_FOLD 8
+
+#if defined(IGMC_FIN_CLOCKS) && !defined(IGMC_HIPEMU)
+__device__ unsigned long long g_fin_clk[64];
+extern "C" int igmc_debug_fin_clocks(unsigned long long* out) {
+  return hipMemcpyFromSymbol(out, HIP_SYMBOL(g_fin_clk), sizeof(g_fin_clk)) != hipSuccess;
+}
+#define TF_STAMP(on, k) do { if ((on) && threadIdx.x == 0) g_fin_clk[k] = __builtin_readcyclecounter(); } while (0)
+#else
+#define TF_STAMP(on, k) do { } while (0)
+#endif
+
+__global__ __launch_bounds__(IGMC_BLOCK) void k_tail_fin(BatchDev b, ModelDev m, const float* P, float grad_scale, float mult,
+                                                           float drop_scale, float* grad, float arr_coef, AdamTail at, int nlin,
+                                                           int nparts, int stride, int B, int bump_seq, int mute_layer) {
+  __builtin_amdgcn_s_setprio(3);
+  igmc_kernarg_warm<sizeof(BatchDev) + sizeof(ModelDev) + sizeof(AdamTail) + 64>();
+  IGMC_DYN_SMEM(smem);
+  float* S = (float*)smem;
+  const int tid = threadIdx.x, lane = tid & 63, wave = tid >> 6;
+  const float* stash = m.fin_stash;
+  if (at.ctrl) {
+    at.step_size = stash[IGMC_STASH_SCAL + 0];
+    at.inv_sqrt_bc2 = stash[IGMC_STASH_SCAL + 1];
+    at.beta1 = stash[IGMC_STASH_SCAL + 2];
+    at.beta2 = stash[IGMC_STASH_SCAL + 3];
+    at.eps = stash[IGMC_STASH_SCAL + 4];
+    at.wd = stash[IGMC_STASH_SCAL + 5];
+  }
+  const int R = m.R, L = m.L, na = R * 4;
+  const int nconv = 96 + L;
+  const int blk = blockIdx.x;
+  TF_STAMP(blk == 0, 0);
+  TF_STAMP(blk == nconv, 16);
+  TF_STAMP(blk == nconv + nlin, 32);
+  if (blk < nconv) {
+    const int l = blk < 96 ? 1 + (blk >> 5) : 0, c = blk < 96 ? (blk & 31) : blk - 96;
+    const int fin = (l == 0) ? L : 32, nE = fin * 32, ts = m.ts_stride;
+    const uint32_t tag = __float_as_uint(stash[IGMC_STASH_SCAL + IGMC_STASH_SEQ]) * 2u + 1u;
+    float4* sred4 = (float4*)S;
+    float* rows = S + IGMC_TF_O_ROWS;
+    float* s_st = S + IGMC_TF_O_ST;
+    float* s_datt = S + IGMC_TF_O_DATT;
+    float* s_attn = S + IGMC_TF_O_ATTN;
+    float* s_pn = S + IGMC_TF_O_PN;
+    int* s_flag = (int*)(S + IGMC_TF_O_SMF + 8);
+    const int ng = g2_groups(R, L);
+    const int o4 = lane & 15, pg = wave * 4 + (lane >> 4);
+    float stq[(IGMC_STASH_LAYER + IGMC_BLOCK - 1) / IGMC_BLOCK];
+#pragma unroll
+    for (int u = 0; u < (IGMC_STASH_LAYER + IGMC_BLOCK - 1) / IGMC_BLOCK; ++u) {
+      const int i = tid + u * IGMC_BLOCK;
+      stq[u] = stash[l * IGMC_STASH_LAYER + (i < IGMC_STASH_LAYER ? i : IGMC_STASH_LAYER - 1)];
+    }
+    const int f = tid & 31, e = c * 32 + f;
+    const bool col = tid < 32, bias_role = c == 0 && tid >= 32 && tid < 64;
+    int64_t idx[5];
+    float pv[5], m1v[5], m2v[5], pvb[4] = {0.f, 0.f, 0.f, 0.f}, bq[4] = {0.f, 0.f, 0.f, 0.f};
+#pragma unroll
+    for (int q = 0; q < 5; ++q) {
+      idx[q] = (q < 4) ? m.off_basis[l] + (int64_t)q * nE + e : m.off_root[l] + e;
+      pv[q] = col ? P[idx[q]] : 0.f;
+      m1v[q] = col ? at.m1[idx[q]] : 0.f;
+      m2v[q] = col ? at.m2[idx[q]] : 0.f;
+    }
+    if (wave == 0) {
+#pragma unroll
+      for (int bb = 0; bb < 4; ++bb) pvb[bb] = P[idx[bb]];
+    }
+    if (bias_role) {
+      const int64_t i = m.off_bias[l] + f;
+      bq[1] = P[i];
+      bq[2] = at.m1[i];
+      bq[3] = at.m2[i];
+    }
+    if (tid == 0) *s_flag = 0;
+    TF_STAMP(blk == 0, 1);
+    const float* pl = m.ts_part + (size_t)l * IGMC_TS_BLOCKS * ts;
+    const TsSlots sl = ts_slots(nparts, stride, B);
+    const int nq = sl.nq;
+    bool first_round = true;
+    auto sum_columns = [&](int k0, int k1) {
+      const int nsets = (k1 - k0 + 15) >> 4;
+      int i0[IGMC_TF_SETS];
+      float4 s4[IGMC_TF_SETS];
+#pragma unroll
+      for (int s = 0; s < IGMC_TF_SETS; ++s) {
+        const int k = k0 + 16 * s + o4, kc = k < k1 ? k : k1 - 1, j = kc >> 3;
+        const int row = j < R ? j * fin + c : j == R ? R * fin + c : R * fin + fin;
+        i0[s] = row * 32 + 4 * (kc & 7);
+        s4[s] = make_float4(0.f, 0.f, 0.f, 0.f);
+      }
+      for (int q0 = pg; q0 < nq; q0 += 16 * 14) {
+        float4 v[IGMC_TF_SETS][14];
+        size_t so[14];
+#pragma unroll
+        for (int u = 0; u < 14; ++u) so[u] = (size_t)ts_slot(sl, q0 + 16 * u) * ts;
+#pragma unroll
+        for (int s = 0; s < IGMC_TF_SETS; ++s)
+          if (s < nsets) {
+#pragma unroll
+            for (int u = 0; u < 14; ++u) v[s][u] = *(const float4*)(pl + so[u] + i0[s]);
+          }
+#pragma unroll
+        for (int s = 0; s < IGMC_TF_SETS; ++s)
+          if (s < nsets) {
+#pragma unroll
+            for (int u = 0; u < 14; ++u)
+              if (q0 + 16 * u < nq) {
+                s4[s].x += v[s][u].x; s4[s].y += v[s][u].y; s4[s].z += v[s][u].z; s4[s].w += v[s][u].w;
+              }
+          }
+      }
+      if (!first_round) __syncthreads();
+#pragma unroll
+      for (int s = 0; s < IGMC_TF_SETS; ++s)
+        if (s < nsets) sred4[(s * 16 + pg) * 16 + o4] = s4[s];
+      if (first_round) {
+#pragma unroll
+        for (int u = 0; u < (IGMC_STASH_LAYER + IGMC_BLOCK - 1) / IGMC_BLOCK; ++u) {
+          const int i = tid + u * IGMC_BLOCK;
+          if (i < IGMC_STASH_LAYER) s_st[i] = stq[u];
+        }
+      }
+      first_round = false;
+      __syncthreads();
+      if (wave < nsets) {
+        const float* sr = (const float*)sred4;
+        float tot = 0.f;
+#pragma unroll
+        for (int g16 = 0; g16 < 16; ++g16) tot += sr[((wave * 16 + g16) * 16 + (lane >> 2)) * 4 + (lane & 3)];
+        const int k = k0 + 16 * wave + (lane >> 2);
+        if (k < k1) rows[k * 4 + (lane & 3)] = tot;
+      }
+    };
+    const int ncol_a = 8 * (R + 1);
+    for (int k0 = 0; k0 < ncol_a; k0 += 16 * IGMC_TF_SETS) sum_columns(k0, k0 + 16 * IGMC_TF_SETS < ncol_a ? k0 + 16 * IGMC_TF_SETS : ncol_a);
+    __syncthreads();
+    TF_STAMP(blk == 0, 2);
+    unsigned long long* words = m.fold_w + (size_t)l * 32 * IGMC_FOLD_NA;
+    if (wave == 0) {
+      const int h = lane >> 5;
+      for (int r2 = 0; r2 < R; r2 += 2) {
+        const int r = r2 + h;
+        const float tot = r < R ? rows[r * 32 + f] : 0.f;
+        float pb[4];
+#pragma unroll
+        for (int bb = 0; bb < 4; ++bb) pb[bb] = tot * pvb[bb];
+#pragma unroll
+        for (int bb = 0; bb < 4; ++bb)
+#pragma unroll
+          for (int d = 16; d >= 1; d >>= 1) pb[bb] += __shfl_xor(pb[bb], d, 64);
+#ifdef IGMC_HIPEMU
+        if (l == mute_layer) continue;
+#endif
+        if (f == 0 && r < R) {
+#pragma unroll
+          for (int bb = 0; bb < 4; ++bb) g2_pub_f32_agent(words + c * IGMC_FOLD_NA + r * 4 + bb, pb[bb], tag);
+        }
+      }
+    }
+    TF_STAMP(blk == 0, 3);
+    if (c == 0) sum_columns(ncol_a, ncol_a + 8);
+    TF_STAMP(blk == 0, 4);
+    {
+      const int nw = fin * na;
+      const unsigned long long* wp[IGMC_TF_POLL];
+      int wi[IGMC_TF_POLL];
+#pragma unroll
+      for (int u = 0; u < IGMC_TF_POLL; ++u) {
+        const int w = tid + u * IGMC_BLOCK, wc = w < nw ? w : nw - 1;
+        wi[u] = (wc / na) * IGMC_FOLD_NA + wc % na;
+        wp[u] = words + wi[u];
+      }
+      bool ok = false;
+#ifndef IGMC_HIPEMU
+      const long long t0 = (long long)wall_clock64();
+#endif
+      for (long it = 0;; ++it) {
+        unsigned long long w[IGMC_TF_POLL];
+        bool all = true;
+#pragma unroll
+        for (int u = 0; u < IGMC_TF_POLL; ++u) w[u] = g2_ld_word(wp[u]);
+#pragma unroll
+        for (int u = 0; u < IGMC_TF_POLL; ++u) all = all && (uint32_t)(w[u] >> 32) == tag;
+        if (all) {
+#pragma unroll
+          for (int u = 0; u < IGMC_TF_POLL; ++u) s_datt[wi[u]] = __uint_as_float((uint32_t)w[u]);
+          ok = true;
+          break;
+        }
+#ifndef IGMC_HIPEMU
+        if ((it & 15) == 15 && (long long)wall_clock64() - t0 > IGMC_TF_TIMEOUT_TICKS) break;
+        __builtin_amdgcn_s_sleep(2);
+#else
+        if (it > (1L << 12)) break;
+        hipemu::yield();
+#endif
+      }
+      if (!ok) *s_flag = 1;
+    }
+    __syncthreads();
+    TF_STAMP(blk == 0, 5);
+    if (*s_flag) {
+      if (tid == 0) {
+        *m.gs_err = 1;
+        if (at.ctrl) atomicOr((unsigned long long*)(at.ctrl + IGMC_CTRL_SYNC_ERR), (unsigned long long)IGMC_SYNC_ERR_FOLD);
+      }
+      return;
+    }
+    const float* st = s_st;
+    if (tid >= 64 && tid - 64 < na) {
+      const int rb = tid - 64;
+      float g = 0.f;
+#pragma unroll
+      for (int k = 0; k < 32; ++k) g += (k < fin) ? s_datt[k * IGMC_FOLD_NA + rb] : 0.f;
+      s_attn[rb] = fts_att_entry(grad, at, st, R, rb, g, arr_coef, m.off_att[l] + rb, st[IGMC_STASH_ATT + rb],
+                                 st[IGMC_STASH_ATTM1 + rb], st[IGMC_STASH_ATTM2 + rb], c == 0);
+    }
+    if (bias_role) {
+      bq[0] = rows[(R + 1) * 32 + f];
+      fts_bias(m, grad, at, ng, l, R, fin, f, bq, true);
+    }
+    if (col) {
+      float g[5] = {0.f, 0.f, 0.f, 0.f, 0.f}, tv[8], pn[5];
+#pragma unroll
+      for (int r = 0; r < 8; ++r) tv[r] = (r < R) ? rows[r * 32 + f] : 0.f;
+      g[4] = rows[R * 32 + f];
+      fts_col_table8(g, st, tv, R);
+      fts_col_emit(grad, at, st, arr_coef, idx, g, pv, m1v, m2v, pn);
+#pragma unroll
+      for (int q = 0; q < 5; ++q) s_pn[q * 32 + f] = pn[q];
+    }
+    TF_STAMP(blk == 0, 6);
+    __syncthreads();
+    {
+      float pn[5];
+#pragma unroll
+      for (int q = 0; q < 5; ++q) pn[q] = s_pn[q * 32 + f];
+      fts_image_col(m, ng, l, R, fin, c, f, s_attn, pn, tid >> 5, IGMC_BLOCK / 32);
+    }
+    TF_STAMP(blk == 0, 7);
+  } else if (blk < nconv + nlin) {
+    const int bx = (blk - nconv) & 7, by = (blk - nconv) >> 3, D = m.D;
+    head_bwd_w_body(b, m, P, nullptr, 1, grad_scale, mult, drop_scale, grad, bx, by, B);
+    __syncthreads();
+    TF_STAMP(blk == nconv, 17);
+    int64_t ix[5];
+    bool okx[5];
+    float gv[5], pv[5], av[5], vv[5];
+#pragma unroll
+    for (int k = 0; k < 4; ++k) {
+      const int el = tid + k * IGMC_BLOCK, colx = by * 64 + (el & 63);
+      okx[k] = colx < D;
+      ix[k] = m.off_l1w + (int64_t)(bx * 16 + (el >> 6)) * D + (okx[k] ? colx : 0);
+    }
+    okx[4] = by == 0 && (tid < 32 || (tid == 32 && bx == 0));
+    ix[4] = tid < 16 ? m.off_l1b + bx * 16 + tid : tid < 32 ? m.off_l2w + bx * 16 + tid - 16 : m.off_l2b;
+    const float* gsrc = grad;
+#pragma unroll
+    for (int k = 0; k < 5; ++k) {
+      const int64_t i = okx[k] ? ix[k] : m.off_l1w;
+      gv[k] = gsrc[i];
+      pv[k] = at.p[i];
+      av[k] = at.m1[i];
+      vv[k] = at.m2[i];
+    }
+#pragma unroll
+    for (int k = 0; k < 5; ++k)
+      if (okx[k]) adam_store_sep(at.p, at.m1, at.m2, ix[k], gv[k], pv[k], av[k], vv[k], at.step_size, at.inv_sqrt_bc2, at.beta1,
+                                 at.beta2, at.eps, at.wd);
+    TF_STAMP(blk == nconv, 18);
+  } else {
+    if (bump_seq && tid == 0) m.gs_bar[1] += 1;
+    loss_body(at.b, m, at.ARR, at.loss, at.total, S + IGMC_TF_O_SMF);
+    TF_STAMP(true, 33);
+    if (tid == 0 && at.ctrl) ctrl_check_and_advance(at.ctrl, at.b, at.use_flags);
+    TF_STAMP(true, 34);
   }
 }
 
@@ -2131,6 +2368,19 @@
                            int nlin, int nparts, int stride, int nstash, const int64_t* ctrl, int bump_seq, void* stream) {
   IGMC_PLAUNCH("k_tail_ts", k_tail_ts, nlin + (4 * m.ts_stride + 63) / 64 + nstash, IGMC_BLOCK, 0, stream, b, m, P, grad_scale,
                mult, 2.f, grad, nlin, nparts, stride, B, nstash, ctrl, bump_seq);
+}
+
+static void launch_tail_fin(const ModelDev& m, const BatchDev& b, const float* P, int B, float grad_scale, float mult, float* grad,
+                            float arr_coef, const AdamTail& at, int nlin, int nparts, int stride, int bump_seq, void* stream) {
+  int mute = -1;
+#ifdef IGMC_HIPEMU
+  if (const char* e = getenv("IGMC_EMU_FOLD_MUTE")) mute = atoi(e);
+  hipemu::rt().co_cs = 32;
+  hipemu::rt().co_stride = -1;
+  hipemu::rt().co_block = 0;
+#endif
+  IGMC_PLAUNCH("k_tail_fin", k_tail_fin, 96 + m.L + nlin + 1, IGMC_BLOCK, (size_t)IGMC_TF_WORDS * sizeof(float), stream, b, m, P,
+               grad_scale, mult, 2.f, grad, arr_coef, at, nlin, nparts, stride, B, bump_seq, mute);
 }
 
 static int launch_exchange(const ModelDev& m, int tail, const StepExchange* xch, float* grad, void* stream) {
@@ -2255,7 +2505,15 @@
   }
   const int tables = sp.tail == IGMC_TAIL_TS;
   if (sp.family == IGMC_FAM_G2) {
-    const int bump_seq = igmc_launch_graph_step2(m, b, sp, Pc, B, 1, use_flags, inj_mask, seed, step, mult, grad_scale, out, stream);
+    const int fold = sp.tail_fold && tables && adam && at.enabled && img && !xch;
+    const int stride = (sp.cs > 1) ? ((B + 7) & ~7) : IGMC_TS_BLOCKS;
+    const int bump_seq = igmc_launch_graph_step2(m, b, sp, Pc, B, 1, use_flags, inj_mask, seed, step, mult, grad_scale, out, stream,
+                                                 fold ? 4 : 0, ctrl);
+    if (fold) {
+      launch_tail_fin(m, b, Pc, B, grad_scale, mult, grad, ARR * arr_scale, at, 8 * ny, sp.grid, stride, bump_seq, stream);
+      if (img_emitted) *img_emitted = 1;
+      return 0;
+    }
     launch_tail_ts(m, b, Pc, B, grad_scale, mult, grad, 8 * ny, sp.grid, (sp.cs > 1) ? ((B + 7) & ~7) : IGMC_TS_BLOCKS,
                    tables ? 4 : 0, ctrl, bump_seq, stream);
   } else {
diff --git a/igmc_amd/csrc/step_plan.h b/igmc_amd/csrc/step_plan.h
--- a/igmc_amd/csrc/step_plan.h
+++ b/igmc_amd/csrc/step_plan.h
@@ -11,6 +11,7 @@
   int dl_gsplit;
   int dl_head;
   int fin_mode;
+  int tail_fold;
 };
 static int step_hook(const char* name, int unset) {
   const char* e = getenv(name);
@@ -27,6 +28,7 @@
   hk.dl_gsplit = step_hook("IGMC_DL_GSPLIT", 1);
   hk.dl_head = step_hook("IGMC_DL_HEAD", 1);
   hk.fin_mode = step_hook("IGMC_FIN_MODE", 1);
+  hk.tail_fold = step_hook("IGMC_TAIL_FOLD", 1);
   return hk;
 }
 int igmc_dl_always() { return step_hook("IGMC_DL_ALWAYS", 0) == 1; }
@@ -135,6 +137,7 @@
     p->grid = (p->cs > 1) ? p->cs * ((B + 7) & ~7) : gs_grid(hk, B);
     p->tail = fts ? IGMC_TAIL_TS : IGMC_TAIL_HANDOFF;
     p->exchange_inside = fused && fts;
+    p->tail_fold = fused && fts && hk.tail_fold != 0 && m.fold_w && m.L <= 32 && 4 * m.R <= IGMC_FOLD_NA;
     p->step_form = 1;
     return;
   }
diff --git a/igmc_amd/stepgraph.py b/igmc_amd/stepgraph.py
--- a/igmc_amd/stepgraph.py
+++ b/igmc_amd/stepgraph.py
@@ -653,6 +653,9 @@
                 what.append('a step trained on an arena whose stamp is not the batch of its cursor')
             if err & 4:
                 what.append('a step trained on edge-dropout draws keyed by another batch')
+            if err & 8:
+                what.append('a hand-off between workgroups of the one-launch tail (k_tail_fin) timed out: a conv layer kept '
+                            'its parameters (GPU shared with another job? IGMC_TAIL_FOLD=0 runs the two-launch tail)')
             raise RuntimeError('device-side step control: %s (sync_err=%d); results of the affected steps are invalid'
                                % ('; '.join(what) or 'error', err))
 
```
